# 54rt1n/shardmerge

Hardware: AMD Instinct MI355X
Metric: merged-weight GB/s per GPU + % HBM roofline, Llama-3-70B 3-way FFT merge (higher is better)
Workload: dtype f32; 1 GPU; Llama-3-70B block tensors, this rank's 1/8 slice (9 per block x 10 blocks), K=3 finetunes, bf16 in/out, resident in HBM; workload_id=llama3-70b-slice, k=3, parallelism=tensor-partition x1 (no data-path collective), streams_per_gpu=8

## Files before the change

shardmerge_amd/csrc/sm_capi.inc:

```

struct smhip_ctx {
    smhip::Pipeline<SM_BACKEND> pipe;
    explicit smhip_ctx(int device) : pipe(device) {}
};

#define SM_GUARD(ctx)                      \
    if (!(ctx)) return SMHIP_ERR_ARG;      \
    (ctx)->pipe.err.clear();
#define SM_FINISH(ctx, rc)                                                        \
    do {                                                                          \
        int rc__ = (rc);                                                          \
        if (rc__ == SMHIP_OK && !(ctx)->pipe.be.ok()) {                           \
            (ctx)->pipe.err = (ctx)->pipe.be.error();                             \
            rc__ = SMHIP_ERR_HIP;                                                 \
        }                                                                         \
        return rc__;                                                              \
    } while (0)

template <class Desc, class Scalars>
static int delta_tensor_check(smhip_ctx* ctx, const char* op, const Desc* d, const void* out, const float* delta_out,
                              bool need_base, Scalars scalars) {
    auto bad = [&](const char* what) { return ctx->pipe.fail(SMHIP_ERR_ARG, std::string(op) + ": " + what); };
    if (!d) return bad("null descriptor");
    if (d->k < 1 || d->k > SMHIP_MAX_MODELS) return bad("k out of range (1..16)");
// ... 160 lines not shown
    SM_FINISH(ctx, ctx->pipe.ties_merge(*d, out, delta_out, report));
}

int smhip_dare_merge(smhip_ctx* ctx, const smhip_dare_desc* d, void* out, float* delta_out, smhip_dare_report* report,
                     void* stream) {
    SM_GUARD(ctx);
    if (int rc = delta_merge_check(ctx, "dare_merge", d, out, delta_out)) return rc;
    if (ctx->pipe.dare_threshold(d->density) == 0)
        return ctx->pipe.fail(SMHIP_ERR_ARG, "dare_merge: density is below the smallest density, 2^-16 = 1.52587890625e-05 (the mask draws 16 bits per element)");
    ctx->pipe.stream = stream;
    SM_FINISH(ctx, ctx->pipe.dare_merge(*d, out, delta_out, report));
}

int smhip_breadcrumbs_merge(smhip_ctx* ctx, const smhip_breadcrumbs_desc* d, void* out, float* delta_out,
                            smhip_breadcrumbs_report* report, void* stream) {
    SM_GUARD(ctx);
    if (int rc = delta_merge_check(ctx, "breadcrumbs_merge", d, out, delta_out)) return rc;
    if (!(d->gamma >= 0.0 && d->gamma < 1.0)) return ctx->pipe.fail(SMHIP_ERR_ARG, "breadcrumbs_merge: gamma must be in [0, 1)");
    if (!(d->density + d->gamma <= 1.0)) return ctx->pipe.fail(SMHIP_ERR_ARG, "breadcrumbs_merge: density + gamma must not exceed 1");
    ctx->pipe.stream = stream;
    SM_FINISH(ctx, ctx->pipe.breadcrumbs_merge(*d, out, delta_out, report));
}

int smhip_geo_merge(smhip_ctx* ctx, const smhip_geo_desc* d, void* out, float* delta_out, smhip_geo_report* report,
                    void* stream) {
    SM_GUARD(ctx);
    const bool weight = d && d->mode == SMHIP_GEO_SLERP;
    if (int rc = delta_tensor_check(ctx, "geo_merge", d, out, delta_out, !weight, [&]() -> const char* {
            if (d->mode < SMHIP_GEO_MODEL_STOCK || d->mode > SMHIP_GEO_SLERP) return "bad mode";
            if (d->mode == SMHIP_GEO_MODEL_STOCK) return nullptr;
            if (d->rowwise) return "rowwise is an option of mode MODEL_STOCK";
            if (d->k > 2) return "modes NUSLERP and SLERP take k <= 2";
            if (d->k == 2 && !(d->alpha[0] >= 0.0 && d->alpha[1] >= 0.0 && d->alpha[0] + d->alpha[1] > 0.0 &&
                               std::isfinite(d->alpha[0] + d->alpha[1])))
                return "modes NUSLERP and SLERP need alphas >= 0 with a sum > 0";
            return nullptr;
        }))
        return rc;
    if (d->n > 0 && (d->rows < 1 || d->n % d->rows)) return ctx->pipe.fail(SMHIP_ERR_ARG, "geo_merge: rows must divide n");
    ctx->pipe.stream = stream;
    SM_FINISH(ctx, ctx->pipe.geo_merge(*d, out, delta_out, report));
}

int smhip_slerp(smhip_ctx* ctx, const float* v0, const float* v1, size_t rows, size_t cols, float t, float* out, void* stream) {
    SM_GUARD(ctx);
    if (rows * cols > 0 && (!v0 || !v1 || !out)) return ctx->pipe.fail(SMHIP_ERR_ARG, "bad argument");
    ctx->pipe.stream = stream;
    SM_FINISH(ctx, ctx->pipe.fn_slerp(v0, v1, rows, cols, t, out));
}

int smhip_div_scalar(smhip_ctx* ctx, const void* x, int dtype, size_t n, float s, void* out, void* stream) {
    SM_GUARD(ctx);
    if (n > 0 && (!x || !out)) return ctx->pipe.fail(SMHIP_ERR_ARG, "bad argument");
    if (dtype < SMHIP_BF16 || dtype > SMHIP_F32) return ctx->pipe.fail(SMHIP_ERR_ARG, "bad dtype");
    ctx->pipe.stream = stream;
    SM_FINISH(ctx, ctx->pipe.fn_div_scalar(x, dtype, n, s, out));
}

int smhip_lora_apply(smhip_ctx* ctx, const void* base, int dtype, int rows, int cols, const void* lora_a,
                     const void* lora_b, int factor_dtype, int rank, float scale, void* out, void* stream) {
    SM_GUARD(ctx);
    if (!base || !lora_a || !lora_b || !out || rows < 1 || cols < 1) return ctx->pipe.fail(SMHIP_ERR_ARG, "bad argument");
    if (dtype < SMHIP_BF16 || dtype > SMHIP_F32 || factor_dtype < SMHIP_BF16 || factor_dtype > SMHIP_F32)
        return ctx->pipe.fail(SMHIP_ERR_ARG, "bad dtype");
    if (rank < 1 || rank > smhip::LORA_MAX_RANK) return ctx->pipe.fail(SMHIP_ERR_ARG, "rank out of range (1..512)");
    const size_t bes = dtype == SMHIP_F32 ? 4 : 2, fes = factor_dtype == SMHIP_F32 ? 4 : 2;
    const uintptr_t o0 = (uintptr_t)out, o1 = o0 + (size_t)rows * cols * bes;
    auto overlaps = [&](const void* p, size_t bytes) { return (uintptr_t)p < o1 && o0 < (uintptr_t)p + bytes; };
    if (overlaps(base, (size_t)rows * cols * bes) || overlaps(lora_a, (size_t)rank * cols * fes) ||
        overlaps(lora_b, (size_t)rows * rank * fes))
        return ctx->pipe.fail(SMHIP_ERR_ARG, "lora_apply: out overlaps an input");
    ctx->pipe.stream = stream;
    SM_FINISH(ctx, ctx->pipe.lora_apply(base, dtype, rows, cols, lora_a, lora_b, factor_dtype, rank, scale, out));
}

int smhip_adapter_apply(smhip_ctx* ctx, const smhip_adapter_desc* d, void* stream) {
    SM_GUARD(ctx);
    if (!d || !d->base || !d->lora_a || !d->lora_b || !d->out || d->rows < 1 || d->cols < 1)
        return ctx->pipe.fail(SMHIP_ERR_ARG, "bad argument");
    if (d->dtype < SMHIP_BF16 || d->dtype > SMHIP_F32 || d->factor_dtype < SMHIP_BF16 || d->factor_dtype > SMHIP_F32 ||
        (d->magnitude && (d->magnitude_dtype < SMHIP_BF16 || d->magnitude_dtype > SMHIP_F32)))
        return ctx->pipe.fail(SMHIP_ERR_ARG, "bad dtype");
    if (d->layout != SMHIP_ADAPTER_LINEAR && d->layout != SMHIP_ADAPTER_EMBEDDING)
        return ctx->pipe.fail(SMHIP_ERR_ARG, "adapter_apply: bad layout");
    if (d->magnitude && d->layout != SMHIP_ADAPTER_LINEAR)
        return ctx->pipe.fail(SMHIP_ERR_ARG, "adapter_apply: DoRA (a magnitude) needs the LINEAR layout");
    if (d->rank < 1 || d->rank > smhip::LORA_MAX_RANK) return ctx->pipe.fail(SMHIP_ERR_ARG, "rank out of range (1..512)");
    const size_t bes = d->dtype == SMHIP_F32 ? 4 : 2, fes = d->factor_dtype == SMHIP_F32 ? 4 : 2;
    const size_t mes = d->magnitude_dtype == SMHIP_F32 ? 4 : 2;
    const bool emb = d->layout == SMHIP_ADAPTER_EMBEDDING;
    const uintptr_t o0 = (uintptr_t)d->out, o1 = o0 + (size_t)d->rows * d->cols * bes;
    auto overlaps = [&](const void* p, size_t bytes) { return (uintptr_t)p < o1 && o0 < (uintptr_t)p + bytes; };
    if (overlaps(d->base, (size_t)d->rows * d->cols * bes) ||
        overlaps(d->lora_a, (size_t)d->rank * (emb ? d->rows : d->cols) * fes) ||
        overlaps(d->lora_b, (size_t)(emb ? d->cols : d->rows) * d->rank * fes) ||
        (d->magnitude && overlaps(d->magnitude, (size_t)d->rows * mes)))
        return ctx->pipe.fail(SMHIP_ERR_ARG, "adapter_apply: out overlaps an input");
    ctx->pipe.stream = stream;
    SM_FINISH(ctx, ctx->pipe.adapter_apply(d->base, d->dtype, d->rows, d->cols, d->lora_a, d->lora_b, d->factor_dtype,
                                           d->rank, d->scale, emb ? 1 : 0, d->magnitude, d->magnitude_dtype, d->out));
}

int smhip_exact_norm(smhip_ctx* ctx, const void* x, int dtype, size_t n, double* norm_out, void* stream) {
    SM_GUARD(ctx);
    if (!norm_out || (n > 0 && !x)) return ctx->pipe.fail(SMHIP_ERR_ARG, "bad argument");
    if (dtype < SMHIP_BF16 || dtype > SMHIP_F32) return ctx->pipe.fail(SMHIP_ERR_ARG, "bad dtype");
    ctx->pipe.stream = stream;
    SM_FINISH(ctx, ctx->pipe.fn_exact_norm(x, dtype, n, norm_out));
}

int smhip_correlate_pairs(smhip_ctx* ctx, int k, const void* const* tensors, int dtype, size_t rows, size_t cols,
                          float* matrix_out, void* stream) {
    SM_GUARD(ctx);
    if (!tensors || !matrix_out || rows < 1 || cols < 1) return ctx->pipe.fail(SMHIP_ERR_ARG, "bad argument");
    if (dtype < SMHIP_BF16 || dtype > SMHIP_F32) return ctx->pipe.fail(SMHIP_ERR_ARG, "bad dtype");
    for (int i = 0; i < k && i < 8; ++i)
        if (!tensors[i]) return ctx->pipe.fail(SMHIP_ERR_ARG, "null tensor");
    ctx->pipe.stream = stream;
    SM_FINISH(ctx, ctx->pipe.correlate_pairs(k, tensors, dtype, rows, cols, matrix_out));
}

int smhip_reference_cpu_norm(smhip_ctx* ctx, const void* x, const void* base, int dtype, size_t n, float* norm_out,
                             void* stream) {
    SM_GUARD(ctx);
    if (!x || !norm_out) return ctx->pipe.fail(SMHIP_ERR_ARG, "bad argument");
    if (dtype < SMHIP_BF16 || dtype > SMHIP_F32) return ctx->pipe.fail(SMHIP_ERR_ARG, "bad dtype");
    ctx->pipe.stream = stream;
    const int rc0 = ctx->pipe.reserve(1, 1);
    if (rc0) SM_FINISH(ctx, rc0);
    smhip::SigDesc sg{x, base, dtype, 1.f};
    double out = 0;
    if (!ctx->pipe.run_serial_norms(&sg, 1, n, &out))
        return ctx->pipe.fail(SMHIP_ERR_ARG, "reference_cpu norm: inputs must be 16-byte aligned");
    *norm_out = (float)out;
    SM_FINISH(ctx, SMHIP_OK);
}

int smhip_debug_option(smhip_ctx* ctx, const char* key, long value) {
    SM_GUARD(ctx);
    if (key && std::string(key) == "aten_overlap") { ctx->pipe.aten_overlap = value != 0; return SMHIP_OK; }
    if (key && std::string(key) == "emf_max_sample") { ctx->pipe.emf_max_sample = value >= 1 && value <= 4096 ? (int)value : smhip::EMF_MAX_SAMPLE; return SMHIP_OK; }
    if (key && std::string(key) == "aten_serial") { ctx->pipe.aten_serial = value != 0; return SMHIP_OK; }
    if (key && std::string(key) == "class_norms") { ctx->pipe.class_norms_mode = value >= 0 && value <= 2 ? (int)value : 1; return SMHIP_OK; }
    if (key && std::string(key) == "cand_cap") { ctx->pipe.debug_cand_cap = value > 0 ? (uint32_t)value : 0u; return SMHIP_OK; }
    if (key && std::string(key) == "sel_chunks") { ctx->pipe.debug_sel_chunks = value > 0 ? (uint32_t)value : 0u; return SMHIP_OK; }
    if (key && std::string(key) == "sel_flush_always") { ctx->pipe.debug_flush_always = value != 0; return SMHIP_OK; }
    if (key && std::string(key) == "fuse_norms") { ctx->pipe.fuse_norms = value != 0; return SMHIP_OK; }
    if (key && std::string(key) == "noise_seed") { ctx->pipe.noise_seed_base = (uint32_t)value; return SMHIP_OK; }
    if (key && std::string(key) == "spectral_intermediates") { ctx->pipe.spectral_inter = value != 0; return SMHIP_OK; }
    if (key && std::string(key) == "fuse_spec_norm") { ctx->pipe.fuse_spec_norm = value != 0; return SMHIP_OK; }
    if (key && std::string(key) == "sel_wgs_per_cu") { ctx->pipe.sel_wgs_per_cu = value > 0 ? (int)value : 5; return SMHIP_OK; }
    if (key && std::string(key) == "pair1d") { ctx->pipe.pair1d_enabled = value != 0; return SMHIP_OK; }
    if (key && std::string(key) == "spec_cull") { ctx->pipe.spec_cull = value != 0; return SMHIP_OK; }
    if (key && std::string(key) == "spec_min_bins") { ctx->pipe.spec_min_bins = value >= 0 ? (size_t)value : (size_t)1 << 20; return SMHIP_OK; }
    if (key && std::string(key) == "dftp_pairs") { ctx->pipe.dftp_pairs_enabled = value != 0; return SMHIP_OK; }
    if (key && std::string(key) == "f2s_pair") { ctx->pipe.f2s_pair = value != 0; return SMHIP_OK; }
    if (key && std::string(key) == "f1_multi") { ctx->pipe.f1_multi = value != 0; return SMHIP_OK; }
    if (key && std::string(key) == "force_bluestein") { ctx->pipe.debug_force_bluestein = value != 0; return SMHIP_OK; }
    if (key && std::string(key) == "force_split") { ctx->pipe.debug_force_split = value > 1 && value <= smhip::DFTP_MAX_P ? (int)value : 0; return SMHIP_OK; }
    if (key && std::string(key) == "fold_columns") { ctx->pipe.fold_enabled = value != 0; return SMHIP_OK; }
    if (key && std::string(key) == "fold_min_rows") { ctx->pipe.fold_min_rows = value > 0 ? (int)value : SM_FOLD_MIN_ROWS; return SMHIP_OK; }
    return ctx->pipe.fail(SMHIP_ERR_ARG, "unknown debug option");
}

int smhip_debug_query(smhip_ctx* ctx, const char* key, long* value) {
    SM_GUARD(ctx);
    if (!key || !value) return SMHIP_ERR_ARG;
    if (std::string(key) == "spec_hit") { *value = ctx->pipe.last_spec_verdict(); SM_FINISH(ctx, SMHIP_OK); }
    if (std::string(key) == "spec_checked" || std::string(key) == "spec_hits") {
        unsigned long long c = 0, h = 0;
        ctx->pipe.spec_totals(&c, &h);
        *value = (long)(std::string(key) == "spec_hits" ? h : c);
        SM_FINISH(ctx, SMHIP_OK);
    }
    if (std::string(key) == "aten_fast" || std::string(key) == "aten_group" || std::string(key) == "aten_slow") {
        unsigned long long v3[3];
        ctx->pipe.aten_stats(1, v3);
        *value = (long)v3[std::string(key) == "aten_fast" ? 0 : std::string(key) == "aten_group" ? 1 : 2];
        SM_FINISH(ctx, SMHIP_OK);
    }
    return ctx->pipe.fail(SMHIP_ERR_ARG, "unknown debug query");
}

int smhip_profile_enable(smhip_ctx* ctx, int on) { SM_GUARD(ctx); ctx->pipe.be.profile_enable(on != 0); return SMHIP_OK; }
int smhip_profile_reset(smhip_ctx* ctx) { SM_GUARD(ctx); ctx->pipe.be.profile_reset(); return SMHIP_OK; }
int smhip_profile_count(smhip_ctx* ctx) { return ctx ? ctx->pipe.be.profile_count() : 0; }
int smhip_profile_get(smhip_ctx* ctx, int i, const char** name, uint64_t* launches, double* total_ms) {
    SM_GUARD(ctx);
    return ctx->pipe.be.profile_get(i, name, launches, total_ms) ? SMHIP_OK : SMHIP_ERR_ARG;
}

}
```

shardmerge_amd/csrc/sm_kernels.hpp:

```cpp
#pragma once
#include <cmath>
#include <cstring>

#include "fft_engine.hpp"
#include "sm_aten_core.hpp"

namespace smhip {

struct cf4 { float x, y, z, w; };
struct u32x4 { uint32_t x, y, z, w; };

enum { DT_BF16 = 0, DT_F16 = 1, DT_F32 = 2 };

struct SigDesc {
    const void* x;
    const void* base;
    int dtype;
    float prescale;
};

SM_HD uint32_t umax(uint32_t a, uint32_t b) { return a > b ? a : b; }
SM_HD float u2f(uint32_t u) { float f; memcpy(&f, &u, 4); return f; }
SM_HD uint32_t f2u(float f) { uint32_t u; memcpy(&u, &f, 4); return u; }
SM_HD float bf16_to_f(uint32_t h) { return u2f(h << 16); }
// ... 1482 lines not shown
                                v *= p.post;
                                if (p.base) {
                                    v += bv[c];
                                    if (is_nan(v)) { v = 0.f; nan2++; }
                                    if (is_inf(v)) inf2 = 1;
                                }
                                o[c] = v;
                            }
                        }
                        if (p.norm_partials) {
                            float ps = 0.f;
#pragma unroll
                            for (int c = 0; c < 8; ++c) ps += o[c] * o[c];
                            ss += ps;
                        }
                        if (p.out_mode == OUT_BF16) {
                            u32x4 w;
                            w.x = pack_bf16x2(o[0], o[1]);
                            w.y = pack_bf16x2(o[2], o[3]);
                            w.z = pack_bf16x2(o[4], o[5]);
                            w.w = pack_bf16x2(o[6], o[7]);
                            ((u32x4*)p.out)[off / 8] = w;
                        } else {
                            cf4 w0 = {o[0], o[1], o[2], o[3]}, w1 = {o[4], o[5], o[6], o[7]};
                            ((cf4*)p.out)[off / 4] = w0;
                            ((cf4*)p.out)[off / 4 + 1] = w1;
                        }
                    }
                }
            } else {
#pragma unroll
                for (int q = 0; q < EMAX; ++q) {
                    const int n = t + q * T;
                    if (n < C) {
                        const size_t off = (size_t)row * C + n;
                        float v;
                        i2_finish(p, x[q], off, nan1, inf1, nan2, inf2, v);
                        ss += (double)v * v;
                        if (p.out_mode == OUT_BF16) ((uint16_t*)p.out)[off] = f_to_bf16(v);
                        else ((float*)p.out)[off] = v;
                    }
                }
            }
        });
        if (nan1) ex.global_atomic_add_u32(&p.flags[0], nan1);
        if (inf1) ex.global_atomic_or_u32(&p.flags[1], 1u);
        if (nan2) ex.global_atomic_add_u32(&p.flags[2], nan2);
        if (inf2) ex.global_atomic_or_u32(&p.flags[3], 1u);
        s.red[0] = ss; s.red[1] = 0.0;
    });
    if (p.norm_partials) {
        ex.sync();
        ex.template block_sum<2>(st, [&](const double* tot) {
            p.norm_partials[2 * (size_t)bid] = tot[0];
            p.norm_partials[2 * (size_t)bid + 1] = 0.0;
        });
    }
}

struct EmptyState { double red[8]; unsigned long long keep[8]; };

SM_HD int sgn(float v) { return (v > 0.f) - (v < 0.f); }
SM_HD bool same_sign(float a, float b) {
    const uint32_t ua = f2u(a), ub = f2u(b);
    const uint32_t ka = ua & 0x7fffffffu, kb = ub & 0x7fffffffu;
    const bool not_nan = ka <= 0x7f800000u && kb <= 0x7f800000u;
    const bool za = ka == 0u, zb = kb == 0u;
    const bool both_nonzero_same = !za && !zb && ((ua ^ ub) >> 31) == 0u;
    return not_nan && ((za && zb) || both_nonzero_same);
}


struct SelState {
    unsigned long long rank;
    uint32_t prefix;
    uint32_t level;
    float value;
    uint32_t pad;
};

struct HistParams {
    const float* X; const float* Y;
    int R, C, Cb;
    int vec4;
    int level;
    const SelState* sel;
    unsigned long long* hist;
    int chunks;
    const uint32_t* only_if;
};

SM_HD int load_quad(const float* src, size_t i0, size_t total, int vec4, float* out) {
    if (vec4) {
        const cf4 v = *(const cf4*)(src + i0);
        out[0] = v.x; out[1] = v.y; out[2] = v.z; out[3] = v.w;
        return 4;
    }
    int n = 0;
    for (int e = 0; e < 4; ++e) {
        if (i0 + e < total) { out[e] = src[i0 + e]; n = e + 1; } else out[e] = 0.f;
    }
    return n;
}

template <class Ex>
SM_HD void k_hist(Ex& ex, const HistParams& p) {
    typename Ex::template State<EmptyState> st;
    ex.init(st);
    uint32_t* lh = (uint32_t*)(ex.lds() + LDS_SCRATCH_FLOATS);
    const int nt = ex.nthreads();
    const int nbins = p.level == 1 ? HIST1_BINS : HIST_LO_BINS;
    const size_t total = (size_t)p.Cb * p.R;
    const size_t nquad = (total + 3) / 4;
    if (p.only_if && !*p.only_if) return;
    const uint32_t prefix = p.sel->prefix;
    const WeightRanges wr = weight_ranges(p.R, p.C, p.Cb);
    ex.each(st, [&](int tid, EmptyState&) { for (int b = tid; b < nbins; b += nt) lh[b] = 0; });
    ex.sync();
    ex.each(st, [&](int tid, EmptyState&) {
        const size_t start = (size_t)ex.bid() * p.chunks * nt;
        for (int c = 0; c < p.chunks; ++c) {
            const size_t qi = start + (size_t)c * nt + tid;
            if (qi >= nquad) break;
            const size_t i0 = 4 * qi;
            for (int which = 0; which < 2; ++which) {
                const float* src = which ? p.Y : p.X;
                if (!src) continue;
                float v[4];
                const int n = load_quad(src, i0, total, p.vec4, v);
#pragma unroll
                for (int e = 0; e < 4; ++e) {
                    if (e < n) {
                        const uint32_t w = weight_at(wr, i0 + e);
                        const uint32_t key = f2u(v[e]) & 0x7fffffffu;
                        if (p.level == 1) ex.lds_atomic_add(&lh[key >> 20], w);
                        else if (p.level == 2) { if ((key >> 20) == prefix) ex.lds_atomic_add(&lh[(key >> 10) & 1023u], w); }
                        else { if ((key >> 10) == prefix) ex.lds_atomic_add(&lh[key & 1023u], w); }
                    }
                }
            }
        }
    });
    ex.sync();
    ex.each(st, [&](int tid, EmptyState&) {
        for (int b = tid; b < nbins; b += nt) {
            const uint32_t v = lh[b];
            if (v) ex.global_atomic_add(&p.hist[b], (unsigned long long)v);
        }
    });
}

constexpr int STAGE_KEYS = 2048;
constexpr int STAGE_PAIRS = 1024;
struct CandLists {
    uint32_t* keys;
    cf4* pairs;
    uint32_t cap_keys, cap_pairs;
    uint32_t* counters;
};
struct BlendConsts {
    float thr;
    float dot;
    float cos_t, sin_t;
    float inv_rel;
    float pad[3];
    double s00, s01, s11;
    unsigned long long n_slerp;
};

struct Select2Params {
    const float* X; const float* Y;
    int R, C, Cb;
    int vec4;
    SelState* sel;
    const unsigned long long* hist1;
    unsigned long long rank;
    unsigned long long* hist;
    CandLists cand;
    int fuse_reduce;
    int sumsq;
    double* partials;
    int chunks;
    int flush_always;
    const uint32_t* skip;
    const float* blendB; float* blendR;
    const BlendConsts* consts; float t_sum;
    unsigned long long* hist1_out;
    const uint32_t* guess;
};

SM_HD float blend_slerp_one(const BlendConsts& c, float t_sum, float a, float b) {
    if (same_sign(a, b)) {
        if (fabsf(b) < c.thr) return a + t_sum * b;
        return a * c.cos_t + ((b - a * c.dot) * c.inv_rel) * c.sin_t;
    }
    return (fabsf(a) > fabsf(b)) ? a : b;
}

template <bool BLEND = false, class Ex>
SM_HD void k_select2(Ex& ex, const Select2Params& p) {
    typename Ex::template State<EmptyState> st;
    ex.init(st);
    uint32_t* lh = (uint32_t*)(ex.lds() + LDS_SCRATCH_FLOATS);
    uint32_t* lctl = lh + HIST_LO_BINS;
    uint32_t* lkeys = lctl + 8;
    cf4* lpairs = (cf4*)(lkeys + STAGE_KEYS);
    const int nt = ex.nthreads();
    const size_t total = (size_t)p.Cb * p.R;
    const size_t nquad = (total + 3) / 4;
    uint32_t* lh1 = lkeys + STAGE_KEYS;
    uint32_t prefix;
    BlendConsts bc;
    if constexpr (BLEND) {
        prefix = *p.guess - 1u;
        bc = *p.consts;
    } else {
        if (p.skip && *p.skip) return;
        wg_resolve(ex, st, p.hist1, HIST1_BINS, p.rank, (unsigned long long*)lkeys, lctl + 4);
        prefix = lctl[4];
        if (ex.bid() == 0) {
            ex.each(st, [&](int tid, EmptyState&) {
                if (tid == 0) {
                    p.sel->prefix = prefix; p.sel->level = 1;
                    p.sel->rank = (unsigned long long)lctl[5] | ((unsigned long long)lctl[6] << 32);
                }
            });
        }
        ex.sync();
    }
    const WeightRanges wr = weight_ranges(p.R, p.C, p.Cb);
    ex.each(st, [&](int tid, EmptyState&) {
        for (int b = tid; b < HIST_LO_BINS; b += nt) lh[b] = 0;
        if (tid < 8) lctl[tid] = 0;
        if constexpr (BLEND) for (int b = tid; b < HIST1_BINS; b += nt) lh1[b] = 0;
    });
    ex.sync();
#ifndef SM_SEL_ROUND
#define SM_SEL_ROUND 16
#endif
#ifndef SM_SEL_U
#define SM_SEL_U 4
#endif
#ifndef SM_DIAG_SEL
#define SM_DIAG_SEL 0
#endif
    constexpr int ROUND = SM_SEL_ROUND;
    ex.each(st, [&](int, EmptyState& s) { s.red[0] = s.red[1] = s.red[2] = s.red[3] = 0.0; });
    for (int r0 = 0; r0 < p.chunks; r0 += ROUND) {
    const int r1 = (r0 + ROUND < p.chunks) ? r0 + ROUND : p.chunks;
    ex.each(st, [&](int tid, EmptyState& s) {
        double s00 = 0, s01 = 0, s11 = 0, cnt = 0;
        const size_t start = (size_t)ex.bid() * p.chunks * nt;
        const bool hasY = !BLEND && p.Y != nullptr;
        auto quad = [&](size_t i0, const float* a_in, const float* b, int n, bool uniform_w) {
            float q00 = 0.f, q01 = 0.f, q11 = 0.f, qc = 0.f;
            const uint32_t w0 = weight_at(wr, i0);
            float rr[4];
            const float* a = a_in;
            if constexpr (BLEND) {
#pragma unroll
                for (int e = 0; e < 4; ++e) rr[e] = blend_slerp_one(bc, p.t_sum, a_in[e], b[e]);
                if (n == 4 && uniform_w) { cf4 v = {rr[0], rr[1], rr[2], rr[3]}; *(cf4*)(p.blendR + i0) = v; }
                else for (int e = 0; e < n; ++e) p.blendR[i0 + e] = rr[e];
                a = rr;
            }
            const uint32_t lo = prefix << 20, hi = lo + (1u << 20);
            const bool has_hi = prefix < 2047u;
            uint32_t ka[4], kb[4], wv[4];
            bool hit = false;
#pragma unroll
            for (int e = 0; e < 4; ++e) {
                wv[e] = (e < n) ? (uniform_w ? w0 : weight_at(wr, i0 + e)) : 0u;
                ka[e] = f2u(a[e]) & 0x7fffffffu;
                kb[e] = hasY ? (f2u(b[e]) & 0x7fffffffu) : 0u;
                hit = hit || ((e < n) && ((ka[e] - lo) < (1u << 20) || (hasY && (kb[e] - lo) < (1u << 20))));
            }
            if constexpr (BLEND) {
#pragma unroll
                for (int e = 0; e < 4; ++e) if (e < n) ex.lds_atomic_add(&lh1[ka[e] >> 20], wv[e]);
            }
            if (hit && !(SM_DIAG_SEL & 1)) {
#pragma unroll
                for (int e = 0; e < 4; ++e) {
                    if (e < n) {
                        const uint32_t w = wv[e];
                        if ((ka[e] - lo) < (1u << 20)) {
                            ex.lds_atomic_add(&lh[(ka[e] >> 10) & 1023u], w);
                            const uint32_t pos = ex.lds_atomic_add_ret(&lctl[0], 1u);
                            if (pos < (uint32_t)STAGE_KEYS) lkeys[pos] = ka[e] | ((w - 1u) << 31);
                        }
                        if (hasY && (kb[e] - lo) < (1u << 20)) {
                            ex.lds_atomic_add(&lh[(kb[e] >> 10) & 1023u], w);
                            const uint32_t pos = ex.lds_atomic_add_ret(&lctl[0], 1u);
                            if (pos < (uint32_t)STAGE_KEYS) lkeys[pos] = kb[e] | ((w - 1u) << 31);
                            if (p.fuse_reduce && same_sign(a[e], b[e])) {
                                const uint32_t pp = ex.lds_atomic_add_ret(&lctl[1], 1u);
                                if (pp < (uint32_t)STAGE_PAIRS) { cf4 v = {a[e], b[e], (float)w, 0.f}; lpairs[pp] = v; }
                            }
                        }
                    }
                }
            }
            if (p.sumsq) {
#pragma unroll
                for (int e = 0; e < 4; ++e) {
                    const bool in = (e < n) && has_hi && ka[e] >= hi;
                    const float av = in ? a[e] : 0.f;
                    q00 += ((float)wv[e] * av) * av;
                }
            }
            if (hasY && p.fuse_reduce && !(SM_DIAG_SEL & 2)) {
#pragma unroll
                for (int e = 0; e < 4; ++e) {
                    const bool in = (e < n) && has_hi && kb[e] >= hi && same_sign(a[e], b[e]);
                    const float wf = (float)wv[e];
                    const float av = in ? a[e] : 0.f, bv = in ? b[e] : 0.f;
                    const float wa = wf * av;
                    q00 += wa * av; q01 += wa * bv; q11 += (wf * bv) * bv; qc += in ? wf : 0.f;
                }
            }
            s00 += q00; s01 += q01; s11 += q11; cnt += qc;
        };
        if (p.vec4) {
            constexpr int U = SM_SEL_U;
            const cf4* X4 = (const cf4*)p.X;
            const cf4* Y4 = (const cf4*)(BLEND ? p.blendB : p.Y);
            for (int c0 = r0; c0 < r1; c0 += U) {
                cf4 av[U], bv[U];
                size_t qv[U];
#pragma unroll
                for (int u = 0; u < U; ++u) {
                    qv[u] = start + (size_t)(c0 + u) * nt + tid;
                    av[u] = X4[qv[u] < nquad ? qv[u] : nquad - 1];
                }
                if (hasY || BLEND) {
#pragma unroll
                    for (int u = 0; u < U; ++u) bv[u] = Y4[qv[u] < nquad ? qv[u] : nquad - 1];
                }
#pragma unroll
                for (int u = 0; u < U; ++u) {
                    if (c0 + u < r1 && qv[u] < nquad) {
                        const float a[4] = {av[u].x, av[u].y, av[u].z, av[u].w};
                        const float b[4] = {bv[u].x, bv[u].y, bv[u].z, bv[u].w};
                        quad(4 * qv[u], a, b, 4, !wr.full);
                    }
                }
            }
        } else {
            for (int c = r0; c < r1; ++c) {
                const size_t qi = start + (size_t)c * nt + tid;
                if (qi >= nquad) break;
                float a[4], b[4] = {0.f, 0.f, 0.f, 0.f};
                const int n = load_quad(p.X, 4 * qi, total, 0, a);
                if (hasY) load_quad(p.Y, 4 * qi, total, 0, b);
                if constexpr (BLEND) load_quad(p.blendB, 4 * qi, total, 0, b);
                quad(4 * qi, a, b, n, false);
            }
        }
        s.red[0] += s00; s.red[1] += s01; s.red[2] += s11; s.red[3] += cnt;
    });
    ex.sync();
    const bool last_round = r1 >= p.chunks;
    if (!last_round && !p.flush_always && lctl[0] <= (uint32_t)STAGE_KEYS / 2 && lctl[1] <= (uint32_t)STAGE_PAIRS / 2) continue;
    ex.each(st, [&](int tid, EmptyState&) {
        if (tid == 0) {
            uint32_t nk = lctl[0], np = lctl[1];
            bool over = false;
            if (nk > (uint32_t)STAGE_KEYS) { nk = STAGE_KEYS; over = true; }
            if (np > (uint32_t)STAGE_PAIRS) { np = STAGE_PAIRS; over = true; }
            const uint32_t bk = nk ? ex.global_atomic_add_ret_u32(&p.cand.counters[0], nk) : 0u;
            const uint32_t bp = np ? ex.global_atomic_add_ret_u32(&p.cand.counters[1], np) : 0u;
            if (bk + nk > p.cand.cap_keys || bp + np > p.cand.cap_pairs) over = true;
            if (over) { ex.global_atomic_or_u32(&p.cand.counters[2], 1u); if (!BLEND) ex.global_atomic_or_u32(&p.cand.counters[3], 1u); }
            lctl[0] = nk; lctl[1] = np; lctl[2] = bk; lctl[3] = bp;
        }
    });
    ex.sync();
    ex.each(st, [&](int tid, EmptyState&) {
        const uint32_t nk = lctl[0], np = lctl[1], bk = lctl[2], bp = lctl[3];
        for (uint32_t q = tid; q < nk; q += nt) if (bk + q < p.cand.cap_keys) p.cand.keys[bk + q] = lkeys[q];
        for (uint32_t q = tid; q < np; q += nt) if (bp + q < p.cand.cap_pairs) p.cand.pairs[bp + q] = lpairs[q];
    });
    ex.sync();
    ex.each(st, [&](int tid, EmptyState&) { if (tid < 4) lctl[tid] = 0; });
    ex.sync();
    }
    ex.each(st, [&](int tid, EmptyState&) {
        for (int b = tid; b < HIST_LO_BINS; b += nt) {
            const uint32_t v = lh[b];
            if (v) ex.global_atomic_add(&p.hist[b], (unsigned long long)v);
        }
        if constexpr (BLEND) {
            for (int b = tid; b < HIST1_BINS; b += nt) {
                const uint32_t v = lh1[b];
                if (v) ex.global_atomic_add(&p.hist1_out[b], (unsigned long long)v);
            }
        }
    });
    if (p.fuse_reduce || p.sumsq) {
        ex.sync();
        ex.template block_sum<4>(st, [&](const double* tot) {
            for (int q = 0; q < 4; ++q) p.partials[4 * (size_t)ex.bid() + q] = tot[q];
        });
    }
}

struct SpecCheckParams {
    const unsigned long long* hist1; unsigned long long rank;
    uint32_t* guess; uint32_t* flag;
    SelState* sel;
    unsigned long long* hist2;
    uint32_t* counters;
};
template <class Ex>
SM_HD void k_spec_check(Ex& ex, const SpecCheckParams& p) {
    typename Ex::template State<EmptyState> st;
    ex.init(st);
    const int nt = ex.nthreads();
    unsigned long long* scratch = (unsigned long long*)(ex.lds() + LDS_SCRATCH_FLOATS);
    uint32_t* res = (uint32_t*)(scratch + nt + 16);
    wg_resolve(ex, st, p.hist1, HIST1_BINS, p.rank, scratch, res);
    ex.each(st, [&](int tid, EmptyState&) {
        if (tid == 0) {
            const uint32_t g = *p.guess;
            const uint32_t hit = (g == res[0] + 1u) ? 1u : 0u;
            res[3] = hit;
            *p.flag = hit;
            p.flag[1] += 1u; p.flag[2] += hit;
            *p.guess = res[0] + 1u;
            if (hit) {
                p.sel->prefix = res[0]; p.sel->level = 1;
                p.sel->rank = (unsigned long long)res[1] | ((unsigned long long)res[2] << 32);
                if (p.counters[2]) p.counters[3] = 1u;
            }
        }
    });
    ex.sync();
    ex.each(st, [&](int tid, EmptyState&) {
        if (res[3]) return;
        for (int b = tid; b < HIST_LO_BINS; b += nt) p.hist2[b] = 0ull;
        if (tid < 3) p.counters[tid] = 0u;
    });
}

struct SumsqCandParams {
    CandLists cand;
    const float* thr;
    double* partials;
};
template <class Ex>
SM_HD void k_sumsq_cand(Ex& ex, const SumsqCandParams& p) {
    typename Ex::template State<EmptyState> st;
    ex.init(st);
    const int nt = ex.nthreads();
    const uint32_t n = p.cand.counters[2] ? 0u : p.cand.counters[0];
    const float thr = *p.thr;
    ex.each(st, [&](int tid, EmptyState& s) {
        double acc = 0;
        for (size_t q = (size_t)ex.bid() * nt + tid; q < n; q += (size_t)ex.nblocks() * nt) {
            const uint32_t v = p.cand.keys[q];
            const float x = u2f(v & 0x7fffffffu);
            if (!(x < thr)) acc += (double)(1u + (v >> 31)) * (double)x * (double)x;
        }
        s.red[0] = acc; s.red[1] = 0; s.red[2] = 0; s.red[3] = 0;
    });
    ex.template block_sum<4>(st, [&](const double* tot) {
        for (int q = 0; q < 4; ++q) p.partials[4 * (size_t)ex.bid() + q] = tot[q];
    });
}
struct SumSpecParams { const double* part4; int n4; const double* part1; int n1; double* out; uint32_t* zero_u32; int zero_u32_count; };
template <class Ex>
SM_HD void k_sum_spec(Ex& ex, const SumSpecParams& p) {
    typename Ex::template State<EmptyState> st;
    ex.init(st);
    const int nt = ex.nthreads();
    ex.each(st, [&](int tid, EmptyState& s) {
        double a0 = 0, a1 = 0;
        for (int i = tid; i < p.n4; i += nt) a0 += p.part4[4 * (size_t)i];
        for (int i = tid; i < p.n1; i += nt) a1 += p.part1[i];
        if (p.zero_u32 && tid < p.zero_u32_count) p.zero_u32[tid] = 0u;
        s.red[0] = a0; s.red[1] = a1;
    });
    ex.template block_sum<2>(st, [&](const double* tot) { p.out[0] = tot[0]; p.out[1] = tot[1]; });
}

struct Select3Params {
    CandLists cand;
    SelState* sel;
    const unsigned long long* hist2;
    unsigned long long* hist;
};
template <class Ex>
SM_HD void k_select3(Ex& ex, const Select3Params& p) {
    typename Ex::template State<EmptyState> st;
    ex.init(st);
    uint32_t* lh = (uint32_t*)(ex.lds() + LDS_SCRATCH_FLOATS);
    uint32_t* lres = lh + HIST_LO_BINS;
    unsigned long long* part = (unsigned long long*)(lres + 8);
    const int nt = ex.nthreads();
    const uint32_t n = p.cand.counters[2] ? 0u : p.cand.counters[0];
    const uint32_t prefix1 = p.sel->prefix;
    const unsigned long long rank1 = p.sel->rank;
    wg_resolve(ex, st, p.hist2, HIST_LO_BINS, rank1, part, lres);
    const uint32_t prefix = (prefix1 << 10) | lres[0];
    const unsigned long long rank2 = (unsigned long long)lres[1] | ((unsigned long long)lres[2] << 32);
    ex.each(st, [&](int tid, EmptyState&) { for (int b = tid; b < HIST_LO_BINS; b += nt) lh[b] = 0; });
    ex.sync();
    ex.each(st, [&](int tid, EmptyState&) {
        for (size_t q = (size_t)ex.bid() * nt + tid; q < n; q += (size_t)ex.nblocks() * nt) {
            const uint32_t v = p.cand.keys[q];
            const uint32_t key = v & 0x7fffffffu;
            if ((key >> 10) == prefix) ex.lds_atomic_add(&lh[key & 1023u], 1u + (v >> 31));
        }
    });
    ex.sync();
    ex.each(st, [&](int tid, EmptyState&) {
        for (int b = tid; b < HIST_LO_BINS; b += nt) {
            const uint32_t v = lh[b];
            if (v) ex.global_atomic_add(&p.hist[b], (unsigned long long)v);
        }
    });
    if (ex.bid() == 0) {
        ex.each(st, [&](int tid, EmptyState&) {
            if (tid == 0) { p.sel[1].prefix = prefix; p.sel[1].rank = rank2; p.sel[1].level = 2; }
        });
    }
}

struct ReduceCandParams {
    CandLists cand;
    const float* thr;
    double* partials;
};
template <class Ex>
SM_HD void k_reduce_cand(Ex& ex, const ReduceCandParams& p) {
    typename Ex::template State<EmptyState> st;
    ex.init(st);
    const int nt = ex.nthreads();
    const bool over = p.cand.counters[2] != 0;
    const uint32_t n = over ? 0u : p.cand.counters[1];
    const float thr = *p.thr;
    ex.each(st, [&](int tid, EmptyState& s) {
        double s00 = 0, s01 = 0, s11 = 0, cnt = 0;
        for (size_t q = (size_t)ex.bid() * nt + tid; q < n; q += (size_t)ex.nblocks() * nt) {
            const cf4 v = p.cand.pairs[q];
            if (!(fabsf(v.y) < thr)) {
                s00 += (double)v.z * v.x * v.x; s01 += (double)v.z * v.x * v.y; s11 += (double)v.z * v.y * v.y; cnt += v.z;
            }
        }
        s.red[0] = s00; s.red[1] = s01; s.red[2] = s11; s.red[3] = cnt;
    });
    ex.template block_sum<4>(st, [&](const double* tot) {
        for (int q = 0; q < 4; ++q) p.partials[4 * (size_t)ex.bid() + q] = tot[q];
    });
}

template <class Ex, class StT>
SM_HD void wg_resolve(Ex& ex, StT& st, const unsigned long long* hist, int nbins, unsigned long long rank,
                      unsigned long long* part, uint32_t* res) {
    using S = typename StT::value_type;
    const int nt = ex.nthreads();
    const int per = (nbins + nt - 1) / nt;
    unsigned long long* grp = part + nt;
    ex.each(st, [&](int tid, S& s) {
        unsigned long long sum = 0;
#pragma unroll
        for (int q = 0; q < 8; ++q) {
            const int b = tid * per + q;
            const unsigned long long h = (q < per && b < nbins) ? hist[b] : 0ull;
            s.keep[q] = h;
            sum += h;
        }
        part[tid] = sum;
        if (tid == 0) { res[0] = 0; res[1] = 0; res[2] = 0; }
    });
    ex.sync();
    ex.each(st, [&](int tid, S&) {
        if (tid < 16) {
// ... 428 lines not shown
            }
            if (p.hist) {
                const uint32_t w0 = weight_at(wr, i0);
#pragma unroll
                for (int e = 0; e < 4; ++e) {
                    if (e < n) {
                        const uint32_t key = f2u(r[e]) & 0x7fffffffu;
                        ex.lds_atomic_add(&lh[key >> 20], (vec && !wr.full) ? w0 : weight_at(wr, i0 + e));
                    }
                }
            }
        };
        if (p.vec4) {
            constexpr int U = 4;
            const cf4* A4 = (const cf4*)p.reA;
            const cf4* B4 = (const cf4*)p.reB;
            for (int q0 = 0; q0 < p.chunks; q0 += U) {
                cf4 av[U], bv[U];
                size_t qv[U];
#pragma unroll
                for (int u = 0; u < U; ++u) {
                    qv[u] = start + (size_t)(q0 + u) * nt + tid;
                    av[u] = A4[qv[u] < nquad ? qv[u] : nquad - 1];
                }
#pragma unroll
                for (int u = 0; u < U; ++u) bv[u] = B4[qv[u] < nquad ? qv[u] : nquad - 1];
#pragma unroll
                for (int u = 0; u < U; ++u) {
                    if (q0 + u < p.chunks && qv[u] < nquad) {
                        const float a[4] = {av[u].x, av[u].y, av[u].z, av[u].w};
                        const float b[4] = {bv[u].x, bv[u].y, bv[u].z, bv[u].w};
                        quad(4 * qv[u], a, b, 4, true);
                    }
                }
            }
        } else {
            for (int q = 0; q < p.chunks; ++q) {
                const size_t qi = start + (size_t)q * nt + tid;
                if (qi >= nquad) break;
                float a[4], b[4];
                const int n = load_quad(p.reA, 4 * qi, total, 0, a);
                load_quad(p.reB, 4 * qi, total, 0, b);
                quad(4 * qi, a, b, n, false);
            }
        }
    });
    if (p.hist) {
        ex.sync();
        ex.each(st, [&](int tid, EmptyState&) {
            for (int b = tid; b < HIST1_BINS; b += nt) {
                const uint32_t v = lh[b];
                if (v) ex.global_atomic_add(&p.hist[b], (unsigned long long)v);
            }
        });
    }
}

struct SpecNormParams {
    const float* re; const float* im;
    int R, C, Cb;
    int vec4;
    const float* thr;
    double* partials;
    int chunks;
};
template <class Ex>
SM_HD void k_spec_norm(Ex& ex, const SpecNormParams& p) {
    typename Ex::template State<EmptyState> st;
    ex.init(st);
    const int nt = ex.nthreads();
    const size_t total = (size_t)p.Cb * p.R;
    const size_t nquad = (total + 3) / 4;
    const float thr = p.thr ? *p.thr : 0.f;
    const WeightRanges wr = weight_ranges(p.R, p.C, p.Cb);
    ex.each(st, [&](int tid, EmptyState& s) {
        double sr = 0, si = 0;
        const size_t start = (size_t)ex.bid() * p.chunks * nt;
        for (int c = 0; c < p.chunks; ++c) {
            const size_t qi = start + (size_t)c * nt + tid;
            if (qi >= nquad) break;
            const size_t i0 = 4 * qi;
            float a[4], b[4];
            const int n = load_quad(p.re, i0, total, p.vec4, a);
            load_quad(p.im, i0, total, p.vec4, b);
            float qr = 0.f, qi2 = 0.f;
#pragma unroll
            for (int e = 0; e < 4; ++e) {
                if (e < n) {
                    const float w = (float)weight_at(wr, i0 + e);
                    if (!(fabsf(a[e]) < thr)) qr += w * a[e] * a[e];
                    qi2 += w * b[e] * b[e];
                }
            }
            sr += qr; si += qi2;
        }
        s.red[0] = sr; s.red[1] = si;
    });
    ex.template block_sum<2>(st, [&](const double* tot) {
        p.partials[2 * (size_t)ex.bid()] = tot[0];
        p.partials[2 * (size_t)ex.bid() + 1] = tot[1];
    });
}

SM_HD uint32_t hash_u32(uint32_t x) {
    x ^= x >> 16; x *= 0x7feb352du; x ^= x >> 15; x *= 0x846ca68bu; x ^= x >> 16;
    return x;
}
SM_HD float model_noise(uint32_t seed, size_t i, float sigma) {
    const uint32_t h1 = hash_u32((uint32_t)i * 2u + 1u + seed * 0x9e3779b9u) ^ hash_u32((uint32_t)(i >> 31) + seed);
    const uint32_t h2 = hash_u32(h1 + 0x68bc21ebu);
    if ((h2 >> 24) < 21u) return 0.f;
    const float s4 = (float)(h1 & 0xffffu) + (float)(h1 >> 16) + (float)(h2 & 0xffffu) + (float)(hash_u32(h2) >> 16);
    return sigma * 1.7320508f * (s4 * (1.0f / 65536.0f) - 2.0f);
}

struct SpecRescaleParams {
    const float* re; const float* im;
    float* dre; float* dim;
    int R, C, Cb;
    int vec4;
    float thr;
    float scale;
    float sigma; uint32_t seed;
    unsigned long long* hist;
    int chunks;
    double* im_partials;
};
template <class Ex>
SM_HD void k_spec_rescale(Ex& ex, const SpecRescaleParams& p) {
    typename Ex::template State<EmptyState> st;
    ex.init(st);
    uint32_t* lh = (uint32_t*)(ex.lds() + LDS_SCRATCH_FLOATS);
    const int nt = ex.nthreads();
    const size_t total = (size_t)p.Cb * p.R;
    const size_t nquad = (total + 3) / 4;
    const WeightRanges wr = weight_ranges(p.R, p.C, p.Cb);
    if (p.hist) {
        ex.each(st, [&](int tid, EmptyState&) { for (int b = tid; b < HIST1_BINS; b += nt) lh[b] = 0; });
        ex.sync();
    }
    ex.each(st, [&](int tid, EmptyState& s) {
        double imacc = 0.0;
        const size_t start = (size_t)ex.bid() * p.chunks * nt;
        for (int c = 0; c < p.chunks; ++c) {
            const size_t qi = start + (size_t)c * nt + tid;
            if (qi >= nquad) break;
            const size_t i0 = 4 * qi;
            float a[4], b[4] = {0.f, 0.f, 0.f, 0.f};
            const int n = load_quad(p.re, i0, total, p.vec4, a);
            if (p.im) load_quad(p.im, i0, total, p.vec4, b);
            float r[4], im[4];
#pragma unroll
            for (int e = 0; e < 4; ++e) {
                r[e] = (fabsf(a[e]) < p.thr) ? model_noise(p.seed, i0 + e, p.sigma) : a[e] * p.scale;
                im[e] = b[e] * p.scale;
            }
            if (p.vec4) {
                cf4 v = {r[0], r[1], r[2], r[3]};
                *(cf4*)(p.dre + i0) = v;
                if (p.im) { cf4 vi = {im[0], im[1], im[2], im[3]}; *(cf4*)(p.dim + i0) = vi; }
            } else {
                for (int e = 0; e < n; ++e) { p.dre[i0 + e] = r[e]; if (p.im) p.dim[i0 + e] = im[e]; }
            }
            if (p.hist) {
#pragma unroll
                for (int e = 0; e < 4; ++e)
                    if (e < n) ex.lds_atomic_add(&lh[(f2u(r[e]) & 0x7fffffffu) >> 20], weight_at(wr, i0 + e));
            }
            if (p.im_partials) {
                float q = 0.f;
#pragma unroll
                for (int e = 0; e < 4; ++e)
                    if (e < n) q += (float)weight_at(wr, i0 + e) * im[e] * im[e];
                imacc += q;
            }
        }
        s.red[0] = imacc;
    });
    if (p.hist) {
        ex.sync();
        ex.each(st, [&](int tid, EmptyState&) {
            for (int b = tid; b < HIST1_BINS; b += nt) {
                const uint32_t v = lh[b];
                if (v) ex.global_atomic_add(&p.hist[b], (unsigned long long)v);
            }
        });
    }
    if (p.im_partials) {
        ex.sync();
        ex.template block_sum<1>(st, [&](const double* tot) { p.im_partials[ex.bid()] = tot[0]; });
    }
}

constexpr int NORMS_MAX = 16;
constexpr int NORMS_K = 8;
struct DeltaNormsParams {
    int k;
    const void* ft[NORMS_K];
    const void* ubase[2];
    int base_of[NORMS_K];
    int dtype;
    size_t n;
    int chunks;
    double* partials;
};
template <class Ex>
SM_HD void k_delta_norms(Ex& ex, const DeltaNormsParams& p) {
    typename Ex::template State<NormsState> st;
    ex.init(st);
    const int nt = ex.nthreads();
    const size_t noct = p.n / 8;
    const u32x4* b0 = (const u32x4*)p.ubase[0];
    const u32x4* b1 = (const u32x4*)(p.ubase[1] ? p.ubase[1] : p.ubase[0]);
    ex.each(st, [&](int tid, NormsState& s) {
        double acc[NORMS_K];
#pragma unroll
        for (int i = 0; i < NORMS_K; ++i) acc[i] = 0.0;
        const size_t start = (size_t)ex.bid() * p.chunks * nt;
        for (int q = 0; q < p.chunks; ++q) {
            const size_t oi = start + (size_t)q * nt + tid;
            if (oi >= noct) break;
            u32x4 rf[NORMS_K];
            const u32x4 r0 = b0[oi], r1 = b1[oi];
#pragma unroll
            for (int i = 0; i < NORMS_K; ++i) rf[i] = ((const u32x4*)p.ft[i < p.k ? i : 0])[oi];
            float v0[8], v1[8];
            decode16x8(r0, p.dtype, v0);
            decode16x8(r1, p.dtype, v1);
#pragma unroll
            for (int i = 0; i < NORMS_K; ++i) {
                float vf[8];
                decode16x8(rf[i], p.dtype, vf);
                const bool second = p.base_of[i] != 0;
                float ps = 0.f;
#pragma unroll
                for (int e = 0; e < 8; ++e) {
                    const float d = vf[e] - (second ? v1[e] : v0[e]);
                    ps += d * d;
                }
                if (i < p.k) acc[i] += ps;
            }
        }
#pragma unroll
        for (int i = 0; i < NORMS_MAX; ++i) s.red[i] = i < NORMS_K ? acc[i < NORMS_K ? i : 0] : 0.0;
    });
    ex.template block_sum<NORMS_MAX>(st, [&](const double* tot) {
        for (int i = 0; i < NORMS_MAX; ++i) p.partials[(size_t)ex.bid() * NORMS_MAX + i] = tot[i];
    });
}
constexpr int SER_CHUNK = 4096;
struct SerialNormParams {
    int k;
    SigDesc sig[16];
    size_t n;
    float* out;
};
template <class Ex>
SM_HD void k_serial_norm(Ex& ex, const SerialNormParams& p) {
    typename Ex::template State<EmptyState> st;
    ex.init(st);
    float* buf = ex.lds() + LDS_SCRATCH_FLOATS;
    const int nt = ex.nthreads();
    const SigDesc sg = p.sig[ex.bid()];
    const size_t nchunks = (p.n + SER_CHUNK - 1) / SER_CHUNK;
    auto stage = [&](size_t c, int which) {
        ex.each(st, [&](int tid, EmptyState&) {
            float* dst = buf + which * SER_CHUNK;
            for (int o = tid; o < SER_CHUNK / 8; o += nt) {
                const size_t i0 = c * SER_CHUNK + (size_t)o * 8;
                float v[8];
                if (i0 < p.n) load_sig8(sg, i0, v);
                else { for (int e = 0; e < 8; ++e) v[e] = 0.f; }
#pragma unroll
                for (int e = 0; e < 8; ++e) dst[o * 8 + e] = v[e];
            }
        });
    };
    ex.each(st, [&](int, EmptyState& s) { s.red[0] = 0.0; });
    if (nchunks) stage(0, 0);
    ex.sync();
    for (size_t c = 0; c < nchunks; ++c) {
        const int cur = (int)(c & 1);
        if (c + 1 < nchunks) stage(c + 1, cur ^ 1);
        ex.each(st, [&](int tid, EmptyState& s) {
            if (tid < 8) {
                float acc = (float)s.red[0];
                const float* src = buf + cur * SER_CHUNK + tid;
                const size_t left = p.n - c * SER_CHUNK;
                const int rows = (int)((left < (size_t)SER_CHUNK ? left : (size_t)SER_CHUNK) / 8);
                int r = 0;
                for (; r + 16 <= rows; r += 16) {
                    float x[16];
#pragma unroll
                    for (int q = 0; q < 16; ++q) x[q] = src[(r + q) * 8];
#pragma unroll
                    for (int q = 0; q < 16; ++q) acc = fmaf(x[q], x[q], acc);
                }
                for (; r < rows; ++r) acc = fmaf(src[r * 8], src[r * 8], acc);
                s.red[0] = (double)acc;
            }
        });
        ex.sync();
    }
    float* lanes = buf;
    ex.each(st, [&](int tid, EmptyState& s) { if (tid < 8) lanes[tid] = (float)s.red[0]; });
    ex.sync();
    ex.each(st, [&](int tid, EmptyState&) {
// ... 1098 lines not shown
```

shardmerge_amd/csrc/sm_pipeline.hpp:

```cpp
#pragma once
#include <algorithm>
#include <cmath>
#include <cstdio>
#include <map>
#include <string>
#include <vector>

#include "../../include/shardmerge_hip.h"
#include "sm_kernels.hpp"
#include "sm_aten_norm.hpp"
#include "sm_bluestein.hpp"
#include "sm_lora.hpp"
#include "sm_ties.hpp"
#include "sm_dare.hpp"
#include "sm_breadcrumbs.hpp"
#include "sm_geo.hpp"

namespace smhip {

#define SM_KERNEL_TAG(Tag, ParamsT, NAME, CALL)                                      \
    struct Tag {                                                                     \
        using Params = ParamsT;                                                      \
        static constexpr int waves = 4;                                              \
        static constexpr int max_threads = 1024;                                     \
        static const char* name() { return NAME; }                                   \
        template <class Ex> static SM_HD void run(Ex& ex, const Params& p) { CALL; } \
    };
#define SM_KERNEL_TAG_LB(Tag, ParamsT, NAME, CALL, MAXT, WAVES)                      \
    struct Tag {                                                                     \
        using Params = ParamsT;                                                      \
        static constexpr int waves = WAVES;                                          \
        static constexpr int max_threads = MAXT;                                     \
        static const char* name() { return NAME; }                                   \
        template <class Ex> static SM_HD void run(Ex& ex, const Params& p) { CALL; } \
    };
template <class P, int GROUPS> constexpr int fft_max_threads() {
    if constexpr (P::is_static) return (GROUPS * P::T < 256) ? 256 : (GROUPS * P::T > 1024 ? 1024 : GROUPS * P::T);
    else return 1024;
}
#ifndef SM_W3_MAX_THREADS
#define SM_W3_MAX_THREADS 256
#endif
#define SM_FFT_KERNEL_TAG(Tag, ParamsT, NAME, CALL, GROUPS, WAVES)                   \
    template <class P> struct Tag {                                                  \
        using Params = ParamsT;                                                      \
        static constexpr int waves = (WAVES < 4 && P::is_static && fft_max_threads<P, GROUPS>() <= SM_W3_MAX_THREADS) ? WAVES : 4; \
        static constexpr int max_threads = waves < 4 ? fft_max_threads<P, GROUPS>() : 1024; \
        static const char* name() { return NAME; }                                   \
        template <class Ex> static SM_HD void run(Ex& ex, const Params& p) { CALL; } \
    };
SM_FFT_KERNEL_TAG(KF1, F1Params, "f1_rows_fwd", k_f1<P>(ex, p), 1, 3)
SM_FFT_KERNEL_TAG(KF2, F2Params, "f2_cols_fwd", (k_f2<P, f2_bins<P>()>(ex, p)), 2 * f2_bins<P>(), 4)
SM_FFT_KERNEL_TAG(KI1x1, I1Params, "i1_cols_inv", (k_i1<P, 1>(ex, p)), 1, 4)
SM_FFT_KERNEL_TAG(KI1x2, I1Params, "i1_cols_inv", (k_i1<P, i1_bins<P>()>(ex, p)), i1_bins<P>(), 4)
SM_FFT_KERNEL_TAG(KI2, I2Params, "i2_rows_inv", k_i2<P>(ex, p), 1, 4)
SM_FFT_KERNEL_TAG(KF2S, F2SParams, "f2s_cols_fwd1", (k_f2s<P, f2s_groups<P>()>(ex, p)), f2s_groups<P>(), 4)
SM_FFT_KERNEL_TAG(KF1Q, F1Params, "f1_rows_fwd", k_f1q<P>(ex, p), 4, 4)
SM_FFT_KERNEL_TAG(KF2Q, F2Params, "f2_cols_fwd", (k_f2<P, f2_bins<P>(), true>(ex, p)), 2 * f2_bins<P>(), 4)
SM_FFT_KERNEL_TAG(KF2SQ, F2SParams, "f2s_cols_fwd1", (k_f2s<P, f2s_groups<P>(), true>(ex, p)), f2s_groups<P>(), 4)
SM_FFT_KERNEL_TAG(KI1x1Q, I1Params, "i1_cols_inv", (k_i1<P, 1, true>(ex, p)), 1, 4)
SM_FFT_KERNEL_TAG(KI1x2Q, I1Params, "i1_cols_inv", (k_i1<P, i1_bins<P>(), true>(ex, p)), i1_bins<P>(), 4)
#define SM_BLUE_KERNEL_TAG(Tag, ParamsT, NAME, CALL)                                 \
    template <class P> struct Tag {                                                  \
        using Params = ParamsT;                                                      \
        static constexpr int max_threads = fft_max_threads<P, 1>();                  \
        static constexpr int waves = max_threads > 512 ? 4 : 2;                      \
        static const char* name() { return NAME; }                                   \
        template <class Ex> static SM_HD void run(Ex& ex, const Params& p) { CALL; } \
    };
SM_BLUE_KERNEL_TAG(KF1B, F1BParams, "f1_rows_fwd", k_f1b<P>(ex, p))
SM_BLUE_KERNEL_TAG(KI2B, I2BParams, "i2_rows_inv", k_i2b<P>(ex, p))
SM_FFT_KERNEL_TAG(KPair1d, Pair1dParams, "pair_1d", k_pair1d<P>(ex, p), 1, 1)

#ifndef SM_COLS_MAX_THREADS
#define SM_COLS_MAX_THREADS 1024
#endif
#ifndef SM_F2_MAX_THREADS
#define SM_F2_MAX_THREADS 512
#endif
#ifndef SM_R14336
#define SM_R14336 16, 16, 8, 7
#endif
#ifndef SM_R7168
#define SM_R7168 32, 32, 7
#endif
#ifndef SM_T8192
#define SM_T8192 256
#define SM_W8192 4
#define SM_R8192 32, 16, 16
#endif
#define SM_STATIC_PLANS(X)                 \
    X(SPlan<1024, 64, false, 4, 32, 32>)       \
    X(SPlan<2048, 64, false, 4, 16, 16, 8>)    \
    X(SPlan<4096, 128, false, 4, 16, 16, 16>)  \
    X(SPlan<8192, SM_T8192, false, SM_W8192, SM_R8192>)  \
    X(SPlan<16384, 512, false, 4, 32, 32, 16>)\
    X(SPlan<14336, 512, false, 4, SM_R14336>) \
    X(SPlan<28672, 1024, false, 4, 16, 16, 16, 7>) \
    X(SPlan<3072, 128, false, 4, 16, 16, 4, 3>)    \
    X(SPlan<3584, 128, false, 4, 16, 32, 7>)       \
    X(SPlan<5120, 256, false, 4, 16, 16, 4, 5>)    \
    X(SPlan<6144, 256, false, 4, 16, 16, 8, 3>)    \
    X(SPlan<7168, 256, false, 4, SM_R7168>)    \
    X(SPlan<12288, 512, false, 4, 16, 16, 16, 3>)  \
    X(SPlan<13824, 512, false, 4, 32, 16, 3, 3, 3>) \
    X(SPlan<27648, 1024, false, 4, 32, 32, 3, 3, 3>) \
    X(SPlan<2304, 128, false, 4, 16, 16, 3, 3>) \
    X(SPlan<256, 64, false, 4, 8, 8, 4>)            \
    X(SPlan<512, 64, false, 4, 32, 16>)             \
    X(SPlan<64, 64, false, 4, 8, 8>)                \
    X(SPlan<128, 64, false, 4, 16, 8>)

inline bool plan_uses_cx(int N) { (void)N; return false; }

template <class PL> inline void plan_from_static(int N, int& T, std::vector<int>& radices, bool& found) {
    if (!found && PL::N == N) {
        T = PL::T; radices.clear();
        for (int i = 0; i < PL::npass; ++i) radices.push_back(PL::radix(i));
        found = true;
    }
}
inline bool plan_shape_static(int N, int& T, std::vector<int>& radices) {
    bool found = false;
#define SM_PLAN_FROM(...) plan_from_static<__VA_ARGS__>(N, T, radices, found);
    SM_STATIC_PLANS(SM_PLAN_FROM)
#undef SM_PLAN_FROM
    return found;
}

template <class PL>
inline bool plan_matches(const FftPlanDev& pl) {
    if (pl.N != PL::N || pl.T != PL::T || pl.npass != PL::npass || pl.lds_floats != PL::lds_floats || (pl.cx != 0) != PL::cx) return false;
    for (int i = 0; i < PL::npass; ++i)
        if (pl.radix[i] != PL::radix(i)) return false;
    return true;
}
SM_KERNEL_TAG(KF2R1, F2Params, "f2_cols_fwd", k_f2_r1(ex, p))
SM_KERNEL_TAG(KI1R1, I1Params, "i1_cols_inv", k_i1_r1(ex, p))
SM_KERNEL_TAG(KPublish, PublishParams, "publish", k_publish(ex, p))
SM_KERNEL_TAG(KHist, HistParams, "select_hist", k_hist(ex, p))
SM_KERNEL_TAG(KScan, ScanParams, "select_scan", k_scan(ex, p))
SM_KERNEL_TAG(KSelect2, Select2Params, "select_lvl2", k_select2<false>(ex, p))
SM_KERNEL_TAG(KSelect2Cull, Select2Params, "select_lvl2_cull", k_select2<false>(ex, p))
SM_KERNEL_TAG(KBlendSel, Select2Params, "blend", k_select2<true>(ex, p))
SM_KERNEL_TAG(KSpecCheck, SpecCheckParams, "select_spec_check", k_spec_check(ex, p))
SM_KERNEL_TAG(KSelect3, Select3Params, "select_lvl3_cand", k_select3(ex, p))
SM_KERNEL_TAG(KReduceCand, ReduceCandParams, "slerp_reduce_cand", k_reduce_cand(ex, p))
SM_KERNEL_TAG(KReduce, ReduceParams, "slerp_reduce", k_reduce(ex, p))
SM_KERNEL_TAG(KSlerpConsts, SlerpConstParams, "slerp_consts", k_slerp_consts(ex, p))
SM_KERNEL_TAG_LB(KClassEmf, ClassEmfParams, "class_norm_stats", k_class_emf(ex, p), 256, 2)
SM_KERNEL_TAG(KSumPartials, SumPartialsParams, "sum_partials", k_sum_partials(ex, p))
SM_KERNEL_TAG(KDeltaNorms, DeltaNormsParams, "delta_norms", k_delta_norms(ex, p))
SM_KERNEL_TAG(KSumPartialsN, SumNParams, "sum_partials", k_sum_partials_n(ex, p))
SM_KERNEL_TAG(KBlend, BlendParams, "blend", k_blend(ex, p))
SM_KERNEL_TAG(KCombine, CombineParams, "combine", k_combine(ex, p))
SM_KERNEL_TAG(KExpand, ExpandParams, "expand_full", k_expand(ex, p))
SM_KERNEL_TAG(KPack, PackParams, "pack_planes", k_pack(ex, p))
SM_KERNEL_TAG(KSplit, SplitParams, "split_complex", k_split(ex, p))
SM_KERNEL_TAG(KJoin, JoinParams, "join_complex", k_join(ex, p))
SM_KERNEL_TAG(KCull, CullParams, "cull_inplace", k_cull(ex, p))
SM_KERNEL_TAG(KAddition, AdditionParams, "addition_merge", k_addition(ex, p))
SM_KERNEL_TAG(KFnSums, FnSumsParams, "fn_slerp_sums", k_fn_sums(ex, p))
SM_KERNEL_TAG(KFnSlerpFin, FnSlerpFinParams, "fn_slerp_consts", k_fn_slerp_fin(ex, p))
SM_KERNEL_TAG(KFnSlerpRows0, FnSlerpRowsParams, "fn_slerp_relnorm", k_fn_slerp_rows<0>(ex, p))
SM_KERNEL_TAG(KFnSlerpRows1, FnSlerpRowsParams, "fn_slerp_out", k_fn_slerp_rows<1>(ex, p))
SM_KERNEL_TAG(KFnSlerpDen, FnSlerpDenParams, "fn_slerp_den", k_fn_slerp_den(ex, p))
SM_KERNEL_TAG(KSumsqAny, SumsqAnyParams, "fn_sumsq", k_sumsq_any(ex, p))
SM_KERNEL_TAG(KDivScalar, DivScalarParams, "fn_div_scalar", k_div_scalar(ex, p))
SM_KERNEL_TAG(KCorrPartial, CorrPartialParams, "correlate_pairs", k_corr_partial(ex, p))
SM_KERNEL_TAG(KCorrFinish, CorrFinishParams, "correlate_finish", k_corr_finish(ex, p))
SM_KERNEL_TAG(KSerialNorm, SerialNormParams, "serial_norm", k_serial_norm(ex, p))
SM_KERNEL_TAG(KSpecNorm, SpecNormParams, "spec_norm", k_spec_norm(ex, p))
SM_KERNEL_TAG(KSumsqCand, SumsqCandParams, "spec_norm_cand", k_sumsq_cand(ex, p))
SM_KERNEL_TAG(KSumSpec, SumSpecParams, "spec_norm_sum", k_sum_spec(ex, p))
SM_KERNEL_TAG(KSpecRescale, SpecRescaleParams, "spec_rescale", k_spec_rescale(ex, p))
SM_KERNEL_TAG(KDftp, DftpParams, "dft_across_slices", k_dftp(ex, p))
SM_KERNEL_TAG(KDftpPairs, DftpParams, "dft_across_slices", k_dftp_pairs(ex, p))
SM_KERNEL_TAG(KTranspose, TransposeParams, "transpose", k_transpose(ex, p))
SM_KERNEL_TAG_LB(KLoraPack, LoraPackParams, "lora_pack", k_lora_pack(ex, p), 256, 4)
SM_KERNEL_TAG_LB(KLoraBf16, LoraApplyParams, "lora_apply", k_lora_apply<DT_BF16>(ex, p), 256, 2)
SM_KERNEL_TAG_LB(KLoraF16, LoraApplyParams, "lora_apply", k_lora_apply<DT_F16>(ex, p), 256, 2)
SM_KERNEL_TAG_LB(KLoraF32, LoraApplyParams, "lora_apply", k_lora_apply<DT_F32>(ex, p), 256, 2)
SM_KERNEL_TAG_LB(KDoraNormBf16, LoraApplyParams, "dora_norm", k_dora_norm<DT_BF16>(ex, p), 256, 2)
SM_KERNEL_TAG_LB(KDoraNormF16, LoraApplyParams, "dora_norm", k_dora_norm<DT_F16>(ex, p), 256, 2)
SM_KERNEL_TAG_LB(KDoraNormF32, LoraApplyParams, "dora_norm", k_dora_norm<DT_F32>(ex, p), 256, 2)
SM_KERNEL_TAG_LB(KDoraScale, DoraScaleParams, "dora_scale", k_dora_scale(ex, p), DORA_SCALE_THREADS, 4)
SM_KERNEL_TAG_LB(KDoraApplyBf16, LoraApplyParams, "dora_apply", k_dora_apply<DT_BF16>(ex, p), 256, 2)
SM_KERNEL_TAG_LB(KDoraApplyF16, LoraApplyParams, "dora_apply", k_dora_apply<DT_F16>(ex, p), 256, 2)
SM_KERNEL_TAG_LB(KDoraApplyF32, LoraApplyParams, "dora_apply", k_dora_apply<DT_F32>(ex, p), 256, 2)
SM_KERNEL_TAG_LB(KTiesHist, TiesHistParams, "ties_hist", k_ties_hist(ex, p), 256, 4)
SM_KERNEL_TAG_LB(KTiesSelect, TiesSelectParams, "ties_select", k_ties_select(ex, p), TIES_SELECT_THREADS, 4)
SM_KERNEL_TAG_LB(KTiesMerge, TiesMergeParams, "ties_merge", k_ties_merge(ex, p), 256, 4)
SM_KERNEL_TAG_LB(KDareMerge, DareMergeParams, "dare_merge", k_dare_merge(ex, p), 256, 4)
SM_KERNEL_TAG_LB(KCrumbsHist, CrumbsHistParams, "crumbs_hist", k_crumbs_hist(ex, p), 256, 4)
SM_KERNEL_TAG_LB(KCrumbsSelect, CrumbsSelectParams, "crumbs_select", k_crumbs_select(ex, p), TIES_SELECT_THREADS, 4)
SM_KERNEL_TAG_LB(KCrumbsMerge, CrumbsMergeParams, "crumbs_merge", k_crumbs_merge(ex, p), 256, 4)
SM_KERNEL_TAG_LB(KGeoGram, GeoGramParams, "geo_gram", k_geo_gram<false>(ex, p), GEO_THREADS, 4)
SM_KERNEL_TAG_LB(KGeoGramTiled, GeoGramParams, "geo_gram", k_geo_gram<true>(ex, p), GEO_THREADS, 2)
SM_KERNEL_TAG_LB(KGeoFold, GeoFoldParams, "geo_gram_fold", k_geo_fold(ex, p), 256, 4)
SM_KERNEL_TAG_LB(KGeoCoef, GeoCoefParams, "geo_coef", k_geo_coef(ex, p), 256, 4)
SM_KERNEL_TAG_LB(KGeoCombine, GeoCombineParams, "geo_combine", k_geo_combine(ex, p), 256, 4)
SM_KERNEL_TAG_LB(KAtenPre, AtenPreParams, "aten_norm_pre", k_aten_pre<0>(ex, p), 256, 4)
SM_KERNEL_TAG_LB(KAtenPreC, AtenPreParams, "aten_norm_pre", k_aten_pre<1>(ex, p), 256, 4)
SM_KERNEL_TAG_LB(KAtenScan, AtenScanParams, "aten_norm_scan", k_aten_scan(ex, p), 256, 4)
SM_KERNEL_TAG_LB(KAtenRec, AtenRecParams, "aten_norm_rec", k_aten_rec(ex, p), 256, 4)
#ifndef SM_ATEN_PART_WAVES
#define SM_ATEN_PART_WAVES 3
#endif
SM_KERNEL_TAG_LB(KAtenPart16, AtenPartParams, "aten_norm_part", k_aten_part<ATEN_PART_RAW16>(ex, p), 256, SM_ATEN_PART_WAVES)
SM_KERNEL_TAG_LB(KAtenPart32, AtenPartParams, "aten_norm_part", k_aten_part<ATEN_PART_RAW32>(ex, p), 256, SM_ATEN_PART_WAVES)
SM_KERNEL_TAG_LB(KAtenPart, AtenPartParams, "aten_norm_part", k_aten_part<ATEN_PART_SIGNAL>(ex, p), 256, 2)
SM_KERNEL_TAG_LB(KAtenPartC, AtenPartParams, "aten_norm_part", k_aten_part<ATEN_PART_CLASS>(ex, p), 256, 2)
SM_KERNEL_TAG_LB(KAtenWalk, AtenWalkParams, "aten_norm_walk", k_aten_walk<0>(ex, p), 256, 4)
SM_KERNEL_TAG_LB(KAtenWalkC, AtenWalkParams, "aten_norm_walk", k_aten_walk<1>(ex, p), 256, 4)
SM_KERNEL_TAG_LB(KAtenFinish, AtenFinishParams, "aten_norm_finish", k_aten_finish(ex, p), 256, 4)
#define SM_SIDE_KERNELS_0(X) X(KAtenPre) X(KAtenPreC) X(KAtenScan) X(KAtenRec) X(KAtenPart16) X(KAtenPart32) X(KAtenPart) X(KAtenPartC) X(KAtenWalk) X(KAtenWalkC) X(KAtenFinish)
#define SM_SIDE_KERNELS_1(X) X(KF2R1) X(KI1R1) X(KPublish) X(KHist) X(KScan) X(KSelect2) X(KSelect2Cull) X(KBlendSel) \
    X(KSpecCheck) X(KSelect3) X(KReduceCand) X(KReduce) X(KSlerpConsts) X(KSumPartials) X(KClassEmf)
#define SM_SIDE_KERNELS_2(X) X(KDeltaNorms) X(KSumPartialsN) X(KBlend) X(KCombine) X(KExpand) X(KPack) X(KSplit) X(KJoin) \
    X(KCull) X(KAddition) X(KFnSums) X(KFnSlerpFin) X(KFnSlerpRows0) X(KFnSlerpRows1) X(KFnSlerpDen) X(KSumsqAny) X(KDivScalar) X(KCorrPartial) X(KCorrFinish) X(KSerialNorm) X(KSpecNorm) X(KSumsqCand) X(KSumSpec)       \
    X(KSpecRescale) X(KDftp) X(KDftpPairs) X(KTranspose) X(KLoraPack) X(KLoraBf16) X(KLoraF16) X(KLoraF32) \
    X(KDoraNormBf16) X(KDoraNormF16) X(KDoraNormF32) X(KDoraScale) X(KDoraApplyBf16) X(KDoraApplyF16) X(KDoraApplyF32)
#define SM_SIDE_KERNELS_7(X) X(KTiesHist) X(KTiesSelect) X(KTiesMerge) X(KDareMerge) X(KCrumbsHist) X(KCrumbsSelect) X(KCrumbsMerge) \
    X(KGeoGram) X(KGeoGramTiled) X(KGeoFold) X(KGeoCoef) X(KGeoCombine)
#define SM_SIDE_GROUPS 8

struct HostPlan {
    FftPlanDev dev;
    bool ok = false;
};

inline bool plan_radices(int N, int T, std::vector<int>& out) {
    out.clear();
    if (N == 1) { out.push_back(1); return true; }
    int rest = N, a = 0;
    while (rest % 2 == 0) { rest /= 2; ++a; }
    std::vector<int> odd;
    for (int p : {3, 5, 7, 11, 13})
        while (rest % p == 0) { rest /= p; odd.push_back(p); }
    if (rest != 1) return false;
    if (a > 0) {
        const int np = (a + 4) / 5;
        const int base = a / np, extra = a % np;
        for (int i = 0; i < np; ++i) out.push_back(1 << (base + (i < extra ? 1 : 0)));
    }
    for (int p : odd) out.push_back(p);
    if ((int)out.size() > MAX_PASSES) return false;
    for (int r : out) {
        const int nb = N / r;
        const int per = (nb + T - 1) / T;
        if (per * r > EMAX) return false;
    }
    return true;
}


inline bool plan_shape(int N, int& T, std::vector<int>& radices) {
    if (N < 1 || N > EMAX * 1024) return false;
    if (plan_shape_static(N, T, radices)) return true;
    int t0 = ((N + EMAX - 1) / EMAX + 63) / 64 * 64;
    if (t0 < 64) t0 = 64;
    for (T = t0; T <= 1024; T += 64)
        if (plan_radices(N, T, radices)) return true;
    return false;
}

inline bool rough_split(int N, int& p, int& M) {
    int T;
    std::vector<int> rad;
    if (plan_shape(N, T, rad)) { p = 1; M = N; return true; }
    for (p = 2; p <= DFTP_MAX_P; ++p) {
        if (N % p) continue;
        M = N / p;
        if (M % 2 == 0 && plan_shape(M, T, rad)) return true;
    }
    return false;
}
inline int bluestein_len(int C) {
    if (C < 2) return 0;
    for (int L = 256; L <= EMAX * 1024; L *= 2)
        if (L >= 2 * C - 1) return L;
    return 0;
}
inline int shape_support(int rows, int cols, bool* transposed = nullptr) {
    int T, p, M;
    std::vector<int> rad;
    if (transposed) *transposed = false;
    if (rows < 1 || cols < 1) return 0;
    if (plan_shape(cols, T, rad) && rough_split(rows, p, M)) return 1;
    if (plan_shape(rows, T, rad) && rough_split(cols, p, M)) { if (transposed) *transposed = true; return 1; }
    if (bluestein_len(cols) && rough_split(rows, p, M)) return 1;
    if (bluestein_len(rows) && rough_split(cols, p, M)) { if (transposed) *transposed = true; return 1; }
    return 0;
}

struct Buffer {
    void* p = nullptr;
    size_t cap = 0;
};

struct ProfEntry { std::string name; uint64_t launches = 0; double ms = 0; };

inline size_t round_up(size_t v, size_t m) { return (v + m - 1) / m * m; }

struct PairOut {
    void* out = nullptr; int out_mode = OUT_F32;
    const void* base = nullptr; int base_dtype = DT_BF16;
    float post = 1.f;
    int ifft_policy = 1;
};

template <class B>
class Pipeline {
  public:
    B be;
    std::string err;
    void* stream = nullptr;
    uint32_t debug_cand_cap = 0;
    uint32_t debug_sel_chunks = 0;
    bool debug_flush_always = false;
    bool spec_cull = true;
    size_t spec_min_bins = 1 << 20;
    bool dftp_pairs_enabled = true;
    int debug_force_split = 0;
    int sel_wgs_per_cu = 5;
    bool safe_select = false;
    uint32_t noise_seed_base = 0;
    bool spectral_inter = true;
    bool f2s_pair = true;
    size_t f2s_pair_max_bins = (size_t)64 << 20;
    bool f1_multi = true;
    bool fuse_spec_norm = true;
    float noise_sigma = 1.2e-7f;

    explicit Pipeline(int device) : be(device) {}
    ~Pipeline() {
        for (auto& kv : plans_) if (kv.second.dev.tw) be.free((void*)kv.second.dev.tw);
        for (Buffer* b : {&cand_, &t1_, &small_, &tmpA_, &tmpB_, &tmpC_, &fullS_, &saveR_, &saveI_, &aten_, &emf_, &lora_, &dora_, &ties_}) if (b->p) be.free(b->p);
        for (Buffer& b : pool_) if (b.p) be.free(b.p);
        if (mail_) be.free_host(mail_);
        for (Buffer& b : inter_) if (b.p) be.free(b.p);
        for (Buffer& b : rowspec_) if (b.p) be.free(b.p);
        for (Buffer& b : tr_) if (b.p) be.free(b.p);
        for (auto& kv : rough_tw_) if (kv.second) be.free(kv.second);
        for (auto& kv : blue_) { if (kv.second.chirp) be.free(kv.second.chirp); if (kv.second.filt) be.free(kv.second.filt); }
    }

    int fail(int code, const std::string& msg) { err = msg; return code; }

    int get_plan(int N, FftPlanDev& out) {
        auto it = plans_.find(N);
        if (it == plans_.end()) {
            HostPlan hp;
            int T;
            std::vector<int> rad;
            if (plan_shape(N, T, rad)) {
                hp.ok = true;
                hp.dev.N = N; hp.dev.T = T; hp.dev.npass = (int)rad.size();
                for (int i = 0; i < MAX_PASSES; ++i) hp.dev.radix[i] = i < (int)rad.size() ? rad[i] : 1;
                hp.dev.cx = plan_uses_cx(N) ? 1 : 0;
                hp.dev.lds_floats = hp.dev.cx ? (int)round_up((size_t)2 * (N + (N >> 4) + 1), 32)
                                              : (int)round_up((size_t)lpad(N) + 1, 32);
                std::vector<cf2> tw(N);
                for (int j = 0; j < N; ++j) {
                    const double ang = -2.0 * M_PI * (double)j / (double)N;
                    tw[j].x = (float)cos(ang); tw[j].y = (float)sin(ang);
                }
                void* d = be.alloc(sizeof(cf2) * N);
                if (!d) return fail(SMHIP_ERR_NOMEM, "twiddle alloc failed");
                be.h2d(d, tw.data(), sizeof(cf2) * N, stream);
                hp.dev.tw = (const cf2*)d;
            } else {
                hp.dev.tw = nullptr;
            }
            it = plans_.emplace(N, hp).first;
        }
        if (!it->second.ok) {
            char buf[256];
            snprintf(buf, sizeof buf, "unsupported transform length %d (a row length needs factors in {2,3,5,7,11,13} and <= %d; the layer merge "
                                       "also takes p * M column lengths, p <= %d)", N, EMAX * 1024, DFTP_MAX_P);
            return fail(SMHIP_ERR_SHAPE, buf);
        }
        out = it->second.dev;
        return SMHIP_OK;
    }

    int ensure(Buffer& b, size_t bytes) {
        if (b.cap >= bytes) return SMHIP_OK;
        if (b.p) { be.sync(stream); be.free(b.p); b.p = nullptr; b.cap = 0; }
        b.p = be.alloc(bytes);
        if (!b.p) return fail(SMHIP_ERR_NOMEM, "workspace allocation failed");
        b.cap = bytes;
        return SMHIP_OK;
    }
    size_t workspace_bytes() const {
        size_t t = cand_.cap + t1_.cap + small_.cap + tmpA_.cap + tmpB_.cap + tmpC_.cap + fullS_.cap + saveR_.cap + saveI_.cap + aten_.cap + emf_.cap + lora_.cap + dora_.cap + ties_.cap;
        for (const Buffer& b : inter_) t += b.cap;
        for (const Buffer& b : rowspec_) t += b.cap;
        for (const Buffer& b : pool_) t += b.cap;
        for (const Buffer& b : tr_) t += b.cap;
        return t;
    }

    struct Geo {
        int R, C, Cb, pitch4, pitchG, ilv;
        size_t plane_floats;
        bool full;
        int Cw;
        int fold;
        int batch;
        size_t t1_slice;
        int rough;
    };
#ifndef SM_FOLD_MIN_ROWS
#define SM_FOLD_MIN_ROWS 14336
#endif
    int fold_min_rows = SM_FOLD_MIN_ROWS;
    bool fold_shape(int R, int C) const {
        if (R < fold_min_rows || !(R == 8192 || R == 14336 || R == 16384 || R == 28672)) return false;
        int T; std::vector<int> rad;
        if (!plan_shape_static(C, T, rad)) return false;
        return 4 * T <= 1024 && (C / T) % 2 == 0 && C % 8 == 0;
    }
    bool fold_enabled = true;
    Geo geo(int R, int C, bool full = false, bool allow_fold = false, int batch = 1) const {
        Geo g;
        g.R = R; g.C = C; g.full = full;
        g.batch = batch < 1 ? 1 : batch;
        g.fold = (allow_fold && fold_enabled && !full && g.batch == 1 && fold_shape(R, C) && !row_bluestein(C)) ? 4 : 1;
        g.Cb = full ? C : (C / 2 + 1) * g.batch;
        g.pitch4 = (int)round_up((size_t)(C / 2 + 1), 8);
        g.t1_slice = round_up((size_t)R, 8) * (size_t)g.pitch4;
        g.pitchG = g.pitch4;
        g.ilv = t1_interleave(R);
        g.plane_floats = round_up((size_t)g.Cb * R, 64);
        g.Cw = full ? -1 : C;
        g.rough = 1;
        return g;
    }
#ifndef SM_T1_ILV
#define SM_T1_ILV 2
#endif
#ifndef SM_T1_ILV_MIN_ROWS
#define SM_T1_ILV_MIN_ROWS 8192
#endif
    static int t1_interleave(int R) { return t1_interleave_rows(R); }
    static constexpr int MAXGRID_PART = 1 << 20;
    int reserve(int R, int C, bool full = false, int batch = 1) {
        const Geo g = geo(R, C, full, false, batch);
        int rc;
        if ((rc = ensure(t1_, g.t1_slice * g.batch * sizeof(cf4)))) return rc;
        for (int i = 0; i < 4; ++i)
            if ((rc = ensure(pool_[pidx_[i]], g.plane_floats * sizeof(float)))) return rc;
        {
            const size_t ck = std::max<size_t>(1 << 16, g.plane_floats / 4), cp = std::max<size_t>(1 << 15, g.plane_floats / 16);
            if ((rc = ensure(cand_, ck * 4 + cp * 16))) return rc;
            cap_keys_ = (uint32_t)std::min<size_t>(ck, 0xffffffffu); cap_pairs_ = (uint32_t)std::min<size_t>(cp, 0xffffffffu);
        }
        if (!small_.p) {
            if ((rc = ensure(small_, SMALL_BYTES))) return rc;
            be.memset(small_.p, 0, SMALL_BYTES, stream);
            if (!mail_) mail_ = (Mailbox*)be.alloc_host(sizeof(Mailbox));
            if (!mail_) return fail(SMHIP_ERR_NOMEM, "host mailbox");
        }
        return SMHIP_OK;
    }
    static constexpr size_t OFF_HIST = 0;
    static constexpr size_t OFF_SEL = OFF_HIST + 8 * (HIST1_BINS + 2 * HIST_LO_BINS);
    static constexpr size_t OFF_CONSTS = OFF_SEL + 2 * sizeof(SelState);
    static constexpr size_t OFF_THR = OFF_CONSTS + 256;
    static constexpr size_t OFF_FLAGS = OFF_THR + 64;
    static constexpr size_t OFF_CANDCTR = OFF_FLAGS + 32;
    static constexpr size_t OFF_NORM2 = OFF_FLAGS + 64;
    static constexpr size_t OFF_PART = OFF_NORM2 + 64;
    static constexpr size_t PART_DOUBLES = 4 * 65536 + 2 * 40000;
    static constexpr size_t OFF_PART_IM = OFF_PART + PART_DOUBLES * 8;
    static constexpr size_t PART_IM_DOUBLES = 131072;
    static constexpr size_t OFF_SPEC = OFF_PART_IM + PART_IM_DOUBLES * 8;
    static constexpr size_t SMALL_BYTES = OFF_SPEC + 64;
    unsigned long long* d_hist() { return (unsigned long long*)((char*)small_.p + OFF_HIST); }
    unsigned long long* d_hist2() { return d_hist() + HIST1_BINS; }
    unsigned long long* d_hist3() { return d_hist2() + HIST_LO_BINS; }
    SelState* d_sel(int i) { return (SelState*)((char*)small_.p + OFF_SEL) + i; }
    BlendConsts* d_consts() { return (BlendConsts*)((char*)small_.p + OFF_CONSTS); }
    float* d_thr(int i) { return (float*)((char*)small_.p + OFF_THR) + i; }
    uint32_t* d_flags() { return (uint32_t*)((char*)small_.p + OFF_FLAGS); }
    uint32_t* d_candctr() { return (uint32_t*)((char*)small_.p + OFF_CANDCTR); }
    CandLists cand_lists() {
        CandLists c;
        c.keys = (uint32_t*)cand_.p; c.pairs = (cf4*)((char*)cand_.p + (size_t)cap_keys_ * 4);
        c.cap_keys = cap_keys_; c.cap_pairs = cap_pairs_; c.counters = d_candctr();
        if (debug_cand_cap) { c.cap_keys = std::min(c.cap_keys, debug_cand_cap); c.cap_pairs = std::min(c.cap_pairs, debug_cand_cap); }
        return c;
    }
    double* d_norm2() { return (double*)((char*)small_.p + OFF_NORM2); }
    double* d_part() { return (double*)((char*)small_.p + OFF_PART); }
    double* d_part_im() { return (double*)((char*)small_.p + OFF_PART_IM); }
    uint32_t* d_spec_guess(int slot) { return (uint32_t*)((char*)small_.p + OFF_SPEC) + (slot < 0 ? 0 : slot > 7 ? 7 : slot); }
    uint32_t* d_spec_flag() { return (uint32_t*)((char*)small_.p + OFF_SPEC) + 8; }
    float* plane(const Geo&, int i) { return (float*)pool_[pidx_[i]].p; }
    enum { P_REA = 0, P_IMA = 1, P_REB = 2, P_RER = 3 };
    int pool_acquire(size_t bytes) {
        int id = -1;
        for (size_t q = 0; q < pool_.size(); ++q) if (!pool_busy_[q]) { id = (int)q; break; }
        if (id < 0) { pool_.emplace_back(); pool_busy_.push_back(0); id = (int)pool_.size() - 1; }
        if (ensure(pool_[id], bytes)) return -1;
        pool_busy_[id] = 1;
        return id;
    }
    void pool_release(int id) { if (id >= 0) pool_busy_[id] = 0; }

    static bool is_static_plan(const FftPlanDev& pl) {
        bool found = false;
#define SM_IS_PLAN(...) if (plan_matches<__VA_ARGS__>(pl)) found = true;
        SM_STATIC_PLANS(SM_IS_PLAN)
#undef SM_IS_PLAN
        return found;
    }
    static int f2_bins_host(const FftPlanDev& pl) { return is_static_plan(pl) ? f2_bins_for(pl.T, pl.N) : 1; }
    static int i1_bins_host(const FftPlanDev& pl) {
        if (2 * pl.T > SM_F2_MAX_THREADS) return 1;
        return is_static_plan(pl) ? i1_bins_for(pl.T) : 2;
    }

    template <template <class> class KT, class Params>
    void launch_fft(const FftPlanDev& pl, int grid, int block, size_t lds, const Params& p, bool allow_static = true) {
        bool done = !allow_static;
#define SM_TRY_PLAN(...)                                                     \
        if (!done && plan_matches<__VA_ARGS__>(pl)) {                        \
            be.template launch<KT<__VA_ARGS__>>(grid, block, lds, p, stream);\
            done = true;                                                     \
        }
        SM_STATIC_PLANS(SM_TRY_PLAN)
#undef SM_TRY_PLAN
        if (!done || !allow_static) be.template launch<KT<DynPlan>>(grid, block, lds, p, stream);
    }

    static int pick_chunks(size_t units, int block, int min_chunks, int wgs_per_cu = 5) {
        const size_t target = (size_t)256 * wgs_per_cu;
        size_t c = (units + (size_t)block * target - 1) / ((size_t)block * target);
        if (c < (size_t)min_chunks) c = min_chunks;
        if (c > 4096) c = 4096;
        return (int)c;
    }
    static int stream_grid(size_t units, int block, int chunks) {
        const size_t per = (size_t)block * chunks;
        size_t g = (units + per - 1) / per;
        return (int)std::max<size_t>(g, 1);
    }
    static bool aligned16(const void* p) { return ((uintptr_t)p & 15) == 0; }
    static int vec4(const Geo& g) { return g.full ? (((size_t)g.R * g.C) % 4 == 0) : (g.R % 4 == 0); }

    bool debug_force_bluestein = false;
    bool row_bluestein(int C) const {
        int T; std::vector<int> rad;
        if (debug_force_bluestein) return bluestein_len(C) > 0;
        return !plan_shape(C, T, rad) && bluestein_len(C) > 0;
    }
    struct BlueHost { void* chirp = nullptr; void* filt = nullptr; int L = 0; };
    int bluestein_tables(int C, BluesteinTab& out, FftPlanDev& plan) {
        const int L = bluestein_len(C);
        if (!L) return fail(SMHIP_ERR_SHAPE, "row length too long for the chirp-z transform");
        int rc = get_plan(L, plan);
        if (rc) return rc;
        auto it = blue_.find(C);
        if (it == blue_.end()) {
            std::vector<double> wr(C), wi(C);
            for (int n = 0; n < C; ++n) {
                const unsigned long long m = ((unsigned long long)n * (unsigned long long)n) % (2ull * (unsigned long long)C);
                const double ang = -M_PI * (double)m / (double)C;
                wr[n] = cos(ang); wi[n] = sin(ang);
            }
            std::vector<double> hr(L, 0.0), hi(L, 0.0);
            for (int m = 0; m < C; ++m) {
                hr[m] = wr[m]; hi[m] = -wi[m];
                if (m) { hr[L - m] = wr[m]; hi[L - m] = -wi[m]; }
            }
            for (int i = 1, j = 0; i < L; ++i) {
                int bit = L >> 1;
                for (; j & bit; bit >>= 1) j ^= bit;
                j ^= bit;
                if (i < j) { std::swap(hr[i], hr[j]); std::swap(hi[i], hi[j]); }
            }
            for (int len = 2; len <= L; len <<= 1) {
                const int half = len / 2;
                for (int k = 0; k < half; ++k) {
                    const double ang = -2.0 * M_PI * (double)k / (double)len;
                    const double cr = cos(ang), ci = sin(ang);
                    for (int i = k; i < L; i += len) {
                        const int j = i + half;
                        const double tr = hr[j] * cr - hi[j] * ci, ti = hr[j] * ci + hi[j] * cr;
                        hr[j] = hr[i] - tr; hi[j] = hi[i] - ti;
                        hr[i] += tr; hi[i] += ti;
                    }
                }
            }
            std::vector<cf2> chirp(C), filt(L);
            for (int n = 0; n < C; ++n) { chirp[n].x = (float)wr[n]; chirp[n].y = (float)wi[n]; }
            for (int k = 0; k < L; ++k) { filt[k].x = (float)(hr[k] / L); filt[k].y = (float)(hi[k] / L); }
            BlueHost bh;
            bh.L = L;
            bh.chirp = be.alloc(sizeof(cf2) * C);
            bh.filt = be.alloc(sizeof(cf2) * L);
            if (!bh.chirp || !bh.filt) return fail(SMHIP_ERR_NOMEM, "chirp table alloc failed");
            be.h2d(bh.chirp, chirp.data(), sizeof(cf2) * C, stream);
            be.h2d(bh.filt, filt.data(), sizeof(cf2) * L, stream);
            be.sync(stream);
            it = blue_.emplace(C, bh).first;
        }
        out.chirp = (const cf2*)it->second.chirp; out.filt = (const cf2*)it->second.filt;
        return SMHIP_OK;
    }
    int get_row_plan(int C, FftPlanDev& plan, bool& blue, BluesteinTab& bt) {
        blue = row_bluestein(C);
        bt.chirp = nullptr; bt.filt = nullptr;
        return blue ? bluestein_tables(C, bt, plan) : get_plan(C, plan);
    }

    int rough_twiddles(int N, const cf2** out) {
        auto it = rough_tw_.find(N);
        if (it == rough_tw_.end()) {
            std::vector<cf2> tw(N);
            for (int j = 0; j < N; ++j) {
                const double ang = -2.0 * M_PI * (double)j / (double)N;
                tw[j].x = (float)cos(ang); tw[j].y = (float)sin(ang);
            }
            void* d = be.alloc(sizeof(cf2) * N);
            if (!d) return fail(SMHIP_ERR_NOMEM, "twiddle alloc failed");
            be.h2d(d, tw.data(), sizeof(cf2) * N, stream);
            be.sync(stream);
            it = rough_tw_.emplace(N, d).first;
        }
        *out = (const cf2*)it->second;
        return SMHIP_OK;
    }
    int run_dftp(const Geo& g, void* buf, bool rowpair, int ilv, int pitch, size_t slice_stride, bool inverse) {
        DftpParams q;
        int rc = rough_twiddles(g.R * g.rough, &q.tw);
        if (rc) return rc;
        q.buf = (cf4*)buf; q.p = g.rough; q.M = g.R; q.units = rowpair ? g.R / 2 : g.R; q.rowpair = rowpair ? 1 : 0;
        q.ilv = ilv; q.pitch = pitch; q.ncols = g.C / 2 + 1; q.slice_stride = slice_stride; q.inverse = inverse ? 1 : 0;
        q.cols = DFTP_COLS;
        if (q.p <= DFTP_PAIR_MAX_P && dftp_pairs_enabled) {
            q.cols = dftp_pairs_cols(q.p);
            const int ntp = (q.ncols + q.cols - 1) / q.cols;
            const size_t ldsp = LDS_SCRATCH_FLOATS * 4 + dftp_pairs_lds_bytes(q.p) + ((size_t)(q.p / 2 + 1) + 64) * sizeof(cf2);
            be.template launch<KDftpPairs>((q.units + DFTP_UNITS - 1) / DFTP_UNITS * ntp, 256, ldsp, q, stream);
            return SMHIP_OK;
        }
        const int ntiles = (q.ncols + DFTP_COLS - 1) / DFTP_COLS;
        const size_t lds = LDS_SCRATCH_FLOATS * 4 + (size_t)q.p * DFTP_COLS * sizeof(cf4) + (size_t)q.p * sizeof(cf2);
        be.template launch<KDftp>(q.units * ntiles, 256, lds, q, stream);
// ... 106 lines not shown
        double* const pbase = p.partials;
        if (multi) {
            for (int i = 0; i < nm; ++i) multi->partials[i] = pbase + (size_t)i * 2 * grid;
            multi->b_off = (long long)((size_t)g.C * dt_size(sig.dtype));
            p.sigs = *multi;
            launch_fft<KF1>(p.plan, grid * nm, p.nb * p.plan.T, lds, p, true);
            if (grid_out) *grid_out = grid;
            return SMHIP_OK;
        }
        for (int bi = 0; bi < nlaunch; ++bi) {
            p.a = sig_at(a, (size_t)bi * g.R * g.C); p.b = sig_at(b, (size_t)bi * g.R * g.C);
            p.t1 = t1base + (size_t)bi * (g.t1_slice / 2);
            p.partials = pbase + (size_t)bi * 2 * grid;
            if (blue) { F1BParams q; q.f = p; q.bt = bt; launch_fft<KF1B>(p.plan, grid, p.plan.T, lds, q); }
            else launch_fft<KF1>(p.plan, grid, p.nb * p.plan.T, lds, p, p.vec != 0);
        }
        if (grid_out) *grid_out = grid * nlaunch;
        if (g.rough > 1) return run_dftp(g, t1base, true, F2S_ILV, g.pitch4, g.t1_slice / 2, false);
        return SMHIP_OK;
    }
    struct F2SSecond { const void* t1; bool role_a; float scale; };
    int run_f2s(const Geo& g, bool role_a, float scale, bool hist, const void* t1buf = nullptr, int* im_parts = nullptr,
                const F2SSecond* second = nullptr) {
        F2SParams p;
        p.two = 0; p.t1_2 = nullptr; p.role_a_2 = 0; p.scale_2 = 0.f; p.re_2 = nullptr;
        if (second) {
            if (g.batch != 1 || second->role_a == role_a) return fail(SMHIP_ERR_ARG, "internal: paired column pass");
            p.two = 1; p.t1_2 = (const cf4*)second->t1; p.role_a_2 = second->role_a ? 1 : 0; p.scale_2 = second->scale;
            p.re_2 = plane(g, second->role_a ? P_REA : P_REB);
        }
        const int nsg = second ? 2 : 1;
        const int Rt = g.R / g.fold;
        int rc = get_plan(Rt, p.plan);
        if (rc) return rc;
        p.t1 = (const cf4*)(t1buf ? t1buf : t1_.p); p.pitch4 = g.pitch4 * g.fold; p.R = Rt; p.C = g.C;
        p.Cb = g.fold == 4 ? 4 * g.pitch4 : g.C / 2 + 1;
        p.slab = g.pitch4; p.Cb_real = g.C / 2 + 1; p.Rfull = g.R; p.slab_elems = fold_slab_elems(g, true);
        p.role_a = role_a ? 1 : 0; p.scale = scale;
        p.re = plane(g, role_a ? P_REA : P_REB); p.im = plane(g, P_IMA);
        p.hist = hist ? d_hist() : nullptr;
        const bool st = is_static_plan(p.plan);
        const int G = st ? (f2_nsig_for(p.plan.T) == 2 ? 2 * f2_bins_for(p.plan.T, p.plan.N) : 1) : 1;
        const int xg = G >= 8 ? 1 : 8 / G;
        const int grid = (int)round_up((size_t)(p.Cb + G - 1) / G, 8 * xg) * nsg;
        const size_t lds = (LDS_SCRATCH_FLOATS + (size_t)G * p.plan.lds_floats + HIST1_BINS) * 4;
        const bool any_a = role_a || (second && second->role_a);
        const bool want_im = im_parts && any_a && (size_t)grid * g.batch <= PART_IM_DOUBLES;
        if (im_parts) *im_parts = want_im ? grid * g.batch : -1;
        p.im_partials = want_im ? d_part_im() : nullptr;
        if (g.fold == 4) { launch_fft<KF2SQ>(p.plan, grid, G * p.plan.T, lds, p); return SMHIP_OK; }
        if (g.batch > 1) { p.sl.wgs = grid; p.sl.t1_stride = g.t1_slice / 2; p.sl.plane_stride = (size_t)(g.C / 2 + 1) * g.R; }
        launch_fft<KF2S>(p.plan, grid * g.batch, G * p.plan.T, lds, p);
        return SMHIP_OK;
    }
    void run_spec_norm(const Geo& g, const float* re, const float* im, const float* thr, double& sre, double& sim) {
        const size_t total = (size_t)g.Cb * g.R;
        SpecNormParams q;
        q.re = re; q.im = im; q.R = g.R; q.C = g.Cw; q.Cb = g.Cb; q.vec4 = vec4(g); q.thr = thr;
        q.chunks = pick_chunks((total + 3) / 4, 256, 8, 8);
        int grid = stream_grid((total + 3) / 4, 256, q.chunks);
        while ((size_t)grid * 2 > PART_DOUBLES) { q.chunks *= 2; grid = stream_grid((total + 3) / 4, 256, q.chunks); }
        q.partials = d_part();
        be.template launch<KSpecNorm>(grid, 256, LDS_SCRATCH_FLOATS * 4, q, stream);
        SumPartialsParams sp;
        sp.partials = d_part(); sp.nparts = grid; sp.out = mail_->norm2;
        be.template launch<KSumPartials>(1, 1024, LDS_SCRATCH_FLOATS * 4, sp, stream);
        PublishParams pp;
        pp.flags = d_flags(); pp.thr = d_thr(0); pp.consts = d_consts(); pp.mail = mail_; pp.zero_flags = nullptr;
        be.template launch<KPublish>(1, 64, LDS_SCRATCH_FLOATS * 4, pp, stream);
        be.sync(stream);
        sre = mail_->norm2[0]; sim = mail_->norm2[1];
    }
    void run_spec_rescale(const Geo& g, const float* re, const float* im, float thr, float scale, bool role_a, bool hist,
                          int* im_parts = nullptr) {
        const size_t total = (size_t)g.Cb * g.R;
        SpecRescaleParams q;
        q.re = re; q.im = role_a ? im : nullptr;
        q.dre = plane(g, role_a ? P_REA : P_REB); q.dim = plane(g, P_IMA);
        q.R = g.R; q.C = g.Cw; q.Cb = g.Cb; q.vec4 = vec4(g);
        q.thr = thr; q.scale = scale; q.sigma = noise_sigma; q.seed = ++noise_seed_;
        q.hist = hist ? d_hist() : nullptr;
        q.chunks = pick_chunks((total + 3) / 4, 256, 8, 8);
        const int grid = stream_grid((total + 3) / 4, 256, q.chunks);
        const bool want_im = im_parts && role_a && (size_t)grid <= PART_IM_DOUBLES;
        if (im_parts) *im_parts = want_im ? grid : -1;
        q.im_partials = want_im ? d_part_im() : nullptr;
        be.template launch<KSpecRescale>(grid, 256, (LDS_SCRATCH_FLOATS + HIST1_BINS) * 4, q, stream);
    }
    void run_spec_norm_fused(int sel_parts, int im_parts, double& sre, double& sim) {
        SumsqCandParams sc;
        sc.cand = cand_lists(); sc.thr = d_thr(1); sc.partials = d_part() + 4 * (size_t)sel_parts;
        be.template launch<KSumsqCand>(CAND_GRID, 256, LDS_SCRATCH_FLOATS * 4, sc, stream);
        SumSpecParams sp;
        sp.part4 = d_part(); sp.n4 = sel_parts + CAND_GRID; sp.part1 = d_part_im(); sp.n1 = im_parts; sp.out = mail_->norm2;
        sp.zero_u32 = d_candctr(); sp.zero_u32_count = 3;
        be.template launch<KSumSpec>(1, 1024, LDS_SCRATCH_FLOATS * 4, sp, stream);
        PublishParams pp;
        pp.flags = d_flags(); pp.thr = d_thr(0); pp.consts = d_consts(); pp.mail = mail_; pp.zero_flags = nullptr;
        be.template launch<KPublish>(1, 64, LDS_SCRATCH_FLOATS * 4, pp, stream);
        be.sync(stream);
        sre = mail_->norm2[0]; sim = mail_->norm2[1];
    }

    void read_norms(int grid, double& na, double& nb) {
        SumPartialsParams sp;
        sp.partials = d_part(); sp.nparts = grid; sp.out = mail_->norm2;
        be.template launch<KSumPartials>(1, 1024, LDS_SCRATCH_FLOATS * 4, sp, stream);
        be.sync(stream);
        na = std::sqrt(mail_->norm2[0]); nb = std::sqrt(mail_->norm2[1]);
    }

    int run_f2(const Geo& g, float scale0, float scale1, int swap, bool hist) {
        F2Params p;
        int rc = get_plan(g.R, p.plan);
        if (rc) return rc;
        if (g.R == 1) {
            p.slab = g.pitch4; p.Cb_real = g.C / 2 + 1; p.Rfull = 1; p.slab_elems = 0;
            p.t1 = (const cf4*)t1_.p; p.pitch4 = g.pitch4; p.ilv = 1; p.R = 1; p.C = g.C; p.Cb = g.C / 2 + 1; p.nsig = 2;
            p.swap = swap; p.scale[0] = scale0; p.scale[1] = scale1;
            p.reA = plane(g, P_REA); p.imA = plane(g, P_IMA); p.reB = plane(g, P_REB);
            p.hist = hist ? d_hist() : nullptr;
            be.template launch<KF2R1>(std::max(1, std::min(64, (p.Cb + 255) / 256)), 256, (LDS_SCRATCH_FLOATS + HIST1_BINS) * 4, p, stream);
            return SMHIP_OK;
        }
        p.slab = g.pitch4; p.Cb_real = g.C / 2 + 1; p.Rfull = g.R; p.slab_elems = fold_slab_elems(g);
        if (g.fold == 4) {
            if ((rc = get_plan(g.R / 4, p.plan))) return rc;
            p.t1 = (const cf4*)t1_.p; p.pitch4 = 4 * g.pitch4; p.ilv = FOLD_ILV; p.R = g.R / 4; p.C = g.C; p.Cb = 4 * g.pitch4;
            p.nsig = 2; p.swap = swap; p.scale[0] = scale0; p.scale[1] = scale1;
            p.reA = plane(g, P_REA); p.imA = plane(g, P_IMA); p.reB = plane(g, P_REB);
            p.hist = hist ? d_hist() : nullptr;
            const int binsq = f2_bins_host(p.plan);
            const int gridq = (int)round_up((size_t)(p.Cb + binsq - 1) / binsq, 64);
            const size_t ldsq = (LDS_SCRATCH_FLOATS + (size_t)2 * binsq * p.plan.lds_floats + HIST1_BINS) * 4;
            launch_fft<KF2Q>(p.plan, gridq, 2 * binsq * p.plan.T, ldsq, p);
            return SMHIP_OK;
        }
        p.t1 = (const cf4*)t1_.p; p.pitch4 = g.pitch4; p.ilv = g.ilv; p.R = g.R; p.C = g.C; p.Cb = g.C / 2 + 1;
        p.nsig = f2_nsig_for(p.plan.T);
        p.swap = swap; p.scale[0] = scale0; p.scale[1] = scale1;
        p.reA = plane(g, P_REA); p.imA = plane(g, P_IMA); p.reB = plane(g, P_REB);
        p.hist = hist ? d_hist() : nullptr;
        const int bins = p.nsig == 2 ? f2_bins_host(p.plan) : 1;
        const int ngroups = p.nsig == 2 ? 2 * bins : 1;
        const int grid = p.nsig == 2 ? (int)round_up((size_t)(p.Cb + bins - 1) / bins, 64) : (int)round_up((size_t)p.Cb * 2, 128);
        const size_t lds = (LDS_SCRATCH_FLOATS + (size_t)ngroups * p.plan.lds_floats + HIST1_BINS) * 4;
        if (g.batch > 1) { p.sl.wgs = grid; p.sl.t1_stride = g.t1_slice; p.sl.plane_stride = (size_t)(g.C / 2 + 1) * g.R; }
        launch_fft<KF2>(p.plan, grid * g.batch, ngroups * p.plan.T, lds, p);
        return SMHIP_OK;
    }

    static constexpr int CAND_GRID = 256;
    void run_select(const Geo& g, const float* X, const float* Y, unsigned long long rank, bool level1_done, float* thr_out,
                    bool fuse_reduce = false, int* nparts_out = nullptr, bool sumsq = false, int spec_slot = -1) {
        const size_t total = (size_t)g.Cb * g.R;
        HistParams h;
        h.X = X; h.Y = Y; h.R = g.R; h.C = g.Cw; h.Cb = g.Cb; h.vec4 = vec4(g); h.sel = d_sel(0);
        h.hist = d_hist(); h.chunks = pick_chunks((total + 3) / 4, 256, 8); h.only_if = nullptr;
        const int hgrid = stream_grid((total + 3) / 4, 256, h.chunks);
        const size_t hlds = (LDS_SCRATCH_FLOATS + HIST1_BINS) * 4;
        const size_t scan_lds = (LDS_SCRATCH_FLOATS + 2 * 256 + 32) * 4;
        ScanParams s;
        s.hist = d_hist(); s.sel = d_sel(0); s.value_out = thr_out; s.zero_also = nullptr; s.zero_count = 0;
        s.zero_u32 = nullptr; s.zero_u32_count = 0;
        if (!level1_done) { h.level = 1; be.template launch<KHist>(hgrid, 256, hlds, h, stream); }
        if (nparts_out) *nparts_out = 0;
        if (safe_select) {
            s.nbins = HIST1_BINS; s.shift = 11; s.final_level = 0; s.init = 1; s.rank_init = rank;
            be.template launch<KScan>(1, 256, scan_lds, s, stream);
            for (int level = 2; level <= 3; ++level) {
                h.level = level;
                be.template launch<KHist>(hgrid, 256, hlds, h, stream);
                s.nbins = HIST_LO_BINS; s.shift = 10; s.final_level = (level == 3); s.init = 0;
                be.template launch<KScan>(1, 256, scan_lds, s, stream);
            }
            return;
        }
        Select2Params q;
        q.X = X; q.Y = Y; q.R = g.R; q.C = g.Cw; q.Cb = g.Cb; q.vec4 = vec4(g); q.sel = d_sel(0);
        q.hist1 = d_hist(); q.rank = rank; q.hist = d_hist2();
        q.cand = cand_lists(); q.fuse_reduce = (fuse_reduce && Y) ? 1 : 0; q.partials = d_part();
        q.sumsq = (sumsq && !Y) ? 1 : 0;
        q.flush_always = debug_flush_always ? 1 : 0;
        q.chunks = debug_sel_chunks ? (int)debug_sel_chunks : pick_chunks((total + 3) / 4, 256, 8, sel_wgs_per_cu);
        int grid2 = stream_grid((total + 3) / 4, 256, q.chunks);
        while ((size_t)(grid2 + CAND_GRID) * 4 > PART_DOUBLES) { q.chunks *= 2; grid2 = stream_grid((total + 3) / 4, 256, q.chunks); }
        const size_t lds2 = (LDS_SCRATCH_FLOATS + HIST_LO_BINS + 8 + STAGE_KEYS) * 4 + (size_t)STAGE_PAIRS * sizeof(cf4);
        q.skip = nullptr; q.blendB = nullptr; q.blendR = nullptr; q.consts = nullptr; q.t_sum = 0.f; q.hist1_out = nullptr; q.guess = nullptr;
        if (spec_slot >= 0) {
            SpecCheckParams sc;
            sc.hist1 = d_hist(); sc.rank = rank; sc.guess = d_spec_guess(spec_slot); sc.flag = d_spec_flag();
            sc.sel = d_sel(0); sc.hist2 = d_hist2(); sc.counters = d_candctr();
            be.template launch<KSpecCheck>(1, 256, LDS_SCRATCH_FLOATS * 4 + (256 + 16) * 8 + 16, sc, stream);
            q.skip = d_spec_flag();
            be.template launch<KSelect2Cull>(grid2, 256, lds2, q, stream);
        } else {
            be.template launch<KSelect2>(grid2, 256, lds2, q, stream);
        }

        Select3Params t3;
        t3.cand = q.cand; t3.sel = d_sel(0); t3.hist2 = d_hist2(); t3.hist = d_hist3();
        be.template launch<KSelect3>(CAND_GRID, 256, (LDS_SCRATCH_FLOATS + HIST_LO_BINS + 8 + 2 * 256 + 32) * 4, t3, stream);

        s.hist = d_hist3(); s.sel = d_sel(1); s.nbins = HIST_LO_BINS; s.shift = 10; s.final_level = 1; s.init = 0;
        s.zero_also = d_hist(); s.zero_count = HIST1_BINS + HIST_LO_BINS;
        if (!q.fuse_reduce && !q.sumsq) { s.zero_u32 = d_candctr(); s.zero_u32_count = 3; }
        be.template launch<KScan>(1, 256, scan_lds, s, stream);

        if (q.sumsq && nparts_out) *nparts_out = grid2;
        if (q.fuse_reduce) {
            ReduceCandParams rc;
            rc.cand = q.cand; rc.thr = thr_out; rc.partials = d_part() + 4 * (size_t)grid2;
            be.template launch<KReduceCand>(CAND_GRID, 256, LDS_SCRATCH_FLOATS * 4, rc, stream);
            if (nparts_out) *nparts_out = grid2 + CAND_GRID;
        }
    }

    void run_blend(const Geo& g, int mode, int agreement, float t, float t_sum, bool hist) {
        const size_t total = (size_t)g.Cb * g.R;
        BlendParams b;
        b.reA = plane(g, P_REA); b.reB = plane(g, P_REB); b.reR = plane(g, P_RER);
        b.R = g.R; b.C = g.Cw; b.Cb = g.Cb; b.vec4 = vec4(g);
        b.mode = mode; b.agreement = agreement; b.t = t; b.t_sum = t_sum;
        b.consts = d_consts(); b.hist = hist ? d_hist() : nullptr; b.chunks = pick_chunks((total + 3) / 4, 256, 8, 8);
        be.template launch<KBlend>(stream_grid((total + 3) / 4, 256, b.chunks), 256, (LDS_SCRATCH_FLOATS + HIST1_BINS) * 4, b, stream);
    }

    void run_blend_spec(const Geo& g, float t_sum, bool sumsq, int spec_slot) {
        const size_t total = (size_t)g.Cb * g.R;
        Select2Params q;
        q.X = plane(g, P_REA); q.Y = nullptr; q.R = g.R; q.C = g.Cw; q.Cb = g.Cb; q.vec4 = vec4(g); q.sel = d_sel(0);
        q.hist1 = nullptr; q.rank = 0; q.hist = d_hist2();
        q.cand = cand_lists(); q.fuse_reduce = 0; q.partials = d_part(); q.sumsq = sumsq ? 1 : 0;
        q.flush_always = debug_flush_always ? 1 : 0;
        q.chunks = cull_select_chunks(total);
        q.skip = nullptr;
        q.blendB = plane(g, P_REB); q.blendR = plane(g, P_RER); q.consts = d_consts(); q.t_sum = t_sum;
        q.hist1_out = d_hist(); q.guess = d_spec_guess(spec_slot);
        const int grid = stream_grid((total + 3) / 4, 256, q.chunks);
        const size_t lds = (LDS_SCRATCH_FLOATS + HIST_LO_BINS + 8 + STAGE_KEYS + HIST1_BINS) * 4;
        be.template launch<KBlendSel>(grid, 256, lds, q, stream);
    }
    long last_spec_verdict() {
        if (!small_.p) return -1;
        uint32_t v = 0;
        be.d2h(&v, d_spec_flag(), sizeof v, stream);
        be.sync(stream);
        return (long)v;
    }
    void spec_totals(unsigned long long* checked, unsigned long long* hits) {
        uint32_t v[3] = {0, 0, 0};
        if (small_.p) { be.d2h(v, d_spec_flag(), sizeof v, stream); be.sync(stream); }
        *checked = v[1]; *hits = v[2];
    }
    int cull_select_chunks(size_t total) const {
        int chunks = debug_sel_chunks ? (int)debug_sel_chunks : pick_chunks((total + 3) / 4, 256, 8, sel_wgs_per_cu);
        int grid2 = stream_grid((total + 3) / 4, 256, chunks);
        while ((size_t)(grid2 + CAND_GRID) * 4 > PART_DOUBLES) { chunks *= 2; grid2 = stream_grid((total + 3) / 4, 256, chunks); }
        return chunks;
    }

    void run_slerp_consts(const Geo& g, bool have_thr, float t, int fused_parts, const float* ref_norms = nullptr,
                          const double* emf_part = nullptr, int emf_nparts = 0, int emf_elo = 0) {
        const size_t total = (size_t)g.Cb * g.R;
        SlerpConstParams c;
        c.ref_norms = ref_norms; c.emf_part = emf_part; c.emf_nparts = emf_nparts; c.emf_elo = emf_elo;
        c.fallback = nullptr; c.nfallback = 0; c.overflow = nullptr;
        c.thr = have_thr ? d_thr(0) : nullptr; c.t = t; c.out = d_consts();
        c.zero_u32 = nullptr; c.zero_u32_count = 0;
        if (fused_parts > 0) {
            c.zero_u32 = d_candctr(); c.zero_u32_count = 3;
            c.partials = d_part(); c.nparts = fused_parts;
        } else {
            ReduceParams r;
            r.reA = plane(g, P_REA); r.reB = plane(g, P_REB); r.R = g.R; r.C = g.Cw; r.Cb = g.Cb; r.vec4 = vec4(g);
            r.thr = c.thr; r.chunks = pick_chunks((total + 3) / 4, 256, 16, 8); r.only_if = nullptr;
            int grid = stream_grid((total + 3) / 4, 256, r.chunks);
            while ((size_t)grid * 4 > PART_DOUBLES) { r.chunks *= 2; grid = stream_grid((total + 3) / 4, 256, r.chunks); }
            r.partials = d_part();
            be.template launch<KReduce>(grid, 256, LDS_SCRATCH_FLOATS * 4, r, stream);
            c.partials = r.partials; c.nparts = grid;
        }
        be.template launch<KSlerpConsts>(1, 256, (2 * LDS_SCRATCH_FLOATS + 4 * EMF_VALS + 8) * 4, c, stream);
    }

    int run_inverse(const Geo& g, const float* reR, const float* imA, const float* cull_thr, const PairOut& o,
                    int* norm_grid = nullptr, float cull_val = 0.f) {
        I1Params a;
        int rc = get_plan(g.R, a.plan);
        if (rc) return rc;
        const int Cb = g.C / 2 + 1;
        a.cull_thr = cull_thr; a.cull_val = cull_val; a.R = g.R; a.Cb = Cb;
        a.G = (cf2*)t1_.p; a.pitchG = g.pitchG;
        a.s = g.R == 1 ? 1 : i1_bins_host(a.plan);
        const size_t lds1 = (LDS_SCRATCH_FLOATS + (size_t)a.s * a.plan.lds_floats) * 4;
        const int grid1 = (int)round_up((size_t)(Cb + a.s - 1) / a.s, 8 * (16 / a.s));

        I2Params b;
        bool blue; BluesteinTab bt;
        if ((rc = get_row_plan(g.C, b.plan, blue, bt))) return rc;
        b.G = (const cf2*)t1_.p; b.pitchG = g.pitchG; b.R = g.R; b.C = g.C; b.Cb = Cb;
        b.nb = blue ? 1 : std::max(1, 256 / b.plan.T);
        b.vec = !blue && (g.C % 8 == 0) && aligned16(o.out) && aligned16(o.base);
        b.inv_n = (float)(1.0 / ((double)g.R * (double)g.rough * (double)g.C));
        b.ifft_policy = o.ifft_policy;
        b.post = o.post; b.base_dtype = o.base_dtype; b.out_mode = o.out_mode;
        b.flags = d_flags();
        const bool joint = joint_rows(g);
        if (joint) b.R = g.R * g.rough;
        const int pairs = (b.R + 1) / 2;
        const int grid2 = (pairs + b.nb - 1) / b.nb;
        const int nrow_launch = joint ? 1 : g.batch;
        const bool want_norm = norm_grid && (size_t)grid2 * 2 * nrow_launch <= PART_DOUBLES;
        if (norm_grid) *norm_grid = want_norm ? grid2 * nrow_launch : -1;
        const size_t lds2 = (LDS_SCRATCH_FLOATS + (size_t)b.nb * b.plan.lds_floats) * 4;
        const size_t pslice = (size_t)Cb * g.R, eslice = (size_t)g.R * g.C;
        const int phases = g.rough > 1 ? 2 : 1;
        for (int phase = 0; phase < phases; ++phase) {
        if (phase == 1 && (rc = run_dftp(g, t1_.p, true, 1, g.pitchG, g.t1_slice / 2, true))) return rc;
        for (int bi = 0; bi < g.batch; ++bi) {
            if (g.rough > 1) { a.G = (cf2*)t1_.p + (size_t)bi * g.t1_slice; b.G = a.G; }
            a.reR = reR + bi * pslice; a.imA = imA + bi * pslice;
            if (phases == 2 && phase == 0 && g.R > 1) {
                if (bi > 0) break;
                a.G = (cf2*)t1_.p;
                a.sl.wgs = grid1; a.sl.t1_stride = g.t1_slice; a.sl.plane_stride = pslice;
                const int gridj = grid1 * g.batch;
                if (a.s >= 2) launch_fft<KI1x2>(a.plan, gridj, a.s * a.plan.T, lds1, a);
                else launch_fft<KI1x1>(a.plan, gridj, a.plan.T, lds1, a);
                continue;
            }
            if (phases == 2 && phase == 1) {
            } else
            if (g.R == 1) {
                be.template launch<KI1R1>(std::max(1, std::min(64, (Cb + 255) / 256)), 256, LDS_SCRATCH_FLOATS * 4, a, stream);
            } else if (g.fold == 4) {
                if (a.s >= 2) launch_fft<KI1x2Q>(a.plan, grid1, a.s * a.plan.T, lds1, a);
                else launch_fft<KI1x1Q>(a.plan, grid1, a.plan.T, lds1, a);
            } else if (a.s >= 2) launch_fft<KI1x2>(a.plan, grid1, a.s * a.plan.T, lds1, a);
            else launch_fft<KI1x1>(a.plan, grid1, a.plan.T, lds1, a);
            if (phases == 2 && phase == 0) continue;
            if (joint) { if (bi > 0) break; b.G = (const cf2*)t1_.p; }
            b.base = o.base ? (const char*)o.base + bi * eslice * dt_size(o.base_dtype) : nullptr;
            b.out = (char*)o.out + bi * eslice * (o.out_mode == OUT_BF16 ? 2 : 4);
            b.norm_partials = want_norm ? d_part() + (size_t)bi * 2 * grid2 : nullptr;
            if (blue) { I2BParams q; q.i = b; q.bt = bt; launch_fft<KI2B>(b.plan, grid2, b.plan.T, lds2, q); }
            else launch_fft<KI2>(b.plan, grid2, b.nb * b.plan.T, lds2, b, b.vec != 0);
        }
        }
        return SMHIP_OK;
    }

    void run_combine(const SigDesc& a, const SigDesc& b, float ca, float cb, size_t n, float* out_f32,
                     const PairOut* fin, bool want_norms, int* grid_out = nullptr) {
        CombineParams c;
        c.a = a; c.b = b; c.ca = ca; c.cb = cb; c.n = n; c.out_f32 = out_f32;
        c.base = fin ? fin->base : nullptr; c.base_dtype = fin ? fin->base_dtype : DT_BF16;
        c.out_final = fin ? fin->out : nullptr; c.out_mode = fin ? fin->out_mode : OUT_F32;
        c.flags = d_flags();
        c.vec8 = (n % 8 == 0) && aligned16(a.x) && aligned16(a.base) && aligned16(b.x) && aligned16(b.base) &&
                 aligned16(out_f32) && aligned16(c.base) && aligned16(c.out_final);
        c.chunks = pick_chunks((n + 7) / 8, 256, 4, 8);
        int grid = stream_grid((n + 7) / 8, 256, c.chunks);
        while ((size_t)grid * 2 > PART_DOUBLES) { c.chunks *= 2; grid = stream_grid((n + 7) / 8, 256, c.chunks); }
        c.partials = want_norms ? d_part() : nullptr;
        be.template launch<KCombine>(grid, 256, LDS_SCRATCH_FLOATS * 4, c, stream);
        if (grid_out) *grid_out = grid;
    }

    void publish(bool zero_flags) {
        PublishParams pp;
        pp.flags = d_flags(); pp.thr = d_thr(0); pp.consts = d_consts(); pp.mail = mail_;
        pp.zero_flags = zero_flags ? d_flags() : nullptr;
        be.template launch<KPublish>(1, 64, LDS_SCRATCH_FLOATS * 4, pp, stream);
        be.sync(stream);
        if (zero_flags) flags_clean_ = true;
    }
    void read_blend_info(smhip_blend_info* info, bool have_cut, bool have_cull, bool have_consts, bool published = false) {
        if (!info) return;
        if (!published) publish(false);
        const BlendConsts c = mail_->consts;
        float thr[4];
        for (int i = 0; i < 4; ++i) thr[i] = mail_->thr[i];
        info->cutoff_threshold = have_cut ? thr[0] : 0.0;
        info->cull_threshold = have_cull ? thr[1] : 0.0;
        info->dot = have_consts ? c.dot : 0.0;
        info->s00 = have_consts ? c.s00 : 0.0; info->s01 = have_consts ? c.s01 : 0.0; info->s11 = have_consts ? c.s11 : 0.0;
        info->n_slerp = have_consts ? c.n_slerp : 0;
        info->t = 0.0; info->cull_pct = 0.0;
    }

    static unsigned long long pct_index(unsigned long long len, double pct) {
        unsigned long long idx = (unsigned long long)((double)len * pct);
        if (idx >= len) idx = len - 1;
        return idx;
    }

    void spectral_blend(const Geo& g, int mode, double t, double t_sum, double cutoff_pct, double cull_pct,
                        int agreement, bool level1_hist_done, bool& have_cull, int* sumsq_parts = nullptr, int spec_slot = 7) {
        const unsigned long long nfull = (unsigned long long)g.R * g.C * (unsigned long long)g.batch;
        have_cull = false;
        if (mode == BLEND_SLERP) {
            const bool have_cut = cutoff_pct > 0;
            int fused = 0;
            if (have_cut)
                run_select(g, plane(g, P_REA), plane(g, P_REB), pct_index(2 * nfull, cutoff_pct), level1_hist_done, d_thr(0),
                           true, &fused);
            const float* class_norms = nullptr;
            const double* emf_part = nullptr;
            int emf_nparts = 0, emf_elo = 0;
            if (ref_mode_ && class_norms_mode == 2 && !g.full) {
                AtenSrc cs[2];
                for (int w = 0; w < 2; ++w) {
                    memset(&cs[w], 0, sizeof(AtenSrc));
                    cs[w].kind = 1; cs[w].reA = plane(g, P_REA); cs[w].reB = plane(g, P_REB);
                    cs[w].thr = have_cut ? d_thr(0) : nullptr; cs[w].which = w;
                    cs[w].R = g.R; cs[w].C = g.Cw; cs[w].Cb = g.Cb; cs[w].n = (size_t)g.Cb * g.R;
                }
                if (run_aten_norms(cs, 2, false)) class_norms = d_aten_out();
            } else if (ref_mode_ && class_norms_mode == 1) {
                ClassEmfParams q;
                q.reA = plane(g, P_REA); q.reB = plane(g, P_REB); q.thr = have_cut ? d_thr(0) : nullptr;
                q.R = g.R; q.C = g.Cw; q.Cb = g.Cb; q.n = (size_t)g.Cb * g.R;
                q.elo = (int)std::floor(std::log2(0.03 * (double)nfull + 1.0)) - 11;
                q.sample = 1;
                while (q.sample < emf_max_sample && q.n / (2 * (size_t)q.sample) >= EMF_MIN_SAMPLED) q.sample *= 2;
                const size_t rows = (q.n + 7) / 8, npieces = (rows + 8 * (size_t)q.sample - 1) / (8 * (size_t)q.sample);
                q.iters = (int)std::max<size_t>(1, std::min<size_t>(64, (npieces + (size_t)32 * 384 - 1) / ((size_t)32 * 384)));
                const int grid = (int)std::max<size_t>(1, (npieces + (size_t)32 * q.iters - 1) / ((size_t)32 * q.iters));
                if (!ensure(emf_, (size_t)grid * 2 * EMF_VALS * sizeof(double))) {
                    q.partials = (double*)emf_.p;
                    be.template launch<KClassEmf>(grid, 256, LDS_SCRATCH_FLOATS * 4 * 2, q, stream);
                    emf_part = q.partials; emf_nparts = grid; emf_elo = q.elo;
                }
            }
            run_slerp_consts(g, have_cut, (float)t, fused, class_norms, emf_part, emf_nparts, emf_elo);
            const bool spec = cull_pct > 0 && spec_cull && !safe_select && !g.full && (size_t)g.Cb * g.R >= spec_min_bins;
            if (spec) run_blend_spec(g, (float)t_sum, sumsq_parts != nullptr, spec_slot);
            else run_blend(g, BLEND_SLERP, 1, (float)t, (float)t_sum, cull_pct > 0);
            if (sumsq_parts) *sumsq_parts = 0;
            if (cull_pct > 0) {
                run_select(g, plane(g, P_RER), nullptr, pct_index(nfull, cull_pct), true, d_thr(1), false, sumsq_parts,
                           sumsq_parts != nullptr, spec ? spec_slot : -1);
                have_cull = true;
            }
        } else {
            run_blend(g, BLEND_ARITH, agreement, (float)t, 1.f, false);
        }
    }

    bool pair1d_enabled = true;
    bool pair1d_ok(const Geo& g) const {
        return pair1d_enabled && g.R == 1 && g.batch == 1 && !g.full && g.C >= 2 && g.C <= PAIR1D_MAX_C && !row_bluestein(g.C);
    }
    int run_pair1d(const Geo& g, const SigDesc& A, const SigDesc& Bs, double na, double nb, double t, double t_sum,
                   double cutoff_pct, double cull_pct, const PairOut& o, int* norm_parts) {
        Pair1dParams q;
        int rc = get_plan(g.C, q.plan);
        if (rc) return rc;
        q.a = A; q.b = Bs; q.C = g.C;
        q.sa = (float)(1.0 / na); q.sb = (float)(1.0 / nb);
        q.t = (float)t; q.t_sum = (float)t_sum;
        const unsigned long long nfull = (unsigned long long)g.C;
        q.have_cut = cutoff_pct > 0; q.rank_cut = pct_index(2 * nfull, cutoff_pct);
        q.have_cull = cull_pct > 0; q.rank_cull = pct_index(nfull, cull_pct);
        memset(&q.fin, 0, sizeof q.fin);
        q.fin.R = 1; q.fin.C = g.C; q.fin.Cb = g.C / 2 + 1;
        q.fin.inv_n = (float)(1.0 / (double)g.C);
        q.fin.ifft_policy = o.ifft_policy; q.fin.post = o.post;
        q.fin.base = o.base; q.fin.base_dtype = o.base_dtype; q.fin.out = o.out; q.fin.out_mode = o.out_mode;
        q.fin.flags = d_flags();
        q.fin.norm_partials = norm_parts ? d_part() : nullptr;
        if (norm_parts) *norm_parts = 1;
        q.thr = d_thr(0); q.consts = d_consts();
        const size_t lds = (LDS_SCRATCH_FLOATS + (size_t)q.plan.lds_floats + 2 * (size_t)g.C + HIST1_BINS + 1024 + 64 + 16) * 4;
        launch_fft<KPair1d>(q.plan, 1, q.plan.T, lds, q);
        return SMHIP_OK;
    }

    int merge_pair_slerp(const float* v0, const float* v1, int R, int C, double t, double bthr, double t_sum,
                         double cutoff_pct, double cull_pct, float* out, double* n0o, double* n1o, int* branch,
                         smhip_blend_info* info) {
        return with_select_retry([&] {
            return merge_pair_slerp_once(v0, v1, R, C, t, bthr, t_sum, cutoff_pct, cull_pct, out, n0o, n1o, branch, info);
        });
    }
    int merge_pair_slerp_once(const float* v0, const float* v1, int R, int C, double t, double bthr, double t_sum,
                              double cutoff_pct, double cull_pct, float* out, double* n0o, double* n1o, int* branch,
                              smhip_blend_info* info) {
        const Geo g = geo(R, C, false, aligned16(v0) && aligned16(v1) && aligned16(out));
        int rc = reserve(R, C);
        if (rc) return rc;
        clear_flags();
        SigDesc a{v0, nullptr, DT_F32, 1.f}, b{v1, nullptr, DT_F32, 1.f};
        int grid;
        if ((rc = run_f1(g, a, b, grid))) return rc;
        double n0, n1;
        read_norms(grid, n0, n1);
        n0 = (double)(float)n0; n1 = (double)(float)n1;
        if (n0o) *n0o = n0;
        if (n1o) *n1o = n1;
        const size_t n = (size_t)R * C;
        if (n1 < 1e-4 || n0 < 1e-4) {
            if (branch) *branch = SMHIP_BRANCH_EARLY_V0;
            SigDesc none{nullptr, nullptr, DT_F32, 1.f};
            run_combine(a, none, n0 != 0 ? (float)(1.0 / n0) : 1.f, 0.f, n, out, nullptr, false);
            read_blend_info(info, false, false, false);
            return SMHIP_OK;
        }
        const double ratio = n1 / (n0 + 1e-10);
        PairOut po;
        po.out = out; po.out_mode = OUT_F32; po.post = 1.f;
        if (ratio < bthr) {
            if (branch) *branch = SMHIP_BRANCH_LINEAR;
            if ((rc = run_f2_linear(g, (float)(1.0 / n0), (float)(1.0 / n1), (float)t))) return rc;
            if ((rc = run_inverse(g, plane(g, P_RER), plane(g, P_IMA), nullptr, po))) return rc;
            read_blend_info(info, false, false, false);
            return check_flags(true, false);
        }
        if (branch) *branch = SMHIP_BRANCH_SLERP;
        if ((rc = run_f2(g, (float)(1.0 / n0), (float)(1.0 / n1), 0, cutoff_pct > 0))) return rc;
        bool have_cull;
        spectral_blend(g, BLEND_SLERP, t, t_sum, cutoff_pct, cull_pct, 1, true, have_cull);
        if ((rc = run_inverse(g, plane(g, P_RER), plane(g, P_IMA), have_cull ? d_thr(1) : nullptr, po))) return rc;
        read_blend_info(info, cutoff_pct > 0, have_cull, true);
        if (info) { info->t = t; info->cull_pct = cull_pct; }
        return check_flags(true, false);
    }

    int run_f2_linear(const Geo& g, float s0, float s1, float t) {
        int rc = run_f2(g, s0, s1, 0, false);
        if (rc) return rc;
        const size_t total = (size_t)g.Cb * g.R;
        run_blend(g, BLEND_ARITH, 0, t, 1.f, false);
        if ((rc = ensure(tmpC_, g.plane_floats * sizeof(float)))) return rc;
        SigDesc ia{plane(g, P_IMA), nullptr, DT_F32, 1.f}, none{nullptr, nullptr, DT_F32, 1.f};
        run_combine(ia, none, 1.f, 0.f, total, (float*)tmpC_.p, nullptr, false);
        if ((rc = run_f2(g, s0, s1, 1, false))) return rc;
        SigDesc ib{plane(g, P_IMA), nullptr, DT_F32, 1.f}, ia2{tmpC_.p, nullptr, DT_F32, 1.f};
        run_combine(ia2, ib, 1.f, t, total, plane(g, P_IMA), nullptr, false);
        return SMHIP_OK;
    }

    void clear_flags() {
        if (!small_.p && reserve(1, 1)) return;
        if (!flags_clean_) be.memset(d_flags(), 0, 48, stream);
        flags_clean_ = false;
        overflow_seen_ = false;
    }
    bool select_overflowed() {
        uint32_t v = 0;
        publish(false);
        v = mail_->flags[11];
        return v != 0;
    }
    template <class F>
    int with_select_retry(F&& body) {
        int rc = body();
        if (!safe_select && overflow_seen_) {
            safe_select = true;
// ... 513 lines not shown
                    stack[i].norm = na;
                    if (two) stack[i + 1].norm = nb;
                }
            }
        }
        fused_.armed = false;
        if (ref_started && d.k != 2 && !fused_done_) { end_delta_ref_norms(); be.sync(stream); }
        if (ref_started) {
            for (int i = 0; i < d.k; ++i) stack[i].norm = (double)mail_->snorm[i];
        } else if (ref_norms) {
            SigDesc sg[16];
            double nr[16];
            for (int i = 0; i < d.k; ++i) sg[i] = stack[i].sig;
            if (!run_serial_norms(sg, d.k, n, nr))
                return fail(SMHIP_ERR_ARG, "norm_mode = reference_cpu: the torch.norm emulation does not apply to these inputs");
            for (int i = 0; i < d.k; ++i) stack[i].norm = nr[i];
        }
        double mean = 0;
        for (int i = 0; i < d.k; ++i) {
            norms32[i] = (float)stack[i].norm;
            rp.delta_norm[i] = norms32[i];
        }
        for (int i = 0; i < d.k; ++i) {
            if (!std::isfinite(norms32[i])) {
                char buf[96];
                snprintf(buf, sizeof buf, "||finetune[%d] - base[%d]|| = %g", i, i, (double)norms32[i]);
                check_flags(false, false);
                return fail(SMHIP_ERR_NONFINITE, buf);
            }
        }
        {
            float acc = 0.f;
            for (int i = 0; i < d.k; ++i) acc += norms32[i];
            mean = (double)(acc / (float)d.k);
        }
        const double target_norm = mean + d.target_norm_offset;
        rp.target_norm = target_norm;
        double cull_pct = d.cull_start_pct;

        std::vector<char> inter_busy(inter_.size(), 0);
        for (size_t q = 0; q < pool_.size(); ++q) {
            bool working = false;
            for (int i = 0; i < 4; ++i) working = working || pidx_[i] == (int)q;
            pool_busy_[q] = working ? 1 : 0;
        }
        noise_seed_ = noise_seed_base;
        int step = 0;
        int round_idx = 0;
        int pair_idx = 0;
        int deferred_step = -1;
        bool deferred_cut = false, deferred_cull = false;
        while (stack.size() > 1) {
            const int m = (int)stack.size();
            std::vector<std::pair<int, int>> pairs;
            correlated_pairs_least(norms32, m, pairs);
            std::vector<Slot> next;
            const bool last_round = (pairs.size() == 1 && pairs[0].second >= 0);
            bool any_pair = false;
            for (auto& pr : pairs) any_pair = any_pair || pr.second >= 0;
            if (!any_pair) { check_flags(false, false); return fail(SMHIP_ERR_NONFINITE, "no pair can be formed (non-finite norms)"); }
            for (auto& pr : pairs) {
                const int x = pr.first, y = pr.second;
                if (step < SMHIP_MAX_PAIRS) { rp.step_x[step] = x; rp.step_y[step] = y; }
                if (y < 0) {
                    next.push_back(stack[x]);
                    if (step < SMHIP_MAX_PAIRS) rp.step_branch[step] = SMHIP_BRANCH_CARRY;
                    ++step;
                    continue;
                }
                Slot A = stack[x], Bs = stack[y];
                const double a_w = stack[x].weight, b_w = stack[y].weight;
                if (A.norm < 0 || Bs.norm < 0) return fail(SMHIP_ERR_ARG, "internal: norm unknown");
                double na = (double)(float)A.norm, nb = (double)(float)Bs.norm;
                bool swapped = false;
                if (std::fabs(na) < std::fabs(nb)) { std::swap(A, Bs); std::swap(na, nb); swapped = true; }
                const double ca = std::fabs(na / target_norm), cb = std::fabs(nb / target_norm);
                const double ratio = cb / (ca + 1e-10);
                PairOut po;
                float* inter = nullptr;
                const bool linear = (nb / (na + 1e-10)) < d.b;
                const bool slerp_proper = !(ca < 1e-6) && !(cb < 1e-6 || ratio < 0.1) && !(nb < 1e-4 || na < 1e-4) && !linear;
                if (last_round) {
                    po = fin;
                } else if (slerp_proper && spectral_ok) {
                } else {
                    int id = -1;
                    for (size_t q = 0; q < inter_.size(); ++q) if (!inter_busy[q]) { id = (int)q; break; }
                    if (id < 0) { inter_.emplace_back(); inter_busy.push_back(0); id = (int)inter_.size() - 1; }
                    Buffer* bb = &inter_[id];
                    if ((rc = ensure(*bb, n * sizeof(float)))) return rc;
                    inter_busy[id] = 1;
                    inter = (float*)bb->p;
                    po.out = inter; po.out_mode = OUT_F32; po.post = 1.f;
                }
                int branch;
                int inv_grid = -1;
                smhip_blend_info info;
                memset(&info, 0, sizeof info);
                double out_norm = -1;
                Slot spec_slot;
                if (!slerp_proper && (A.spectral || Bs.spectral)) {
                    if ((rc = materialise(g, stack[x], inter_busy))) return rc;
                    if ((rc = materialise(g, stack[y], inter_busy))) return rc;
                    A = swapped ? stack[y] : stack[x]; Bs = swapped ? stack[x] : stack[y];
                }
                bool out_spectral = false;
                if (ca < 1e-6) {
                    branch = SMHIP_BRANCH_ADD;
                    int grid;
                    if (last_round) run_combine(A.sig, Bs.sig, 1.f, 1.f, n, delta_out, &po, false, &grid);
                    else run_combine(A.sig, Bs.sig, 1.f, 1.f, n, inter, nullptr, false, &grid);
                } else if (cb < 1e-6 || ratio < 0.1) {
                    branch = SMHIP_BRANCH_ARITH;
                    const double s = target_norm / na;
                    const double w = b_w / (a_w + 1e-10);
                    PairOut pa = po;
                    float* dtmp = nullptr;
                    if (last_round && delta_out) { pa = PairOut(); pa.out = delta_out; dtmp = delta_out; }
                    pa.ifft_policy = 0;
                    if ((rc = pair_arith(A.sig, Bs.sig, R, C, (float)s, (float)(w * s), 1.0, 1, pa, na, nb, &g))) return rc;
                    if (dtmp) {
                        SigDesc ds{dtmp, nullptr, DT_F32, 1.f}, none{nullptr, nullptr, DT_F32, 1.f};
                        run_combine(ds, none, 1.f, 0.f, n, nullptr, &fin, false);
                    }
                    f1_ready = false;
                } else {
                    branch = SMHIP_BRANCH_SLERP;
                    const double t = a_w / (a_w + b_w);
                    if (nb < 1e-4 || na < 1e-4) {
                        SigDesc none{nullptr, nullptr, DT_F32, 1.f};
                        const float sc = (float)(target_norm / na);
                        if (last_round) run_combine(A.sig, none, sc, 0.f, n, delta_out, &po, false);
                        else run_combine(A.sig, none, sc, 0.f, n, inter, nullptr, false);
                        branch = SMHIP_BRANCH_EARLY_V0;
                    } else if (linear) {
                        branch = SMHIP_BRANCH_LINEAR;
                        int grid;
                        if ((rc = run_f1(g, A.sig, Bs.sig, grid))) return rc;
                        f1_ready = false;
                        if ((rc = run_f2_linear(g, (float)(1.0 / na), (float)(1.0 / nb), (float)t))) return rc;
                        PairOut ps = po;
                        ps.post = (float)target_norm;
                        float* dtmp = nullptr;
                        if (last_round && delta_out) { ps = PairOut(); ps.out = delta_out; ps.post = (float)target_norm; dtmp = delta_out; }
                        if ((rc = run_inverse(g, plane(g, P_RER), plane(g, P_IMA), nullptr, ps, last_round ? nullptr : &inv_grid))) return rc;
                        if (dtmp) {
                            SigDesc ds{dtmp, nullptr, DT_F32, 1.f}, none{nullptr, nullptr, DT_F32, 1.f};
                            run_combine(ds, none, 1.f, 0.f, n, nullptr, &fin, false);
                        }
                    } else {
                        int im_parts = -1;
                        const bool any_spec = stack[x].spectral || stack[y].spectral ||
                                              (stack[x].rows_id >= 0 && stack[y].rows_id >= 0);
                        const bool fused1d = !any_spec && pair1d_ok(g);
                        if (fused1d) {
                            f1_ready = false;
                        } else if (!any_spec) {
                            if (!(f1_ready && d.k == 2)) {
                                int grid;
                                if ((rc = run_f1(g, stack[x].sig, stack[y].sig, grid))) return rc;
                            }
                            f1_ready = false;
                            const float s0 = (float)(1.0 / (double)(float)stack[x].norm);
                            const float s1 = (float)(1.0 / (double)(float)stack[y].norm);
                            if ((rc = run_f2(g, s0, s1, swapped ? 1 : 0, d.cutoff_pct > 0))) return rc;
                        } else {
                            f1_ready = false;
                            int* imp = (!last_round && spectral_ok && fuse_spec_norm) ? &im_parts : nullptr;
                            if (f2s_pair && g.batch == 1 && g.fold == 1 && (size_t)g.Cb * g.R <= f2s_pair_max_bins &&
                                !stack[x].spectral && !stack[y].spectral &&
                                stack[x].rows_id >= 0 && stack[y].rows_id >= 0) {
                                const bool xa = !swapped;
                                F2SSecond sec{rowspec_[stack[y].rows_id].p, !xa, (float)(1.0 / (double)(float)stack[y].norm)};
                                if ((rc = run_f2s(g, xa, (float)(1.0 / (double)(float)stack[x].norm), d.cutoff_pct > 0,
                                                  rowspec_[stack[x].rows_id].p, imp, &sec))) return rc;
                            } else
                            for (int side = 0; side < 2; ++side) {
                                const Slot& in = side == 0 ? stack[x] : stack[y];
                                const bool role_a = (side == 0) != swapped;
                                int* ip = role_a ? imp : nullptr;
                                if (in.spectral) {
                                    run_spec_rescale(g, (const float*)pool_[in.re_id].p, (const float*)pool_[in.im_id].p, in.thr,
                                                     (float)in.spec_scale, role_a, d.cutoff_pct > 0, ip);
                                } else if (in.rows_id >= 0) {
                                    if ((rc = run_f2s(g, role_a, (float)(1.0 / (double)(float)in.norm), d.cutoff_pct > 0,
                                                      rowspec_[in.rows_id].p, ip))) return rc;
                                } else {
                                    if ((rc = run_f1_rowpairs(g, in.sig))) return rc;
                                    if ((rc = run_f2s(g, role_a, (float)(1.0 / (double)(float)in.norm), d.cutoff_pct > 0, nullptr, ip))) return rc;
                                }
                            }
                        }
                        bool have_cull;
                        int sel_parts = 0;
                        const bool fused_norm = im_parts > 0 && !safe_select && cull_pct > 0;
                        if (fused1d) have_cull = cull_pct > 0;
                        else spectral_blend(g, BLEND_SLERP, t, d.t_sum, d.cutoff_pct, cull_pct, 1, true, have_cull,
                                            fused_norm ? &sel_parts : nullptr, std::min(pair_idx++, 6));
                        for (int side = 0; side < 2; ++side) {
                            Slot& in = side == 0 ? stack[x] : stack[y];
                            if (in.spectral) { pool_release(in.re_id); pool_release(in.im_id); in.re_id = in.im_id = -1; }
                        }
                        if (!last_round && spectral_ok) {
                            double sre, sim;
                            if (fused_norm && sel_parts > 0) run_spec_norm_fused(sel_parts, im_parts, sre, sim);
                            else run_spec_norm(g, plane(g, P_RER), plane(g, P_IMA), have_cull ? d_thr(1) : nullptr, sre, sim);
                            read_blend_info(&info, d.cutoff_pct > 0, have_cull, true, true);
                            const double ssum = (sre + sim) / ((double)R * (double)C);
                            out_spectral = true;
                            spec_slot = Slot();
                            spec_slot.spectral = true;
                            spec_slot.re_id = pidx_[P_RER]; spec_slot.im_id = pidx_[P_IMA];
                            spec_slot.thr = have_cull ? mail_->thr[1] : 0.f;
                            const double nrm_exact = target_norm * std::sqrt(ssum);
                            const double bias = ref_norms ? aten_gauss_norm_ratio((double)n, nrm_exact / std::sqrt((double)n)) : 1.0;
                            spec_slot.spec_scale = ssum > 0 ? 1.0 / (std::sqrt(ssum) * bias) : 1.0;
                            spec_slot.post = target_norm;
                            spec_slot.norm = nrm_exact * bias;
                            spec_slot.sig = SigDesc{nullptr, nullptr, DT_F32, 1.f};
                            const int r1 = pool_acquire(g.plane_floats * sizeof(float));
                            const int r2 = pool_acquire(g.plane_floats * sizeof(float));
                            if (r1 < 0 || r2 < 0) return SMHIP_ERR_NOMEM;
                            pidx_[P_RER] = r1; pidx_[P_IMA] = r2;
                        } else {
                        PairOut ps = po;
                        ps.post = (float)target_norm;
                        float* dtmp = nullptr;
                        if (last_round && delta_out) { ps = PairOut(); ps.out = delta_out; ps.post = (float)target_norm; dtmp = delta_out; }
                        if (fused1d) {
                            if ((rc = run_pair1d(g, A.sig, Bs.sig, na, nb, t, d.t_sum, d.cutoff_pct, cull_pct, ps,
                                                 last_round ? nullptr : &inv_grid))) return rc;
                        } else
                        if ((rc = run_inverse(g, plane(g, P_RER), plane(g, P_IMA), have_cull ? d_thr(1) : nullptr, ps,
                                              last_round ? nullptr : &inv_grid))) return rc;
                        if (dtmp) {
                            SigDesc ds{dtmp, nullptr, DT_F32, 1.f}, none{nullptr, nullptr, DT_F32, 1.f};
                            run_combine(ds, none, 1.f, 0.f, n, nullptr, &fin, false);
                        }
                        if (last_round) {
                            deferred_step = step; deferred_cut = d.cutoff_pct > 0; deferred_cull = have_cull;
                        } else {
                            read_blend_info(&info, d.cutoff_pct > 0, have_cull, true);
                        }
                        }
                    }
                }
                if (branch == SMHIP_BRANCH_SLERP || branch == SMHIP_BRANCH_LINEAR) { info.t = a_w / (a_w + b_w); info.cull_pct = cull_pct; }
                if (step < SMHIP_MAX_PAIRS) { rp.step_branch[step] = branch; rp.step_info[step] = info; }
                ++step;
                for (size_t q = 0; q < inter_.size(); ++q)
                    if (inter_[q].p && (inter_[q].p == stack[x].sig.x || inter_[q].p == stack[y].sig.x)) inter_busy[q] = 0;
                if (!last_round && out_spectral) {
                    spec_slot.weight = (a_w + b_w) / 2.0;
                    next.push_back(spec_slot);
                } else if (!last_round) {
                    SigDesc ms{inter, nullptr, DT_F32, 1.f}, none{nullptr, nullptr, DT_F32, 1.f};
                    int grid = inv_grid;
                    if (grid < 0) run_combine(ms, none, 0.f, 0.f, n, nullptr, nullptr, true, &grid);
                    double nm, dummy;
                    read_norms(grid, nm, dummy);
                    if (ref_norms) {
                        double nr;
                        if (!run_serial_norms(&ms, 1, n, &nr))
                            return fail(SMHIP_ERR_ARG, "norm_mode = reference_cpu: the torch.norm emulation does not apply to an intermediate");
                        nm = nr;
                    }
                    out_norm = nm;
                    Slot s;
                    s.sig = ms; s.weight = (a_w + b_w) / 2.0; s.norm = out_norm;
                    next.push_back(s);
                }
            }
            stack.swap(next);
            cull_pct = cull_pct / 2.0;
            ++round_idx;
            if (last_round) break;
        }
        rp.n_steps = std::min(step, (int)SMHIP_MAX_PAIRS);
        if (delta_out) {
            SigDesc ds{delta_out, nullptr, DT_F32, 1.f}, none{nullptr, nullptr, DT_F32, 1.f};
            int grid;
            run_combine(ds, none, 0.f, 0.f, n, nullptr, nullptr, true, &grid);
            double nm, dummy;
            read_norms(grid, nm, dummy);
            rp.merged_delta_norm = nm;
        }
        rc = check_flags(true, true, &rp.nan_ifft, &rp.nan_final);
        if (deferred_step >= 0 && deferred_step < SMHIP_MAX_PAIRS) {
            const double t_keep = rp.step_info[deferred_step].t, c_keep = rp.step_info[deferred_step].cull_pct;
            read_blend_info(&rp.step_info[deferred_step], deferred_cut, deferred_cull, true, true);
            rp.step_info[deferred_step].t = t_keep; rp.step_info[deferred_step].cull_pct = c_keep;
        }
        return rc;
    }

    int addition_merge(int k, const void* const* fts, const void* base, int dtype, size_t n, int mode, void* out) {
        if (k < 1 || k > ADD_MAX_MODELS) return fail(SMHIP_ERR_ARG, "k out of range");
        AdditionParams a;
        a.k = k; a.base = base; a.dtype = dtype; a.n = n; a.mode = mode; a.out = out;
        bool al = aligned16(base) && aligned16(out);
        for (int i = 0; i < ADD_MAX_MODELS; ++i) { a.ft[i] = fts[i < k ? i : 0]; al = al && aligned16(a.ft[i]); }
        a.vec8 = (n % 8 == 0) && al;
        a.chunks = pick_chunks((n + 7) / 8, 256, 2, 8);
        be.template launch<KAddition>(stream_grid((n + 7) / 8, 256, a.chunks), 256, LDS_SCRATCH_FLOATS * 4, a, stream);
        return SMHIP_OK;
    }

    static unsigned long long delta_k_keep(double density, size_t n) {
        return density == 1.0 ? (unsigned long long)n : (unsigned long long)std::floor(density * (double)n);
    }
    template <class Desc, class MergeParams>
    void delta_merge_params(const Desc& d, void* out, float* delta_out, MergeParams& m) {
        const int k = d.k;
        TiesInputs& in = m.in;
        in.k = k; in.dtype = d.in_dtype; in.n = d.n;
        bool al = aligned16(d.base_out) && aligned16(out) && aligned16(delta_out), shared = true;
        for (int i = 0; i < TIES_MAX_MODELS; ++i) {
            in.ft[i] = d.finetune[i < k ? i : 0]; in.base[i] = d.base[i < k ? i : 0];
            al = al && aligned16(in.ft[i]) && aligned16(in.base[i]);
            shared = shared && in.base[i] == in.base[0];
            m.alpha[i] = (float)d.alpha[i < k ? i : 0];
        }
        in.aligned = al ? 1 : 0; in.shared_base = shared ? 1 : 0;
        m.base_out = d.base_out; m.base_out_dtype = d.base_out_dtype;
        m.out_is_base0 = (shared && d.base_out == in.base[0] && d.base_out_dtype == d.in_dtype) ? 1 : 0;
        m.lambda = (float)d.lambda; m.normalize = d.normalize ? 1 : 0;
        m.out = out; m.delta_out = delta_out;
        m.chunks = pick_chunks((d.n + 7) / 8, 256, 2, 8);
    }
    template <class Readback>
    int delta_readback(const char* op, int k, const Readback* rb, Readback& host) {
        be.d2h(&host, rb, sizeof host, stream);
        if (!be.ok()) { host = Readback{}; return SMHIP_OK; }
        if (!host.flags[0]) return SMHIP_OK;
        std::string which;
        for (int i = 0; i < k; ++i)
            if (host.flags[0] & (1u << i)) which += (which.empty() ? "" : ", ") + std::to_string(i);
        return fail(SMHIP_ERR_NONFINITE, std::string(op) + ": NaN or Inf in finetune - base of finetune " + which);
    }
    static constexpr size_t SELECT_HIST_LEVEL = (size_t)TIES_MAX_MODELS * HIST1_BINS * sizeof(unsigned long long);
    template <class State, class Readback>
    int select_workspace(size_t states, State*& state, Readback*& rb) {
        const size_t off_state = 3 * SELECT_HIST_LEVEL, off_rb = off_state + states * sizeof(State);
        const size_t ws = off_rb + sizeof(Readback);
        int rc;
        if ((rc = ensure(ties_, ws))) return rc;
        be.memset(ties_.p, 0, ws, stream);
        state = (State*)((char*)ties_.p + off_state);
        rb = (Readback*)((char*)ties_.p + off_rb);
        return SMHIP_OK;
    }
// ... 348 lines not shown
        be.sync(stream);
        size_t nbad = 0;
        uint32_t first = ~0u;
        for (int gi = 0; gi < sgrid; ++gi) {
            nbad += h[2 * gi];
            if (h[2 * gi] && first == ~0u) first = h[2 * gi + 1];
        }
        if (nbad)
            return fail(SMHIP_ERR_ROW_NORM, "DoRA row " + std::to_string(first) + " has a zero or non-finite norm of " +
                                                "base + scale * (B @ A), or a non-finite magnitude (" + std::to_string(nbad) +
                                                " of " + std::to_string(rows) + " rows)");
        return SMHIP_OK;
    }
    int fn_exact_norm(const void* x, int dtype, size_t n, double* norm_out) {
        *norm_out = 0.0;
        if (n == 0) return SMHIP_OK;
        int rc;
        if (!small_.p && (rc = reserve(1, 1))) return rc;
        SumsqAnyParams q;
        q.x = x; q.dtype = dtype; q.n = n; q.chunks = pick_chunks(n, 256, 2, 8);
        const int grid = stream_grid(n, 256, q.chunks);
        if ((rc = ensure(tmpA_, (size_t)grid * 2 * sizeof(double)))) return rc;
        q.partials = (double*)tmpA_.p;
        be.template launch<KSumsqAny>(grid, 256, LDS_SCRATCH_FLOATS * 4, q, stream);
        SumPartialsParams sp;
        sp.partials = q.partials; sp.nparts = grid; sp.out = mail_->norm2;
        be.template launch<KSumPartials>(1, 256, LDS_SCRATCH_FLOATS * 4, sp, stream);
        be.sync(stream);
        *norm_out = std::sqrt(mail_->norm2[0]);
        return SMHIP_OK;
    }

    int correlate_pairs(int k, const void* const* tensors, int dtype, size_t rows, size_t cols, float* matrix_out) {
        if (k < 2 || k > CORR_MAX_K) return fail(SMHIP_ERR_ARG, "correlate_pairs: 2 <= k <= 8");
        int rc;
        if (!small_.p && (rc = reserve(1, 1))) return rc;
        const int P = k * (k + 1) / 2;
        const size_t cblocks = (cols + 255) / 256;
        int splits = (int)std::max<size_t>(1, std::min<size_t>(64, (size_t)1024 / cblocks));
        splits = (int)std::min<size_t>((size_t)splits, std::max<size_t>(rows, 1));
        if ((rc = ensure(tmpA_, (size_t)splits * P * cols * sizeof(double)))) return rc;
        CorrPartialParams a;
        a.k = k; a.dtype = dtype; a.rows = rows; a.cols = cols; a.splits = splits; a.part = (double*)tmpA_.p;
        for (int i = 0; i < CORR_MAX_K; ++i) a.t[i] = tensors[i < k ? i : 0];
        be.template launch<KCorrPartial>((int)(cblocks * splits), 256, LDS_SCRATCH_FLOATS * 4, a, stream);
        CorrFinishParams f;
        f.k = k; f.cols = cols; f.splits = splits; f.part = (const double*)tmpA_.p; f.eps = 1e-8f;
        f.out = (float*)mail_->corr;
        for (int i = 0; i < k * k; ++i) mail_->corr[i] = 0.f;
        be.template launch<KCorrFinish>(k * (k - 1) / 2, 256, LDS_SCRATCH_FLOATS * 4, f, stream);
        be.sync(stream);
        for (int i = 0; i < k * k; ++i) matrix_out[i] = mail_->corr[i];
        return SMHIP_OK;
    }

    int fft_transform(const float* x, int R, int C, float* spectrum) {
        const Geo g = geo(R, C);
        int rc = reserve(R, C);
        if (rc) return rc;
        SigDesc a{x, nullptr, DT_F32, 1.f}, none{nullptr, nullptr, DT_F32, 1.f};
        int grid;
        if ((rc = run_f1(g, a, none, grid))) return rc;
        if ((rc = run_f2(g, 1.f, 1.f, 0, false))) return rc;
        ExpandParams e;
        e.re = plane(g, P_REA); e.im = plane(g, P_IMA); e.R = R; e.C = C; e.Cb = g.Cb; e.full = (cf2*)spectrum; e.chunks = 8;
        be.template launch<KExpand>(stream_grid((size_t)R * C, 256, e.chunks), 256, LDS_SCRATCH_FLOATS * 4, e, stream);
        return SMHIP_OK;
    }
    int ifft_transform(const float* spectrum, int R, int C, float* out) {
        const Geo g = geo(R, C);
        int rc = reserve(R, C);
        if (rc) return rc;
        be.memset(d_flags(), 0, 32, stream);
        PackParams pk;
        pk.full = (const cf2*)spectrum; pk.R = R; pk.C = C; pk.Cb = g.Cb; pk.re = plane(g, P_RER); pk.im = plane(g, P_IMA);
        pk.chunks = 8; pk.sym = 1;
        be.template launch<KPack>(stream_grid((size_t)g.Cb * R, 256, pk.chunks), 256, LDS_SCRATCH_FLOATS * 4, pk, stream);
        PairOut po;
        po.out = out; po.out_mode = OUT_F32; po.post = 1.f;
        return run_inverse(g, plane(g, P_RER), plane(g, P_IMA), nullptr, po);
    }

    int blend_full(const float* f0, const float* f1, int R, int C, int mode, double t, double t_sum, double cutoff_pct,
                   double cull_pct, int agreement, int do_imag, float* out_spec, smhip_blend_info* info) {
        clear_flags();
        int rc = blend_full_once(f0, f1, R, C, mode, t, t_sum, cutoff_pct, cull_pct, agreement, do_imag, out_spec, info);
        if (rc == SMHIP_OK && !safe_select && select_overflowed()) {
            safe_select = true;
            rc = blend_full_once(f0, f1, R, C, mode, t, t_sum, cutoff_pct, cull_pct, agreement, do_imag, out_spec, info);
            safe_select = false;
        }
        return rc;
    }
    int blend_full_once(const float* f0, const float* f1, int R, int C, int mode, double t, double t_sum, double cutoff_pct,
                        double cull_pct, int agreement, int do_imag, float* out_spec, smhip_blend_info* info) {
        const Geo g = geo(R, C, true);
        int rc = reserve(R, C, true);
        if (rc) return rc;
        const size_t total = (size_t)R * C;
        const int sgrid = stream_grid(total, 256, 8);
        const size_t slds = LDS_SCRATCH_FLOATS * 4;
        if ((rc = ensure(fullS_, 2 * total * sizeof(float)))) return rc;
        float* im0 = (float*)fullS_.p;
        float* im1 = im0 + total;
        SplitParams sp;
        sp.n = total; sp.chunks = 8;
        sp.full = (const cf2*)f0; sp.re = plane(g, P_REA); sp.im = im0;
        be.template launch<KSplit>(sgrid, 256, slds, sp, stream);
        sp.full = (const cf2*)f1; sp.re = plane(g, P_REB); sp.im = im1;
        be.template launch<KSplit>(sgrid, 256, slds, sp, stream);
        bool have_cull;
        spectral_blend(g, mode, t, t_sum, cutoff_pct, cull_pct, agreement, false, have_cull);
        if (have_cull) {
            CullParams cp;
            cp.x = plane(g, P_RER); cp.n = total; cp.thr = d_thr(1); cp.chunks = 8;
            be.template launch<KCull>(sgrid, 256, slds, cp, stream);
        }
        read_blend_info(info, mode == BLEND_SLERP && cutoff_pct > 0, have_cull, mode == BLEND_SLERP);
        if (info) { info->t = t; info->cull_pct = cull_pct; }
        JoinParams jp;
        jp.n = total; jp.chunks = 8; jp.full = (cf2*)out_spec;
        if (!do_imag) {
            jp.re = plane(g, P_RER); jp.im = im0;
            be.template launch<KJoin>(sgrid, 256, slds, jp, stream);
            return SMHIP_OK;
        }
        if ((rc = ensure(saveR_, total * sizeof(float)))) return rc;
        if ((rc = ensure(saveI_, total * sizeof(float)))) return rc;
        if ((rc = ensure(tmpA_, 2 * total * sizeof(float)))) return rc;
        if ((rc = ensure(tmpB_, 2 * total * sizeof(float)))) return rc;
        if ((rc = ensure(tmpC_, 2 * total * sizeof(float)))) return rc;
        SigDesc rr{plane(g, P_RER), nullptr, DT_F32, 1.f}, none{nullptr, nullptr, DT_F32, 1.f};
        run_combine(rr, none, 1.f, 0.f, total, (float*)saveR_.p, nullptr, false);
        if ((rc = fft_transform(im0, R, C, (float*)tmpA_.p))) return rc;
        if ((rc = fft_transform(im1, R, C, (float*)tmpB_.p))) return rc;
        if ((rc = blend_full_once((const float*)tmpA_.p, (const float*)tmpB_.p, R, C, mode, t, 1.0, 0, 0, agreement, 0,
                                  (float*)tmpC_.p, nullptr))) return rc;
        if ((rc = ifft_transform((const float*)tmpC_.p, R, C, (float*)saveI_.p))) return rc;
        jp.re = (const float*)saveR_.p; jp.im = (const float*)saveI_.p;
        be.template launch<KJoin>(sgrid, 256, slds, jp, stream);
        return SMHIP_OK;
    }

  private:
    std::map<int, HostPlan> plans_;
    Buffer t1_, small_, tmpA_, tmpB_, tmpC_, fullS_, saveR_, saveI_, cand_, aten_, emf_;
    Buffer lora_;
    Buffer ties_;
    Buffer dora_;
    std::vector<Buffer> pool_ = std::vector<Buffer>(4);
    std::vector<char> pool_busy_ = std::vector<char>(4, 1);
    int pidx_[4] = {0, 1, 2, 3};
    uint32_t noise_seed_ = 0;
    uint32_t cap_keys_ = 0, cap_pairs_ = 0;
    bool overflow_seen_ = false;
    bool flags_clean_ = false;
    Mailbox* mail_ = nullptr;
    std::vector<Buffer> inter_;
    std::vector<Buffer> rowspec_;
    std::vector<Buffer> tr_;
    std::map<int, void*> rough_tw_;
    std::map<int, BlueHost> blue_;
    std::vector<double> host_part_;
};

}
```

Baseline: 87.48 GB/s.

## Fuse spectral rescale with speculative cutoff selection pass

Adds rescale modes to the select2 kernel. It rescales the spectral input (noise for small magnitudes, scaling otherwise), writes the rescaled planes, and in the same pass builds the level-1/level-2 histograms and candidate pairs for the cutoff selection. The selection uses a speculative guess of the threshold prefix from a previous pair slot, which is later checked by KSpecCheck, with a fallback to a normal select when the guess misses. This removes a separate pass over the data for rescale plus histogram. In exchange it adds a smaller pair staging buffer, overflow flags that mark a miss, and more register pressure. It is gated by the spec_cutoff flag.

```diff
diff --git a/shardmerge_amd/csrc/sm_capi.inc b/shardmerge_amd/csrc/sm_capi.inc
--- a/shardmerge_amd/csrc/sm_capi.inc
+++ b/shardmerge_amd/csrc/sm_capi.inc
@@ -336,6 +336,7 @@
     if (key && std::string(key) == "sel_wgs_per_cu") { ctx->pipe.sel_wgs_per_cu = value > 0 ? (int)value : 5; return SMHIP_OK; }
     if (key && std::string(key) == "pair1d") { ctx->pipe.pair1d_enabled = value != 0; return SMHIP_OK; }
     if (key && std::string(key) == "spec_cull") { ctx->pipe.spec_cull = value != 0; return SMHIP_OK; }
+    if (key && std::string(key) == "spec_cutoff") { ctx->pipe.spec_cutoff = value != 0; return SMHIP_OK; }
     if (key && std::string(key) == "spec_min_bins") { ctx->pipe.spec_min_bins = value >= 0 ? (size_t)value : (size_t)1 << 20; return SMHIP_OK; }
     if (key && std::string(key) == "dftp_pairs") { ctx->pipe.dftp_pairs_enabled = value != 0; return SMHIP_OK; }
     if (key && std::string(key) == "f2s_pair") { ctx->pipe.f2s_pair = value != 0; return SMHIP_OK; }
@@ -357,6 +358,14 @@
         *value = (long)(std::string(key) == "spec_hits" ? h : c);
         SM_FINISH(ctx, SMHIP_OK);
     }
+    if (std::string(key) == "cut_spec_role") { *value = ctx->pipe.last_cut_role(); SM_FINISH(ctx, SMHIP_OK); }
+    if (std::string(key) == "cut_spec_hit") { *value = ctx->pipe.last_spec_verdict(true); SM_FINISH(ctx, SMHIP_OK); }
+    if (std::string(key) == "cut_spec_checked" || std::string(key) == "cut_spec_hits") {
+        unsigned long long c = 0, h = 0;
+        ctx->pipe.spec_totals(&c, &h, true);
+        *value = (long)(std::string(key) == "cut_spec_hits" ? h : c);
+        SM_FINISH(ctx, SMHIP_OK);
+    }
     if (std::string(key) == "aten_fast" || std::string(key) == "aten_group" || std::string(key) == "aten_slow") {
         unsigned long long v3[3];
         ctx->pipe.aten_stats(1, v3);
diff --git a/shardmerge_amd/csrc/sm_kernels.hpp b/shardmerge_amd/csrc/sm_kernels.hpp
--- a/shardmerge_amd/csrc/sm_kernels.hpp
+++ b/shardmerge_amd/csrc/sm_kernels.hpp
@@ -1658,6 +1658,7 @@
 
 constexpr int STAGE_KEYS = 2048;
 constexpr int STAGE_PAIRS = 1024;
+constexpr int STAGE_PAIRS_RESCALE = 512;
 struct CandLists {
     uint32_t* keys;
     cf4* pairs;
@@ -1693,7 +1694,16 @@
     const BlendConsts* consts; float t_sum;
     unsigned long long* hist1_out;
     const uint32_t* guess;
+    float* rsRe; const float* rsImIn; float* rsIm;
+    float rs_thr, rs_scale, rs_sigma; uint32_t rs_seed;
+    double* rs_im_partials;
 };
+enum { SEL_PLAIN = 0, SEL_BLEND = 1, SEL_RESCALE_B = 2, SEL_RESCALE_A = 3 };
+
+SM_HD float model_noise(uint32_t seed, size_t i, float sigma);
+SM_HD float spec_rescale_one(float x, float thr, float scale, uint32_t seed, size_t i, float sigma) {
+    return (fabsf(x) < thr) ? model_noise(seed, i, sigma) : x * scale;
+}
 
 SM_HD float blend_slerp_one(const BlendConsts& c, float t_sum, float a, float b) {
     if (same_sign(a, b)) {
@@ -1703,8 +1713,10 @@
     return (fabsf(a) > fabsf(b)) ? a : b;
 }
 
-template <bool BLEND = false, class Ex>
+template <int MODE = SEL_PLAIN, class Ex>
 SM_HD void k_select2(Ex& ex, const Select2Params& p) {
+    constexpr bool BLEND = MODE == SEL_BLEND, ROLE_A = MODE == SEL_RESCALE_A, RESC = MODE == SEL_RESCALE_B || ROLE_A;
+    constexpr uint32_t NSTAGE_PAIRS = RESC ? STAGE_PAIRS_RESCALE : STAGE_PAIRS;
     typename Ex::template State<EmptyState> st;
     ex.init(st);
     uint32_t* lh = (uint32_t*)(ex.lds() + LDS_SCRATCH_FLOATS);
@@ -1714,12 +1726,12 @@
     const int nt = ex.nthreads();
     const size_t total = (size_t)p.Cb * p.R;
     const size_t nquad = (total + 3) / 4;
-    uint32_t* lh1 = lkeys + STAGE_KEYS;
+    uint32_t* lh1 = RESC ? (uint32_t*)(lpairs + STAGE_PAIRS_RESCALE) : lkeys + STAGE_KEYS;
     uint32_t prefix;
     BlendConsts bc;
-    if constexpr (BLEND) {
+    if constexpr (BLEND || RESC) {
         prefix = *p.guess - 1u;
-        bc = *p.consts;
+        if constexpr (BLEND) bc = *p.consts;
     } else {
         if (p.skip && *p.skip) return;
         wg_resolve(ex, st, p.hist1, HIST1_BINS, p.rank, (unsigned long long*)lkeys, lctl + 4);
@@ -1738,7 +1750,7 @@
     ex.each(st, [&](int tid, EmptyState&) {
         for (int b = tid; b < HIST_LO_BINS; b += nt) lh[b] = 0;
         if (tid < 8) lctl[tid] = 0;
-        if constexpr (BLEND) for (int b = tid; b < HIST1_BINS; b += nt) lh1[b] = 0;
+        if constexpr (BLEND || RESC) for (int b = tid; b < HIST1_BINS; b += nt) lh1[b] = 0;
     });
     ex.sync();
 #ifndef SM_SEL_ROUND
@@ -1747,22 +1759,56 @@
 #ifndef SM_SEL_U
 #define SM_SEL_U 4
 #endif
+#ifndef SM_SEL_U_RESCALE_B
+#define SM_SEL_U_RESCALE_B 3
+#endif
+#ifndef SM_SEL_U_RESCALE_A
+#define SM_SEL_U_RESCALE_A 2
+#endif
 #ifndef SM_DIAG_SEL
 #define SM_DIAG_SEL 0
 #endif
     constexpr int ROUND = SM_SEL_ROUND;
-    ex.each(st, [&](int, EmptyState& s) { s.red[0] = s.red[1] = s.red[2] = s.red[3] = 0.0; });
+    ex.each(st, [&](int, EmptyState& s) { s.red[0] = s.red[1] = s.red[2] = s.red[3] = s.red[4] = 0.0; });
     for (int r0 = 0; r0 < p.chunks; r0 += ROUND) {
     const int r1 = (r0 + ROUND < p.chunks) ? r0 + ROUND : p.chunks;
     ex.each(st, [&](int tid, EmptyState& s) {
-        double s00 = 0, s01 = 0, s11 = 0, cnt = 0;
+        double s00 = 0, s01 = 0, s11 = 0, cnt = 0, imacc = 0;
         const size_t start = (size_t)ex.bid() * p.chunks * nt;
-        const bool hasY = !BLEND && p.Y != nullptr;
-        auto quad = [&](size_t i0, const float* a_in, const float* b, int n, bool uniform_w) {
+        const bool hasY = RESC || (!BLEND && p.Y != nullptr);
+        const bool fuse_reduce = RESC || p.fuse_reduce, sumsq = !RESC && p.sumsq;
+        auto quad = [&](size_t i0, const float* a_in, const float* b_in, int n, bool uniform_w, const float* im_in = nullptr) {
             float q00 = 0.f, q01 = 0.f, q11 = 0.f, qc = 0.f;
             const uint32_t w0 = weight_at(wr, i0);
             float rr[4];
-            const float* a = a_in;
+            const float* a = (RESC && !ROLE_A) ? b_in : a_in;
+            const float* b = (RESC && !ROLE_A) ? rr : b_in;
+            if constexpr (RESC) {
+                const bool vst = n == 4 && uniform_w;
+#pragma unroll
+                for (int e = 0; e < 4; ++e) {
+                    uint32_t ilo = (uint32_t)i0 + (uint32_t)e;
+                    SM_OPAQUE(ilo);
+                    rr[e] = spec_rescale_one(a_in[e], p.rs_thr, p.rs_scale, p.rs_seed, (i0 & ~(size_t)0xffffffffu) | ilo, p.rs_sigma);
+                    SM_OPAQUE(rr[e]);
+                }
+                if (vst) { cf4 v = {rr[0], rr[1], rr[2], rr[3]}; *(cf4*)(p.rsRe + i0) = v; }
+                else for (int e = 0; e < n; ++e) p.rsRe[i0 + e] = rr[e];
+                if constexpr (ROLE_A) {
+                    float im[4], q = 0.f;
+#pragma unroll
+                    for (int e = 0; e < 4; ++e) im[e] = im_in[e] * p.rs_scale;
+                    if (vst) { cf4 v = {im[0], im[1], im[2], im[3]}; *(cf4*)(p.rsIm + i0) = v; }
+                    else for (int e = 0; e < n; ++e) p.rsIm[i0 + e] = im[e];
+                    if (p.rs_im_partials) {
+#pragma unroll
+                        for (int e = 0; e < 4; ++e)
+                            if (e < n) q += (float)(uniform_w ? w0 : weight_at(wr, i0 + e)) * im[e] * im[e];
+                        imacc += q;
+                    }
+                }
+                if constexpr (ROLE_A) a = rr;
+            }
             if constexpr (BLEND) {
 #pragma unroll
                 for (int e = 0; e < 4; ++e) rr[e] = blend_slerp_one(bc, p.t_sum, a_in[e], b[e]);
@@ -1784,6 +1830,10 @@
             if constexpr (BLEND) {
 #pragma unroll
                 for (int e = 0; e < 4; ++e) if (e < n) ex.lds_atomic_add(&lh1[ka[e] >> 20], wv[e]);
+            }
+            if constexpr (RESC) {
+#pragma unroll
+                for (int e = 0; e < 4; ++e) if (e < n) ex.lds_atomic_add(&lh1[(f2u(rr[e]) & 0x7fffffffu) >> 20], wv[e]);
             }
             if (hit && !(SM_DIAG_SEL & 1)) {
 #pragma unroll
@@ -1799,15 +1849,15 @@
                             ex.lds_atomic_add(&lh[(kb[e] >> 10) & 1023u], w);
                             const uint32_t pos = ex.lds_atomic_add_ret(&lctl[0], 1u);
                             if (pos < (uint32_t)STAGE_KEYS) lkeys[pos] = kb[e] | ((w - 1u) << 31);
-                            if (p.fuse_reduce && same_sign(a[e], b[e])) {
+                            if (fuse_reduce && same_sign(a[e], b[e])) {
                                 const uint32_t pp = ex.lds_atomic_add_ret(&lctl[1], 1u);
-                                if (pp < (uint32_t)STAGE_PAIRS) { cf4 v = {a[e], b[e], (float)w, 0.f}; lpairs[pp] = v; }
+                                if (pp < NSTAGE_PAIRS) { cf4 v = {a[e], b[e], (float)w, 0.f}; lpairs[pp] = v; }
                             }
                         }
                     }
                 }
             }
-            if (p.sumsq) {
+            if (sumsq) {
 #pragma unroll
                 for (int e = 0; e < 4; ++e) {
                     const bool in = (e < n) && has_hi && ka[e] >= hi;
@@ -1815,24 +1865,24 @@
                     q00 += ((float)wv[e] * av) * av;
                 }
             }
-            if (hasY && p.fuse_reduce && !(SM_DIAG_SEL & 2)) {
+            if (hasY && fuse_reduce && !(SM_DIAG_SEL & 2)) {
 #pragma unroll
                 for (int e = 0; e < 4; ++e) {
                     const bool in = (e < n) && has_hi && kb[e] >= hi && same_sign(a[e], b[e]);
                     const float wf = (float)wv[e];
                     const float av = in ? a[e] : 0.f, bv = in ? b[e] : 0.f;
                     const float wa = wf * av;
-                    q00 += wa * av; q01 += wa * bv; q11 += (wf * bv) * bv; qc += in ? wf : 0.f;
+                    q00 = fmaf(wa, av, q00); q01 = fmaf(wa, bv, q01); q11 = fmaf(wf * bv, bv, q11); qc += in ? wf : 0.f;
                 }
             }
             s00 += q00; s01 += q01; s11 += q11; cnt += qc;
         };
         if (p.vec4) {
-            constexpr int U = SM_SEL_U;
+            constexpr int U = ROLE_A ? SM_SEL_U_RESCALE_A : RESC ? SM_SEL_U_RESCALE_B : SM_SEL_U;
             const cf4* X4 = (const cf4*)p.X;
             const cf4* Y4 = (const cf4*)(BLEND ? p.blendB : p.Y);
             for (int c0 = r0; c0 < r1; c0 += U) {
-                cf4 av[U], bv[U];
+                cf4 av[U], bv[U], iv[ROLE_A ? U : 1];
                 size_t qv[U];
 #pragma unroll
                 for (int u = 0; u < U; ++u) {
@@ -1842,12 +1892,22 @@
                 if (hasY || BLEND) {
 #pragma unroll
                     for (int u = 0; u < U; ++u) bv[u] = Y4[qv[u] < nquad ? qv[u] : nquad - 1];
+                }
+                if constexpr (ROLE_A) {
+#pragma unroll
+                    for (int u = 0; u < U; ++u) iv[u] = ((const cf4*)p.rsImIn)[qv[u] < nquad ? qv[u] : nquad - 1];
                 }
 #pragma unroll
                 for (int u = 0; u < U; ++u) {
                     if (c0 + u < r1 && qv[u] < nquad) {
                         const float a[4] = {av[u].x, av[u].y, av[u].z, av[u].w};
                         const float b[4] = {bv[u].x, bv[u].y, bv[u].z, bv[u].w};
+                        if constexpr (ROLE_A) {
+                            const float im[4] = {iv[u].x, iv[u].y, iv[u].z, iv[u].w};
+                            quad(4 * qv[u], a, b, 4, true, im);
+                        } else if constexpr (RESC) {
+                            quad(4 * qv[u], a, b, 4, true);
+                        } else
                         quad(4 * qv[u], a, b, 4, !wr.full);
                     }
                 }
@@ -1860,24 +1920,33 @@
                 const int n = load_quad(p.X, 4 * qi, total, 0, a);
                 if (hasY) load_quad(p.Y, 4 * qi, total, 0, b);
                 if constexpr (BLEND) load_quad(p.blendB, 4 * qi, total, 0, b);
+                if constexpr (ROLE_A) {
+                    float im[4];
+                    load_quad(p.rsImIn, 4 * qi, total, 0, im);
+                    quad(4 * qi, a, b, n, false, im);
+                } else
                 quad(4 * qi, a, b, n, false);
             }
         }
         s.red[0] += s00; s.red[1] += s01; s.red[2] += s11; s.red[3] += cnt;
+        if constexpr (ROLE_A) s.red[4] += imacc;
     });
     ex.sync();
     const bool last_round = r1 >= p.chunks;
-    if (!last_round && !p.flush_always && lctl[0] <= (uint32_t)STAGE_KEYS / 2 && lctl[1] <= (uint32_t)STAGE_PAIRS / 2) continue;
+    if (!last_round && !p.flush_always && lctl[0] <= (uint32_t)STAGE_KEYS / 2 && lctl[1] <= NSTAGE_PAIRS / 2) continue;
     ex.each(st, [&](int tid, EmptyState&) {
         if (tid == 0) {
             uint32_t nk = lctl[0], np = lctl[1];
             bool over = false;
             if (nk > (uint32_t)STAGE_KEYS) { nk = STAGE_KEYS; over = true; }
-            if (np > (uint32_t)STAGE_PAIRS) { np = STAGE_PAIRS; over = true; }
+            if (np > NSTAGE_PAIRS) {
+                np = NSTAGE_PAIRS; over = true;
+                if constexpr (RESC) ex.global_atomic_or_u32(&p.cand.counters[2], 2u);
+            }
             const uint32_t bk = nk ? ex.global_atomic_add_ret_u32(&p.cand.counters[0], nk) : 0u;
             const uint32_t bp = np ? ex.global_atomic_add_ret_u32(&p.cand.counters[1], np) : 0u;
             if (bk + nk > p.cand.cap_keys || bp + np > p.cand.cap_pairs) over = true;
-            if (over) { ex.global_atomic_or_u32(&p.cand.counters[2], 1u); if (!BLEND) ex.global_atomic_or_u32(&p.cand.counters[3], 1u); }
+            if (over) { ex.global_atomic_or_u32(&p.cand.counters[2], 1u); if (MODE == SEL_PLAIN) ex.global_atomic_or_u32(&p.cand.counters[3], 1u); }
             lctl[0] = nk; lctl[1] = np; lctl[2] = bk; lctl[3] = bp;
         }
     });
@@ -1896,7 +1965,7 @@
             const uint32_t v = lh[b];
             if (v) ex.global_atomic_add(&p.hist[b], (unsigned long long)v);
         }
-        if constexpr (BLEND) {
+        if constexpr (BLEND || RESC) {
             for (int b = tid; b < HIST1_BINS; b += nt) {
                 const uint32_t v = lh1[b];
                 if (v) ex.global_atomic_add(&p.hist1_out[b], (unsigned long long)v);
@@ -1908,6 +1977,13 @@
         ex.template block_sum<4>(st, [&](const double* tot) {
             for (int q = 0; q < 4; ++q) p.partials[4 * (size_t)ex.bid() + q] = tot[q];
         });
+    }
+    if constexpr (ROLE_A) {
+        if (p.rs_im_partials) {
+            ex.each(st, [&](int, EmptyState& s) { s.red[0] = s.red[4]; });
+            ex.sync();
+            ex.template block_sum<1>(st, [&](const double* tot) { p.rs_im_partials[ex.bid()] = tot[0]; });
+        }
     }
 }
 
@@ -1929,7 +2005,7 @@
     ex.each(st, [&](int tid, EmptyState&) {
         if (tid == 0) {
             const uint32_t g = *p.guess;
-            const uint32_t hit = (g == res[0] + 1u) ? 1u : 0u;
+            const uint32_t hit = (g == res[0] + 1u && !(p.counters[2] & 2u)) ? 1u : 0u;
             res[3] = hit;
             *p.flag = hit;
             p.flag[1] += 1u; p.flag[2] += hit;
@@ -2664,7 +2740,7 @@
             float r[4], im[4];
 #pragma unroll
             for (int e = 0; e < 4; ++e) {
-                r[e] = (fabsf(a[e]) < p.thr) ? model_noise(p.seed, i0 + e, p.sigma) : a[e] * p.scale;
+                r[e] = spec_rescale_one(a[e], p.thr, p.scale, p.seed, i0 + e, p.sigma);
                 im[e] = b[e] * p.scale;
             }
             if (p.vec4) {
diff --git a/shardmerge_amd/csrc/sm_pipeline.hpp b/shardmerge_amd/csrc/sm_pipeline.hpp
--- a/shardmerge_amd/csrc/sm_pipeline.hpp
+++ b/shardmerge_amd/csrc/sm_pipeline.hpp
@@ -140,9 +140,11 @@
 SM_KERNEL_TAG(KPublish, PublishParams, "publish", k_publish(ex, p))
 SM_KERNEL_TAG(KHist, HistParams, "select_hist", k_hist(ex, p))
 SM_KERNEL_TAG(KScan, ScanParams, "select_scan", k_scan(ex, p))
-SM_KERNEL_TAG(KSelect2, Select2Params, "select_lvl2", k_select2<false>(ex, p))
-SM_KERNEL_TAG(KSelect2Cull, Select2Params, "select_lvl2_cull", k_select2<false>(ex, p))
-SM_KERNEL_TAG(KBlendSel, Select2Params, "blend", k_select2<true>(ex, p))
+SM_KERNEL_TAG(KSelect2, Select2Params, "select_lvl2", k_select2<SEL_PLAIN>(ex, p))
+SM_KERNEL_TAG(KSelect2Cull, Select2Params, "select_lvl2_cull", k_select2<SEL_PLAIN>(ex, p))
+SM_KERNEL_TAG(KBlendSel, Select2Params, "blend", k_select2<SEL_BLEND>(ex, p))
+SM_KERNEL_TAG_LB(KRescaleSelB, Select2Params, "spec_rescale", k_select2<SEL_RESCALE_B>(ex, p), 256, 5)
+SM_KERNEL_TAG_LB(KRescaleSelA, Select2Params, "spec_rescale", k_select2<SEL_RESCALE_A>(ex, p), 256, 5)
 SM_KERNEL_TAG(KSpecCheck, SpecCheckParams, "select_spec_check", k_spec_check(ex, p))
 SM_KERNEL_TAG(KSelect3, Select3Params, "select_lvl3_cand", k_select3(ex, p))
 SM_KERNEL_TAG(KReduceCand, ReduceCandParams, "slerp_reduce_cand", k_reduce_cand(ex, p))
@@ -215,7 +217,7 @@
 SM_KERNEL_TAG_LB(KAtenWalkC, AtenWalkParams, "aten_norm_walk", k_aten_walk<1>(ex, p), 256, 4)
 SM_KERNEL_TAG_LB(KAtenFinish, AtenFinishParams, "aten_norm_finish", k_aten_finish(ex, p), 256, 4)
 #define SM_SIDE_KERNELS_0(X) X(KAtenPre) X(KAtenPreC) X(KAtenScan) X(KAtenRec) X(KAtenPart16) X(KAtenPart32) X(KAtenPart) X(KAtenPartC) X(KAtenWalk) X(KAtenWalkC) X(KAtenFinish)
-#define SM_SIDE_KERNELS_1(X) X(KF2R1) X(KI1R1) X(KPublish) X(KHist) X(KScan) X(KSelect2) X(KSelect2Cull) X(KBlendSel) \
+#define SM_SIDE_KERNELS_1(X) X(KF2R1) X(KI1R1) X(KPublish) X(KHist) X(KScan) X(KSelect2) X(KSelect2Cull) X(KBlendSel) X(KRescaleSelB) X(KRescaleSelA) \
     X(KSpecCheck) X(KSelect3) X(KReduceCand) X(KReduce) X(KSlerpConsts) X(KSumPartials) X(KClassEmf)
 #define SM_SIDE_KERNELS_2(X) X(KDeltaNorms) X(KSumPartialsN) X(KBlend) X(KCombine) X(KExpand) X(KPack) X(KSplit) X(KJoin) \
     X(KCull) X(KAddition) X(KFnSums) X(KFnSlerpFin) X(KFnSlerpRows0) X(KFnSlerpRows1) X(KFnSlerpDen) X(KSumsqAny) X(KDivScalar) X(KCorrPartial) X(KCorrFinish) X(KSerialNorm) X(KSpecNorm) X(KSumsqCand) X(KSumSpec)       \
@@ -320,6 +322,7 @@
     uint32_t debug_sel_chunks = 0;
     bool debug_flush_always = false;
     bool spec_cull = true;
+    bool spec_cutoff = false;
     size_t spec_min_bins = 1 << 20;
     bool dftp_pairs_enabled = true;
     int debug_force_split = 0;
@@ -477,7 +480,7 @@
     static constexpr size_t OFF_PART_IM = OFF_PART + PART_DOUBLES * 8;
     static constexpr size_t PART_IM_DOUBLES = 131072;
     static constexpr size_t OFF_SPEC = OFF_PART_IM + PART_IM_DOUBLES * 8;
-    static constexpr size_t SMALL_BYTES = OFF_SPEC + 64;
+    static constexpr size_t SMALL_BYTES = OFF_SPEC + 128;
     unsigned long long* d_hist() { return (unsigned long long*)((char*)small_.p + OFF_HIST); }
     unsigned long long* d_hist2() { return d_hist() + HIST1_BINS; }
     unsigned long long* d_hist3() { return d_hist2() + HIST_LO_BINS; }
@@ -498,6 +501,8 @@
     double* d_part_im() { return (double*)((char*)small_.p + OFF_PART_IM); }
     uint32_t* d_spec_guess(int slot) { return (uint32_t*)((char*)small_.p + OFF_SPEC) + (slot < 0 ? 0 : slot > 7 ? 7 : slot); }
     uint32_t* d_spec_flag() { return (uint32_t*)((char*)small_.p + OFF_SPEC) + 8; }
+    uint32_t* d_cut_guess(int slot) { return (uint32_t*)((char*)small_.p + OFF_SPEC) + 16 + (slot < 0 ? 0 : slot > 7 ? 7 : slot); }
+    uint32_t* d_cut_flag() { return (uint32_t*)((char*)small_.p + OFF_SPEC) + 24; }
     float* plane(const Geo&, int i) { return (float*)pool_[pidx_[i]].p; }
     enum { P_REA = 0, P_IMA = 1, P_REB = 2, P_RER = 3 };
     int pool_acquire(size_t bytes) {
@@ -910,7 +915,7 @@
 
     static constexpr int CAND_GRID = 256;
     void run_select(const Geo& g, const float* X, const float* Y, unsigned long long rank, bool level1_done, float* thr_out,
-                    bool fuse_reduce = false, int* nparts_out = nullptr, bool sumsq = false, int spec_slot = -1) {
+                    bool fuse_reduce = false, int* nparts_out = nullptr, bool sumsq = false, int spec_slot = -1, int cut_slot = -1) {
         const size_t total = (size_t)g.Cb * g.R;
         HistParams h;
         h.X = X; h.Y = Y; h.R = g.R; h.C = g.Cw; h.Cb = g.Cb; h.vec4 = vec4(g); h.sel = d_sel(0);
@@ -945,6 +950,7 @@
         while ((size_t)(grid2 + CAND_GRID) * 4 > PART_DOUBLES) { q.chunks *= 2; grid2 = stream_grid((total + 3) / 4, 256, q.chunks); }
         const size_t lds2 = (LDS_SCRATCH_FLOATS + HIST_LO_BINS + 8 + STAGE_KEYS) * 4 + (size_t)STAGE_PAIRS * sizeof(cf4);
         q.skip = nullptr; q.blendB = nullptr; q.blendR = nullptr; q.consts = nullptr; q.t_sum = 0.f; q.hist1_out = nullptr; q.guess = nullptr;
+        no_rescale(q);
         if (spec_slot >= 0) {
             SpecCheckParams sc;
             sc.hist1 = d_hist(); sc.rank = rank; sc.guess = d_spec_guess(spec_slot); sc.flag = d_spec_flag();
@@ -952,6 +958,13 @@
             be.template launch<KSpecCheck>(1, 256, LDS_SCRATCH_FLOATS * 4 + (256 + 16) * 8 + 16, sc, stream);
             q.skip = d_spec_flag();
             be.template launch<KSelect2Cull>(grid2, 256, lds2, q, stream);
+        } else if (cut_slot >= 0) {
+            SpecCheckParams sc;
+            sc.hist1 = d_hist(); sc.rank = rank; sc.guess = d_cut_guess(cut_slot); sc.flag = d_cut_flag();
+            sc.sel = d_sel(0); sc.hist2 = d_hist2(); sc.counters = d_candctr();
+            be.template launch<KSpecCheck>(1, 256, LDS_SCRATCH_FLOATS * 4 + (256 + 16) * 8 + 16, sc, stream);
+            q.skip = d_cut_flag();
+            be.template launch<KSelect2>(grid2, 256, lds2, q, stream);
         } else {
             be.template launch<KSelect2>(grid2, 256, lds2, q, stream);
         }
@@ -984,9 +997,14 @@
         be.template launch<KBlend>(stream_grid((total + 3) / 4, 256, b.chunks), 256, (LDS_SCRATCH_FLOATS + HIST1_BINS) * 4, b, stream);
     }
 
+    static void no_rescale(Select2Params& q) {
+        q.rsRe = nullptr; q.rsImIn = nullptr; q.rsIm = nullptr;
+        q.rs_thr = 0.f; q.rs_scale = 1.f; q.rs_sigma = 0.f; q.rs_seed = 0; q.rs_im_partials = nullptr;
+    }
     void run_blend_spec(const Geo& g, float t_sum, bool sumsq, int spec_slot) {
         const size_t total = (size_t)g.Cb * g.R;
         Select2Params q;
+        no_rescale(q);
         q.X = plane(g, P_REA); q.Y = nullptr; q.R = g.R; q.C = g.Cw; q.Cb = g.Cb; q.vec4 = vec4(g); q.sel = d_sel(0);
         q.hist1 = nullptr; q.rank = 0; q.hist = d_hist2();
         q.cand = cand_lists(); q.fuse_reduce = 0; q.partials = d_part(); q.sumsq = sumsq ? 1 : 0;
@@ -999,16 +1017,40 @@
         const size_t lds = (LDS_SCRATCH_FLOATS + HIST_LO_BINS + 8 + STAGE_KEYS + HIST1_BINS) * 4;
         be.template launch<KBlendSel>(grid, 256, lds, q, stream);
     }
-    long last_spec_verdict() {
+    void run_rescale_spec(const Geo& g, const float* re, const float* im, float thr, float scale, bool role_a, int cut_slot,
+                          int* im_parts = nullptr) {
+        const size_t total = (size_t)g.Cb * g.R;
+        Select2Params q;
+        q.X = re; q.Y = plane(g, role_a ? P_REB : P_REA); q.R = g.R; q.C = g.Cw; q.Cb = g.Cb; q.vec4 = vec4(g); q.sel = d_sel(0);
+        q.hist1 = nullptr; q.rank = 0; q.hist = d_hist2();
+        q.cand = cand_lists(); q.fuse_reduce = 1; q.partials = d_part(); q.sumsq = 0;
+        q.flush_always = debug_flush_always ? 1 : 0;
+        q.chunks = cull_select_chunks(total);
+        q.skip = nullptr;
+        q.blendB = nullptr; q.blendR = nullptr; q.consts = nullptr; q.t_sum = 0.f;
+        q.hist1_out = d_hist(); q.guess = d_cut_guess(cut_slot);
+        q.rsRe = plane(g, role_a ? P_REA : P_REB); q.rsImIn = role_a ? im : nullptr; q.rsIm = plane(g, P_IMA);
+        last_cut_role_ = role_a ? 1 : 0;
+        q.rs_thr = thr; q.rs_scale = scale; q.rs_sigma = noise_sigma; q.rs_seed = ++noise_seed_;
+        const int grid = stream_grid((total + 3) / 4, 256, q.chunks);
+        const bool want_im = im_parts && role_a && (size_t)grid <= PART_IM_DOUBLES;
+        if (im_parts) *im_parts = want_im ? grid : -1;
+        q.rs_im_partials = want_im ? d_part_im() : nullptr;
+        const size_t lds = (LDS_SCRATCH_FLOATS + HIST_LO_BINS + 8 + STAGE_KEYS + HIST1_BINS) * 4 + (size_t)STAGE_PAIRS_RESCALE * sizeof(cf4);
+        if (role_a) be.template launch<KRescaleSelA>(grid, 256, lds, q, stream);
+        else be.template launch<KRescaleSelB>(grid, 256, lds, q, stream);
+    }
+    long last_cut_role() const { return last_cut_role_; }
+    long last_spec_verdict(bool cutoff = false) {
         if (!small_.p) return -1;
         uint32_t v = 0;
-        be.d2h(&v, d_spec_flag(), sizeof v, stream);
+        be.d2h(&v, cutoff ? d_cut_flag() : d_spec_flag(), sizeof v, stream);
         be.sync(stream);
         return (long)v;
     }
-    void spec_totals(unsigned long long* checked, unsigned long long* hits) {
+    void spec_totals(unsigned long long* checked, unsigned long long* hits, bool cutoff = false) {
         uint32_t v[3] = {0, 0, 0};
-        if (small_.p) { be.d2h(v, d_spec_flag(), sizeof v, stream); be.sync(stream); }
+        if (small_.p) { be.d2h(v, cutoff ? d_cut_flag() : d_spec_flag(), sizeof v, stream); be.sync(stream); }
         *checked = v[1]; *hits = v[2];
     }
     int cull_select_chunks(size_t total) const {
@@ -1155,7 +1197,8 @@
     }
 
     void spectral_blend(const Geo& g, int mode, double t, double t_sum, double cutoff_pct, double cull_pct,
-                        int agreement, bool level1_hist_done, bool& have_cull, int* sumsq_parts = nullptr, int spec_slot = 7) {
+                        int agreement, bool level1_hist_done, bool& have_cull, int* sumsq_parts = nullptr, int spec_slot = 7,
+                        int cut_slot = -1) {
         const unsigned long long nfull = (unsigned long long)g.R * g.C * (unsigned long long)g.batch;
         have_cull = false;
         if (mode == BLEND_SLERP) {
@@ -1163,7 +1206,7 @@
             int fused = 0;
             if (have_cut)
                 run_select(g, plane(g, P_REA), plane(g, P_REB), pct_index(2 * nfull, cutoff_pct), level1_hist_done, d_thr(0),
-                           true, &fused);
+                           true, &fused, false, -1, cut_slot);
             const float* class_norms = nullptr;
             const double* emf_part = nullptr;
             int emf_nparts = 0, emf_elo = 0;
@@ -1983,6 +2026,10 @@
                         int im_parts = -1;
                         const bool any_spec = stack[x].spectral || stack[y].spectral ||
                                               (stack[x].rows_id >= 0 && stack[y].rows_id >= 0);
+                        const int pair_slot = std::min(pair_idx, 6);
+                        const bool cut_spec = (stack[x].spectral || stack[y].spectral) && d.cutoff_pct > 0 && spec_cutoff &&
+                                              !safe_select && !g.full && (size_t)g.Cb * g.R >= spec_min_bins;
+                        const int cut_slot = cut_spec ? pair_slot : -1;
                         const bool fused1d = !any_spec && pair1d_ok(g);
                         if (fused1d) {
                             f1_ready = false;
@@ -2006,11 +2053,16 @@
                                 if ((rc = run_f2s(g, xa, (float)(1.0 / (double)(float)stack[x].norm), d.cutoff_pct > 0,
                                                   rowspec_[stack[x].rows_id].p, imp, &sec))) return rc;
                             } else
-                            for (int side = 0; side < 2; ++side) {
+                            for (int turn = 0; turn < 2; ++turn) {
+                                const int fused_side = cut_spec ? (stack[y].spectral ? 1 : 0) : -1;
+                                const int side = (cut_spec && fused_side == 0) ? 1 - turn : turn;
                                 const Slot& in = side == 0 ? stack[x] : stack[y];
                                 const bool role_a = (side == 0) != swapped;
                                 int* ip = role_a ? imp : nullptr;
-                                if (in.spectral) {
+                                if (in.spectral && side == fused_side) {
+                                    run_rescale_spec(g, (const float*)pool_[in.re_id].p, (const float*)pool_[in.im_id].p, in.thr,
+                                                     (float)in.spec_scale, role_a, cut_slot, ip);
+                                } else if (in.spectral) {
                                     run_spec_rescale(g, (const float*)pool_[in.re_id].p, (const float*)pool_[in.im_id].p, in.thr,
                                                      (float)in.spec_scale, role_a, d.cutoff_pct > 0, ip);
                                 } else if (in.rows_id >= 0) {
@@ -2027,7 +2079,7 @@
                         const bool fused_norm = im_parts > 0 && !safe_select && cull_pct > 0;
                         if (fused1d) have_cull = cull_pct > 0;
                         else spectral_blend(g, BLEND_SLERP, t, d.t_sum, d.cutoff_pct, cull_pct, 1, true, have_cull,
-                                            fused_norm ? &sel_parts : nullptr, std::min(pair_idx++, 6));
+                                            fused_norm ? &sel_parts : nullptr, std::min(pair_idx++, 6), cut_slot);
                         for (int side = 0; side < 2; ++side) {
                             Slot& in = side == 0 ? stack[x] : stack[y];
                             if (in.spectral) { pool_release(in.re_id); pool_release(in.im_id); in.re_id = in.im_id = -1; }
@@ -2682,6 +2734,7 @@
     std::vector<char> pool_busy_ = std::vector<char>(4, 1);
     int pidx_[4] = {0, 1, 2, 3};
     uint32_t noise_seed_ = 0;
+    int last_cut_role_ = -1;
     uint32_t cap_keys_ = 0, cap_pairs_ = 0;
     bool overflow_seen_ = false;
     bool flags_clean_ = false;
```

Result: slower. 86.33 GB/s (-1.3%).
